# IGNF/StrataNet2-Vegetation-Coverage-Maps

Measured on AMD Instinct MI355X. Metric: plots/s fwd+bwd, 32k-pt synthetic plots, batch 16/GPU, higher is better.
Workload: dtype f32; 1 GPU; C2 ref-arch: 16 plots/GPU x 32768 pts, SA npoint 1024/256 + global, r 1/2 m, train step fwd+P2+loss+bwd+Adam, inputs resident in HBM; plots_per_gpu=16, points_per_plot=32768, batches_per_geometry_pass=8, exchange=none (single GPU), parallelism=single GPU, ranks_seen=1, exchange_in_graph=False

## Files before the change

### include/strata_hip.h

```cpp
#ifndef STRATA_HIP_H
#define STRATA_HIP_H

#include <stddef.h>

#ifdef __cplusplus
extern "C" {
#endif

#define SN2_VERSION 102
#define SN2_EINVAL (-1)
#define SN2_ELIMIT (-2)

#define SN2_MAX_NEIGHBORS 2000
#define SN2_STAT_SLOTS 1024

int sn2_version(void);
int sn2_debug_mfma_chain(const float *a, const float *b, float *d, int mode, void *stream);
int sn2_debug_spin(int blocks, long long clocks, int *out, void *stream);

int sn2_debug_fp1_backward_parts(int mask);
int sn2_debug_fp_rows_form(int form);
int sn2_debug_fp_table_form(int form);
#define SN2_PROBE_SINK_WORDS 4096
int sn2_debug_stream_probe(const float *src, float *dst, size_t n_floats, int mode, float *sink, void *stream);
// ... 35 lines not shown
int sn2_fps_waves(const float *pos_soa, int B, int N, int M, const int *start, int *idx, float *cpos_soa,
                  float *cpos_aos, int *order_ws, int waves, void *stream);
int sn2_fps_status(const float *pos_soa, int B, int N, int M, const int *start, int *idx, float *cpos_soa,
                   float *cpos_aos, int *order_ws, int waves, unsigned *status, void *stream);
int sn2_fps_live(const float *pos_soa, int B, int N, int M, const int *start, const int *n_live, int *idx, float *cpos_soa,
                 float *cpos_aos, int *order_ws, int waves, int *n_live_out, unsigned *status, void *stream);
int sn2_debug_fps_spin_limit(unsigned sweeps);

int sn2_ball_query(const float *src_soa, int B, int N, const float *cpos_soa, int M, float r2, int cap,
                   int *nbr, int *cnt, unsigned long long *total, const int *fps_ws, void *stream);

int sn2_count_sum(const int *cnt, int n, unsigned long long *total, void *stream);
int sn2_count_sum_group(const int *cnt, int G, int n, unsigned long long *total, size_t total_stride, void *stream);

#define SN2_THREE_NN_WS_WORDS(B, S) ((size_t)(B) * (4 * (size_t)(S) + 1032))
size_t sn2_three_nn_ws_words(int B, int S);
int sn2_three_nn(const float *src_soa, int B, int S, const float *dst_soa, int T, int k, int *idx, float *w,
                 void *ws, const int *dst_fps_ws, void *stream);
#define SN2_THREE_NN_XY_WS_WORDS(B, S, T) ((size_t)(B) * (4 * (size_t)(S) + 5 * (size_t)(T) + 1032))
size_t sn2_three_nn_xy_ws_words(int B, int S, int T);
int sn2_three_nn_xy(const float *src_soa, int B, int S, const float *dst_soa, int T, int k, int *idx, float *w,
                    void *ws, void *stream);

int sn2_prepare_plots(const float *raw, long T, const int *offsets, const float *centers, const float *fake_xy, int n_fake,
                      const int *idx, int B, int N, int train, const double *rot, const int *flips, const float *noise,
                      const long *noise_offsets, long noise_T, float z_max, float *cloud, float *xyz, void *stream);

#define SN2_SUBSAMPLE_LDS 1
#define SN2_SUBSAMPLE_GLOBAL 2
#define SN2_SUBSAMPLE_COARSE 4
#define SN2_SUBSAMPLE_LDS_MAX 16384
int sn2_subsample_form(int n_max, int N);
size_t sn2_subsample_ws_words(int B, int n_max, int N, int form);
int sn2_subsample(const int *offsets, int extra, int n_max, int B, int N, unsigned long long seed, const long long *plot_keys,
                  int form, int *ws, size_t ws_words, int *idx, void *stream);

int sn2_train_batch_ws_words(int B, int n_max, int N, size_t *words);
int sn2_train_batch(const float *raw, long T, const int *offsets, const float *centers, const double *coverages, int P,
                    const int *plot_ids, int B, const float *fake_xy, int n_fake, int n_max, int N, int M1, float z_max,
                    unsigned long long seed, long long epoch, const double *cos_sin, int train, int noise, int *ws,
                    size_t ws_words, float *cloud, float *xyz, double *gt, int *fps_start, void *stream);
int sn2_train_batch_live(const float *raw, long T, const int *offsets, const float *centers, const double *coverages, int P,
                         const int *plot_ids, int B, const float *fake_xy, int n_fake, int n_max, int N, int M1, float z_max,
                         unsigned long long seed, long long epoch, const double *cos_sin, int train, int noise, int *ws,
                         size_t ws_words, float *cloud, float *xyz, double *gt, int *fps_start, int *n_live, void *stream);

int sn2_plots_append(const float *src_raw, long src_T, const int *src_offsets, const float *src_centers, const float *src_cov,
                     const int *sel, int K, float *dst_raw, long cap_T, int *dst_offsets, float *dst_centers, double *dst_cov,
                     int cap_P, int P0, long T0, const int *dst_start, long new_T, void *stream);

#define SN2_ZNORM_WS_WORDS(n, cells) ((size_t)5 * (n) + 3 * (size_t)(cells) + 8)
size_t sn2_znorm_ws_words(int n, long cells);
int sn2_znorm(const float *x, const float *y, const float *z, int n, float radius, float x_min, float y_min, float x_max,
              float y_max, int *ws, float *zmin, float *z_out, void *stream);

size_t sn2_parcel_count_ws_words(int P, int rows);
size_t sn2_parcel_znorm_ws_words(long T, float radius, float x_min, float y_min, float x_max, float y_max);
int sn2_parcel_count(const float *cloud, long T, int L, int rows, const float *centers, int P, const int *cell_start,
                     const int *cell_items, int GX, int GY, double gx0, double gy0, double cell_inv, float radius, int *ws,
                     size_t ws_words, int *prefix, long long *total, void *stream);
int sn2_parcel_fill(const float *cloud, long T, int L, int rows, const float *centers, int P, const int *cell_start,
                    const int *cell_items, int GX, int GY, double gx0, double gy0, double cell_inv, float radius, int *prefix,
                    const int *plot_base, long sum_n, float *raw, int *point_index, void *stream);
int sn2_parcel_znorm(const float *cloud, long T, float x_min, float y_min, float x_max, float y_max, float radius,
                     float disc_radius, const int *offsets, const float *centers, int P, const int *point_index, long sum_n,
                     int *ws, size_t ws_words, float *raw, void *stream);

typedef struct sn2_sa {
    int B, Nsrc, M, cap;
    int cf;
    int nl;
    const float *feat; int feat_stride;
    const float *spos; int spos_stride;
    const float *cpos;
    const int *nbr, *cnt;
    const unsigned long long *total;
    const int *order;
    sn2_block blk[2];
    float *ext; int *arg;
    float *out;
    const float *dout;
    float *dfeat;
    float *bwd_ws;
} sn2_sa;
#define SN2_SA_BWD_WS_REPLICAS 32
#define SN2_SA_BWD_WS_WORDS (SN2_SA_BWD_WS_REPLICAS * 2 * 16 * 12)
#define SN2_SA_SOLO_MIN 64
#define SN2_SA_QUAD_MIN 8
#define SN2_SA_OCT_MIN 4
#define SN2_SA_SOLO_FLAG 0x40000000
#define SN2_SA_OCT_FLAG 0x20000000
#define SN2_SA_PACKED_ITEMS(M) ((M) / 8 + 2)
#define SN2_SA_ORDER_WORDS(B, M) ((size_t)4 * (B) * (M) + (size_t)16 * (B) * SN2_SA_PACKED_ITEMS(M) + 8)
size_t sn2_sa_order_words(int B, int M);
int sn2_sa_order(const int *cnt, int B, int M, int *order, void *stream);
int sn2_sa_order_group(const int *cnt, int G, int B, int M, int *order, size_t stride_words, void *stream);
int sn2_sa_forward(const sn2_sa *p, int training, void *stream);
int sn2_sa_backward(const sn2_sa *p, void *stream);

typedef struct sn2_fp {
    int B, R_per_plot, S_per_plot;
    int ca, cb;
    const float *src; int src_stride; const float *src_a, *src_c;
    const int *knn_idx; const float *knn_w;
    const float *skip; int skip_stride;
    sn2_block blk;
    float *h; int h_stride;
    const float *dy;
    float *dsrc; int dsrc_stride;
    float *dskip; int dskip_stride;
    float *du_scratch;
    float *scatter_ws;
    int scatter_ready;
    const int *bn_sums_done;
    float *src_ws;
    int act_bf16;
    const int *row_perm;
} sn2_fp;
#define SN2_INTERP_CHUNKS(R, S) ((3 * (size_t)(R) + 62) / 63 + (size_t)(S))
#define SN2_FP_SRC_WS_WORDS(B, R, S, cout) ((size_t)(B) * SN2_INTERP_CHUNKS(R, S) * ((((cout) + 3) / 4) * 4))
size_t sn2_interp_chunks(int R_per_plot, int S_per_plot);
size_t sn2_fp_src_ws_words(int B, int R_per_plot, int S_per_plot, int cout);
#define SN2_INTERP_WS_WORDS(B, R, S) \
    ((size_t)(B) * (S) * (((R) + 2047) / 2048 + 6) + 6 * (size_t)(B) * (R) + 64 + 4 * (size_t)(B) * SN2_INTERP_CHUNKS(R, S))
size_t sn2_interp_ws_words(int B, int R_per_plot, int S_per_plot);
int sn2_interp_index(const int *knn_idx, const float *knn_w, const float *src_pos, int B, int R_per_plot,
                     int S_per_plot, float *ws, void *stream);
int sn2_interp_index_perm(const int *knn_idx, const float *knn_w, const float *src_pos, const int *row_perm, int B,
                          int R_per_plot, int S_per_plot, float *ws, void *stream);
int sn2_interp_index_group(const int *knn_idx, const float *knn_w, const float *src_pos, const int *row_perm, int G, int B,
                           int R_per_plot, int S_per_plot, float *ws, size_t ws_stride_words, void *stream);
int sn2_fp_forward(const sn2_fp *p, int training, void *stream);
int sn2_fp_backward(const sn2_fp *p, void *stream);

int sn2_plot_max_forward(const float *h, const float *a, const float *c, int B, int R_per_plot, int C, float *out,
                         int *arg, void *stream);
int sn2_plot_max_backward(const float *dout, const int *arg, int B, int R_per_plot, int C, float *dy, void *stream);

int sn2_global_pool_backward(const float *du, int du_stride, const int *arg, const float *h, const float *mean,
                             const float *invstd, int B, int R_per_plot, int C, float *dx, float *dy, float *dgamma,
                             float *dbeta, void *stream);

#define SN2_GLOBAL_MAX_PLOTS 28
#define SN2_GLOBAL_XCHG_WORDS(B) ((size_t)2 * (size_t)(B) * 4 * 128)
#define SN2_GLOBAL_CTL_WORDS 8
size_t sn2_global_xchg_words(int B);
int sn2_global_level_forward(const sn2_fp *sa3, const sn2_fp *fp3, float *x3, int *arg3, unsigned long long *xchg,
                             unsigned *ctl, void *stream);
#define SN2_GLOBAL_BWD_MAX_ROWS 256
#define SN2_GLOBAL_BWD_XCHG_WORDS ((size_t)2 * SN2_GLOBAL_MAX_PLOTS * 128)
#define SN2_GLOBAL_BWD_CTL_WORDS 64
int sn2_global_level_backward(const sn2_fp *sa3, const sn2_fp *fp3, const int *arg3, unsigned long long *xchg, unsigned *ctl,
                              void *stream);
int sn2_debug_global_spin_limit(unsigned sweeps);

#define SN2_HEAD_LOSS_MAX_PLOTS 128
typedef struct sn2_loss_grad {
    const float *pred;
    const double *gt;
    const float *proba;
    const double *pdf;
    const double *grad_total;
    const int *arg, *nocc, *pix;
    int B, N, D;
    double m, e;
} sn2_loss_grad;

typedef struct sn2_head {
    int R, cin, f_stride;
    const float *f, *fa, *fc;
    const float *W1, *b1, *W2, *b2;
    float *coverages, *proba;
    const float *dcoverages, *dproba;
    float *dy;
    float *dW1, *db1, *dW2, *db2;
    int grad_replicas, grad_replica_stride;
    const int *drop_mask;
    float drop_scale;
    int act_bf16;
    float *zero_fill; long zero_fill_words;
    const sn2_loss_grad *loss;
} sn2_head;
int sn2_head_forward(const sn2_head *p, void *stream);
int sn2_fp_head_eval(const sn2_fp *p, const sn2_head *hd, void *stream);
int sn2_head_backward(const sn2_head *p, void *stream);
int sn2_debug_head_backward_occupancy(int bf16, int with_loss);
int sn2_head_bn_sums(const sn2_head *p, const float *gamma, const float *beta, const float *mean, const float *invstd,
                     float *dgamma, float *dbeta, int *ok, void *stream);
int sn2_fp_bn_sums(const sn2_fp *p, const float *gamma, const float *beta, const float *mean, const float *invstd,
                   float *dgamma, float *dbeta, int *ok, void *stream);


int sn2_plot_project_forward(const float *pred_pointwise, const float *cloud_xy, long plot_stride, int B, int N,
                             int D, unsigned long long *keys, int *pix, int *arg, int *nocc, float *pred,
                             void *stream);
#define SN2_P2_KEY_PARTS(N) (((N) + 4095) / 4096 < 1 ? 1 : (((N) + 4095) / 4096 > 64 ? 64 : ((N) + 4095) / 4096))
size_t sn2_p2_key_parts(int N);
int sn2_plot_pixels(const float *cloud_xy, long plot_stride, int B, int N, int D, float *mm, int *pix, void *stream);
int sn2_plot_project_forward_pix(const float *pred_pointwise, const int *pix, int B, int N, int D,
                                 unsigned long long *keys, int *arg, int *nocc, float *pred, void *stream);
int sn2_plot_project_backward(const float *dpred, const int *arg, const int *nocc, const int *pix, int B, int N,
                              int D, float *dpointwise, void *stream);

int sn2_raster_project(const float *coverages, const float *cloud_xy, long plot_stride, int B, int N, int D,
                       int diam_meters, unsigned long long *keys, int *pix, float *rasters, void *stream);

int sn2_mosaic_merge(const float *rasters, const float *weights, const int *offsets, int B, int D, int H, int W,
                     float *mean, float *wsum, int win_y0, int win_x0, int win_h, int win_w, void *stream);

#define SN2_MOSAIC_HIST_WORDS 10004
int sn2_mosaic_finalize(const float *mean, const float *wsum, int H, int W, int *hist_ws, double *sum_ws, float *thr_out,
                        float *out, void *stream);

#define SN2_MOSAIC_CROP_MAX_BANDS 8
#define SN2_MOSAIC_CROP_MAX_EDGES (1 << 20)
#define SN2_MOSAIC_CROP_MAX_BLOCKS 2048
#define SN2_MOSAIC_CROP_BLOCKS(H, W) \
    ((size_t)(H) * (((size_t)(W) + 255) / 256) < SN2_MOSAIC_CROP_MAX_BLOCKS ? (size_t)(H) * (((size_t)(W) + 255) / 256) \
                                                                           : (size_t)SN2_MOSAIC_CROP_MAX_BLOCKS)
#define SN2_MOSAIC_CROP_WS_WORDS(C, H, W) (4 * (size_t)(C) * SN2_MOSAIC_CROP_BLOCKS(H, W))
extern size_t sn2_mosaic_crop_ws_words(int C, int H, int W);
int sn2_mosaic_crop_stats(float *bands, int C, int H, int W, double x_min, double y_max, double pix, const double *edges, int E,
                          void *ws, double *mean, long long *count, void *stream);

#define SN2_ATLAS_CANVAS_COLS 8
#define SN2_ATLAS_SEG_COLS 8
#define SN2_ATLAS_FINALIZE_MAX_BLOCKS 1024
#define SN2_ATLAS_FINALIZE_BLOCKS(H, W) \
    (((size_t)(H) * (size_t)(W) + 255) / 256 < SN2_ATLAS_FINALIZE_MAX_BLOCKS ? ((size_t)(H) * (size_t)(W) + 255) / 256 \
                                                                            : (size_t)SN2_ATLAS_FINALIZE_MAX_BLOCKS)
int sn2_atlas_canvas_table(int K, const int *H, const int *W, const double *x_min, const double *y_max, long long *table);

int sn2_atlas_merge(const float *rasters, const float *weights, const int *place, int B, int D, int K, const long long *canvas_host,
                    const long long *canvas_dev, const int *seg_host, const int *seg_dev, int S, float *mean, float *wsum,
                    void *stream);

#define SN2_ATLAS_FINALIZE_CANVAS_WORDS (SN2_MOSAIC_HIST_WORDS + 2 * SN2_ATLAS_FINALIZE_MAX_BLOCKS)
#define SN2_ATLAS_FINALIZE_WS_WORDS(K) ((size_t)(K) * SN2_ATLAS_FINALIZE_CANVAS_WORDS)
int sn2_atlas_finalize_ws_words(int K, size_t *words);
int sn2_atlas_finalize(const float *mean, const float *wsum, int K, const long long *canvas_host, const long long *canvas_dev,
                       void *ws, float *thr, float *bands, void *stream);

int sn2_atlas_crop_stats(float *bands, int C, int K, const long long *canvas_host, const long long *canvas_dev, double pix,
                         const double *edges, const int *edge_start_host, const int *edge_start_dev, void *ws, double *mean,
                         long long *count, void *stream);

int sn2_kde_lookup(const float *cloud, int B, int C, int N, int z_channel, float z_max, const double *X, const double *Y,
                   int K, double *pdf, void *stream);
#define SN2_KDE_FIT_MAX_K 65536
#define SN2_KDE_FIT_ABS_SLOTS 256
#define SN2_KDE_FIT_SLICES 8
#define SN2_KDE_FIT_WS_WORDS(K) \
    (2 * ((4 + 3 * SN2_KDE_FIT_SLICES) * (size_t)(K) + 3 * (((size_t)(K) + 255) / 256)) + SN2_KDE_FIT_ABS_SLOTS)
size_t sn2_kde_fit_ws_words(int K);
int sn2_kde_fit(const float *z, long n, double bw, int K, void *ws, double *X, double *Y, void *stream);
#define SN2_LOSS_BLOCKS 1024
int sn2_loss_forward(const float *pred, const double *gt, int B, const float *proba, const double *pdf, int R, double m,
                     double e, double *partials, double *out, void *stream);
int sn2_loss_backward(const float *pred, const double *gt, int B, const float *proba, const double *pdf, int R, double m,
                      double e, const double *grad_total, float *dpred, float *dproba, void *stream);

#define SN2_PROJECTED_LOSS_WS (2 * 512 + 2)
int sn2_projected_loss_forward(const float *coverages, const int *pix, const float *proba, const double *pdf, const double *gt,
                               int B, int N, int D, double m, double e, unsigned long long *keys, int *arg, int *nocc,
                               float *pred, double *partials, double *out, void *stream);
int sn2_projected_loss_backward(const float *pred, const double *gt, int B, const float *proba, const double *pdf, int N, int D,
                                double m, double e, const double *grad_total, const int *arg, const int *nocc, const int *pix,
                                float *dcoverages, float *dproba, void *stream);

#define SN2_PLOT_LOSSES_SLICE_ROWS 2048
#define SN2_PLOT_LOSSES_SLICES(N) \
    (((N) + SN2_PLOT_LOSSES_SLICE_ROWS - 1) / SN2_PLOT_LOSSES_SLICE_ROWS < 1 ? 1 : \
     (((N) + SN2_PLOT_LOSSES_SLICE_ROWS - 1) / SN2_PLOT_LOSSES_SLICE_ROWS > 64 ? 64 : ((N) + SN2_PLOT_LOSSES_SLICE_ROWS - 1) / SN2_PLOT_LOSSES_SLICE_ROWS))
size_t sn2_plot_losses_ws_words(int B, int N, int D);
int sn2_plot_losses(const float *coverages, const int *pix, const float *proba, const double *pdf, const double *gt, int B, int N,
                    int D, double m, double e, void *ws, float *pred, double *out, void *stream);

int sn2_adam_step(float *param, const float *grad, float *exp_avg, float *exp_avg_sq, int n, float lr, float beta1,
                  float beta2, float eps, float weight_decay, int *step_dev ,
                  float grad_scale, void *stream);

#define SN2_METER_TERMS 4
int sn2_adam_step_dev(float *param, const float *grad, float *exp_avg, float *exp_avg_sq, int n, const float *lr_dev, float beta1,
                      float beta2, float eps, float weight_decay, int *step_dev, float grad_scale, const double *terms, int n_terms,
                      double *meter, void *stream);


typedef struct sn2_net_layer {
    int cin, cout;
    const float *W, *b, *gamma, *beta;
    float *running_mean, *running_var;
    long long *num_batches_tracked;
    int gW, gb, ggamma, gbeta;
    int mma_bf16;
} sn2_net_layer;

typedef struct sn2_net_model {
    sn2_net_layer sa1[2], sa2, sa3, fp3, fp2, fp1;
    const float *lin1_W, *lin1_b, *lin2_W, *lin2_b;
    int g_lin1_W, g_lin1_b, g_lin2_W, g_lin2_b;
    int n_flat;
    float r1_sq, r2_sq;
    int max_neighbors;
    float drop_p;
    int fuse_global_level;
    int fuse_eval_head;
    int source_side;
    int fps_waves_shared, fps_waves_many;
} sn2_net_model;

typedef struct sn2_net_dims {
    int B, N, M1, M2;
    int cap1, cap2;
    int act_bf16;
    int p2_diam_pix;
} sn2_net_dims;

typedef struct sn2_net_geo {
    const float *xyz;
    int *idx1; float *pos1_soa, *pos1_aos; int *ws1;
    int *nbr1, *cnt1; unsigned long long *tot1; int *ord1;
    int *idx2; float *pos2_soa, *pos2_aos; int *ws2;
    int *nbr2, *cnt2; unsigned long long *tot2; int *ord2;
    const float *pos3;
    int *knn3_idx; float *knn3_w;
    int *knn2_idx; float *knn2_w;
    int *knn1_idx; float *knn1_w;
    float *inv3, *inv2, *inv1;
    int *nn_ws2, *nn_ws1;
    const int *rank1;
    float *rows0;
    int *p2_pix; float *p2_mm;
} sn2_net_geo;

typedef struct sn2_net_act {
    float *aux;
    float *stats;
    float *ext1; int *arg1; float *x1;
    float *ext2; int *arg2; float *x2;
    float *h_sa3, *h3;
    float *x3; int *arg3;
    float *h2;
    void *h1;
    float *src_ws1, *src_ws2;
    float *cov, *proba;
    const int *drop_mask;
    float *bwd_arena; long bwd_arena_words;
} sn2_net_act;

#define SN2_NET_GRAD_IMAGES 32
typedef struct sn2_net_bwd {
    const float *dcov, *dproba;
    float *arena; long arena_words;
    int images, image_stride;
    float *dy2, *dy3, *dx1, *dx2, *dx3, *dy_sa3;
    float *sa1_ws;
    void *dy1, *du1;
    float *du2, *du3;
    int *bn_ok;
    float *src_ws1, *src_ws2;
    int defer_grad_reduce;
    int arena_is_zero;
    int frozen_stats;
    unsigned long long *gl_xchg; unsigned *gl_ctl;
    const sn2_loss_grad *loss;
} sn2_net_bwd;

#define SN2_NET_FORK 1
#define SN2_NET_SHARED 2
#define SN2_NET_INVERTED 4
#define SN2_NET_DEFER_JOIN 8
#define SN2_NET_INPUT_ONLY 16
#define SN2_NET_HAS_ROWS0 32
#define SN2_NET_JOIN_PENDING 64
#define SN2_NET_WITH_GEOMETRY 128
#define SN2_NET_HAS_INVERTED 256

typedef struct sn2_net_io {
    const float *cloud;
    const int *fps_start;
    unsigned *fps_status;
    unsigned long long *gl_xchg; unsigned *gl_ctl;
    void *stream_b, *stream_c, *stream_pack;
    void *ctx;
    int flags;
    int training;
    const int *fps_live;
    int *fps_live1;
} sn2_net_io;

int sn2_net_ctx_create(void **ctx);
int sn2_net_ctx_destroy(void *ctx);
int sn2_net_geo_carve(const sn2_net_model *m, const sn2_net_dims *d, void *base, sn2_net_geo *out, size_t *bytes);
int sn2_net_act_carve(const sn2_net_model *m, const sn2_net_dims *d, int training, void *base, sn2_net_act *out, size_t *bytes);
int sn2_net_bwd_carve(const sn2_net_model *m, const sn2_net_dims *d, void *arena_base, void *scratch_base, sn2_net_bwd *out,
                      size_t *arena_bytes, size_t *scratch_bytes);
int sn2_net_geometry(const sn2_net_model *m, const sn2_net_dims *d, const sn2_net_geo *g, const sn2_net_io *io, void *stream);
int sn2_net_forward(const sn2_net_model *m, const sn2_net_dims *d, const sn2_net_geo *g, const sn2_net_act *a,
                    const sn2_net_io *io, void *stream);
int sn2_net_backward(const sn2_net_model *m, const sn2_net_dims *d, const sn2_net_geo *g, const sn2_net_act *a,
                     const sn2_net_bwd *b, void *stream);

int sn2_adam_step_images(float *param, float *grad_images, int replicas, int stride, float *exp_avg, float *exp_avg_sq, int n,
                         float lr, float beta1, float beta2, float eps, float weight_decay, int *step_dev, float grad_scale,
                         void *stream);
int sn2_adam_step_images_dev(float *param, float *grad_images, int replicas, int stride, float *exp_avg, float *exp_avg_sq, int n,
                             const float *lr_dev, float beta1, float beta2, float eps, float weight_decay, int *step_dev,
                             float grad_scale, const double *terms, int n_terms, double *meter, void *stream);

int sn2_fps_fills_ws(int B, int N, int M);
int sn2_three_nn_uses_grid(int S, int T);
int sn2_fp_rows_small(long R);
int sn2_fp_source_side(long R, int cb, int force);
int sn2_global_level_forward_route(int B, int bf16);
int sn2_global_level_backward_route(int B, int M2, int frozen, int bf16);
int sn2_head_loss_route(int B, int N, int D);

#ifdef __cplusplus
}
#endif
#endif
```

### stratanet2_vegetation_coverage_maps_amd/_lib.py

```python
import ctypes
import functools
import os
from ctypes import POINTER, Structure, c_double, c_float, c_int, c_long, c_longlong, c_void_p

HERE = os.path.dirname(os.path.abspath(__file__))
LIB_PATH = os.path.join(HERE, "csrc", "libstrata_hip.so")

CONSTANTS = {
    "SN2_VERSION": 102, "SN2_EINVAL": -1, "SN2_ELIMIT": -2,
    "SN2_MAX_NEIGHBORS": 2000, "SN2_STAT_SLOTS": 1024, "SN2_BN_FROZEN_KEEP": 2,
    "SN2_FPS_WS_GRID_WORDS": 4104, "SN2_FPS_WS_CTL_WORDS": 32,
    "SN2_SUBSAMPLE_LDS": 1, "SN2_SUBSAMPLE_GLOBAL": 2, "SN2_SUBSAMPLE_COARSE": 4, "SN2_SUBSAMPLE_LDS_MAX": 16384,
    "SN2_SA_BWD_WS_WORDS": 32 * 2 * 16 * 12,
    "SN2_GLOBAL_MAX_PLOTS": 28, "SN2_GLOBAL_CTL_WORDS": 8, "SN2_GLOBAL_BWD_MAX_ROWS": 256,
    "SN2_GLOBAL_BWD_XCHG_WORDS": 2 * 28 * 128, "SN2_GLOBAL_BWD_CTL_WORDS": 64,
    "SN2_MOSAIC_HIST_WORDS": 10004, "SN2_MOSAIC_CROP_MAX_BANDS": 8, "SN2_MOSAIC_CROP_MAX_EDGES": 1 << 20,
    "SN2_MOSAIC_CROP_MAX_BLOCKS": 2048, "SN2_ATLAS_CANVAS_COLS": 8, "SN2_ATLAS_SEG_COLS": 8, "SN2_ATLAS_FINALIZE_MAX_BLOCKS": 1024,
    "SN2_ATLAS_FINALIZE_CANVAS_WORDS": 10004 + 2 * 1024, "SN2_KDE_FIT_MAX_K": 65536, "SN2_LOSS_BLOCKS": 1024, "SN2_PROJECTED_LOSS_WS": 2 * 512 + 2,
    "SN2_NET_GRAD_IMAGES": 32, "SN2_METER_TERMS": 4,
    "SN2_NET_FORK": 1, "SN2_NET_SHARED": 2, "SN2_NET_INVERTED": 4, "SN2_NET_DEFER_JOIN": 8, "SN2_NET_INPUT_ONLY": 16,
    "SN2_NET_HAS_ROWS0": 32, "SN2_NET_JOIN_PENDING": 64, "SN2_NET_WITH_GEOMETRY": 128, "SN2_NET_HAS_INVERTED": 256,
}
globals().update(CONSTANTS)
MAX_NEIGHBORS, STAT_SLOTS, BN_FROZEN_KEEP = CONSTANTS["SN2_MAX_NEIGHBORS"], CONSTANTS["SN2_STAT_SLOTS"], CONSTANTS["SN2_BN_FROZEN_KEEP"]
(NET_FORK, NET_SHARED, NET_INVERTED, NET_DEFER_JOIN, NET_INPUT_ONLY, NET_HAS_ROWS0, NET_JOIN_PENDING, NET_WITH_GEOMETRY,
 NET_HAS_INVERTED) = (CONSTANTS["SN2_NET_" + n] for n in ("FORK", "SHARED", "INVERTED", "DEFER_JOIN", "INPUT_ONLY", "HAS_ROWS0",
                                                          "JOIN_PENDING", "WITH_GEOMETRY", "HAS_INVERTED"))


class Block(Structure):
    _fields_ = [("cin", c_int), ("cout", c_int), ("W", c_void_p), ("b", c_void_p), ("gamma", c_void_p),
                ("beta", c_void_p), ("running_mean", c_void_p), ("running_var", c_void_p), ("a", c_void_p),
                ("c", c_void_p), ("mean", c_void_p), ("invstd", c_void_p), ("stat_slots", c_void_p),
                ("dW", c_void_p), ("db", c_void_p), ("dgamma", c_void_p), ("dbeta", c_void_p),
                ("grad_replicas", c_int), ("grad_replica_stride", c_int), ("mma_bf16", c_int),
                ("num_batches_tracked", c_void_p), ("frozen_stats", c_int)]


class SA(Structure):
    _fields_ = [("B", c_int), ("Nsrc", c_int), ("M", c_int), ("cap", c_int), ("cf", c_int), ("nl", c_int),
                ("feat", c_void_p), ("feat_stride", c_int), ("spos", c_void_p), ("spos_stride", c_int),
                ("cpos", c_void_p), ("nbr", c_void_p), ("cnt", c_void_p), ("total", c_void_p), ("order", c_void_p),
                ("blk", Block * 2),
                ("ext", c_void_p), ("arg", c_void_p), ("out", c_void_p), ("dout", c_void_p), ("dfeat", c_void_p),
                ("bwd_ws", c_void_p)]


class FP(Structure):
    _fields_ = [("B", c_int), ("R_per_plot", c_int), ("S_per_plot", c_int), ("ca", c_int), ("cb", c_int),
                ("src", c_void_p), ("src_stride", c_int), ("src_a", c_void_p), ("src_c", c_void_p),
                ("knn_idx", c_void_p), ("knn_w", c_void_p), ("skip", c_void_p), ("skip_stride", c_int),
                ("blk", Block), ("h", c_void_p), ("h_stride", c_int), ("dy", c_void_p), ("dsrc", c_void_p),
                ("dsrc_stride", c_int), ("dskip", c_void_p), ("dskip_stride", c_int), ("du_scratch", c_void_p),
                ("scatter_ws", c_void_p), ("scatter_ready", c_int), ("bn_sums_done", c_void_p), ("src_ws", c_void_p),
                ("act_bf16", c_int), ("row_perm", c_void_p)]


class LossGrad(Structure):
    _fields_ = [(n, c_void_p) for n in ("pred", "gt", "proba", "pdf", "grad_total", "arg", "nocc", "pix")] + [
        ("B", c_int), ("N", c_int), ("D", c_int), ("m", c_double), ("e", c_double)]


class Head(Structure):
    _fields_ = [("R", c_int), ("cin", c_int), ("f_stride", c_int), ("f", c_void_p), ("fa", c_void_p),
                ("fc", c_void_p), ("W1", c_void_p), ("b1", c_void_p), ("W2", c_void_p), ("b2", c_void_p),
                ("coverages", c_void_p), ("proba", c_void_p), ("dcoverages", c_void_p), ("dproba", c_void_p),
                ("dy", c_void_p), ("dW1", c_void_p), ("db1", c_void_p), ("dW2", c_void_p), ("db2", c_void_p),
                ("grad_replicas", c_int), ("grad_replica_stride", c_int), ("drop_mask", c_void_p), ("drop_scale", c_float),
                ("act_bf16", c_int), ("zero_fill", c_void_p), ("zero_fill_words", c_long), ("loss", POINTER(LossGrad))]


class NetLayer(Structure):
    _fields_ = [("cin", c_int), ("cout", c_int), ("W", c_void_p), ("b", c_void_p), ("gamma", c_void_p), ("beta", c_void_p),
                ("running_mean", c_void_p), ("running_var", c_void_p), ("num_batches_tracked", c_void_p),
                ("gW", c_int), ("gb", c_int), ("ggamma", c_int), ("gbeta", c_int), ("mma_bf16", c_int)]


class NetModel(Structure):
    _fields_ = [("sa1", NetLayer * 2), ("sa2", NetLayer), ("sa3", NetLayer), ("fp3", NetLayer), ("fp2", NetLayer), ("fp1", NetLayer),
                ("lin1_W", c_void_p), ("lin1_b", c_void_p), ("lin2_W", c_void_p), ("lin2_b", c_void_p),
                ("g_lin1_W", c_int), ("g_lin1_b", c_int), ("g_lin2_W", c_int), ("g_lin2_b", c_int), ("n_flat", c_int),
                ("r1_sq", c_float), ("r2_sq", c_float), ("max_neighbors", c_int), ("drop_p", c_float),
                ("fuse_global_level", c_int), ("fuse_eval_head", c_int), ("source_side", c_int),
                ("fps_waves_shared", c_int), ("fps_waves_many", c_int)]


class NetDims(Structure):
    _fields_ = [("B", c_int), ("N", c_int), ("M1", c_int), ("M2", c_int), ("cap1", c_int), ("cap2", c_int), ("act_bf16", c_int),
                ("p2_diam_pix", c_int)]


class NetGeo(Structure):
    _fields_ = [(n, c_void_p) for n in (
        "xyz", "idx1", "pos1_soa", "pos1_aos", "ws1", "nbr1", "cnt1", "tot1", "ord1",
        "idx2", "pos2_soa", "pos2_aos", "ws2", "nbr2", "cnt2", "tot2", "ord2", "pos3",
        "knn3_idx", "knn3_w", "knn2_idx", "knn2_w", "knn1_idx", "knn1_w", "inv3", "inv2", "inv1", "nn_ws2", "nn_ws1",
        "rank1", "rows0", "p2_pix", "p2_mm")]


class NetAct(Structure):
    _fields_ = [(n, c_void_p) for n in (
        "aux", "stats", "ext1", "arg1", "x1", "ext2", "arg2", "x2", "h_sa3", "h3", "x3", "arg3", "h2", "h1", "src_ws1", "src_ws2",
        "cov", "proba", "drop_mask", "bwd_arena")] + [("bwd_arena_words", c_long)]


class NetBwd(Structure):
    _fields_ = [("dcov", c_void_p), ("dproba", c_void_p), ("arena", c_void_p), ("arena_words", c_long), ("images", c_int),
                ("image_stride", c_int)] + [(n, c_void_p) for n in (
                    "dy2", "dy3", "dx1", "dx2", "dx3", "dy_sa3", "sa1_ws", "dy1", "du1", "du2", "du3", "bn_ok", "src_ws1", "src_ws2")] + [
                        ("defer_grad_reduce", c_int), ("arena_is_zero", c_int), ("frozen_stats", c_int), ("gl_xchg", c_void_p),
                        ("gl_ctl", c_void_p), ("loss", POINTER(LossGrad))]


class NetIO(Structure):
    _fields_ = [("cloud", c_void_p), ("fps_start", c_void_p), ("fps_status", c_void_p), ("gl_xchg", c_void_p), ("gl_ctl", c_void_p),
                ("stream_b", c_void_p), ("stream_c", c_void_p), ("stream_pack", c_void_p), ("ctx", c_void_p), ("flags", c_int),
                ("training", c_int), ("fps_live", c_void_p), ("fps_live1", c_void_p)]


SIGNATURES = {
    "sn2_version": [],
    "sn2_debug_mfma_chain": [c_void_p, c_void_p, c_void_p, c_int, c_void_p],
    "sn2_debug_spin": [c_int, c_longlong, c_void_p, c_void_p],
    "sn2_debug_fp1_backward_parts": [c_int],
    "sn2_debug_fp_rows_form": [c_int],
    "sn2_debug_fp_table_form": [c_int],
    "sn2_debug_stream_probe": [c_void_p, c_void_p, ctypes.c_size_t, c_int, c_void_p, c_void_p],
    "sn2_debug_mfma_probe": [c_int, c_int, c_void_p, POINTER(c_double), c_void_p],
    "sn2_pack_rows": [c_void_p, c_void_p, c_int, c_int, c_int, c_void_p, c_void_p],
    "sn2_fps": [c_void_p, c_int, c_int, c_int, c_void_p, c_void_p, c_void_p, c_void_p, c_void_p, c_void_p],
    "sn2_fps_waves": [c_void_p, c_int, c_int, c_int, c_void_p, c_void_p, c_void_p, c_void_p, c_void_p, c_int, c_void_p],
    "sn2_fps_status": [c_void_p, c_int, c_int, c_int, c_void_p, c_void_p, c_void_p, c_void_p, c_void_p, c_int, c_void_p, c_void_p],
    "sn2_fps_live": [c_void_p, c_int, c_int, c_int, c_void_p, c_void_p, c_void_p, c_void_p, c_void_p, c_void_p, c_int, c_void_p, c_void_p,
                     c_void_p],
    "sn2_debug_fps_spin_limit": [ctypes.c_uint],
    "sn2_ball_query": [c_void_p, c_int, c_int, c_void_p, c_int, c_float, c_int, c_void_p, c_void_p, c_void_p, c_void_p,
                       c_void_p],
    "sn2_three_nn": [c_void_p, c_int, c_int, c_void_p, c_int, c_int, c_void_p, c_void_p, c_void_p, c_void_p, c_void_p],
    "sn2_count_sum": [c_void_p, c_int, c_void_p, c_void_p],
    "sn2_count_sum_group": [c_void_p, c_int, c_int, c_void_p, ctypes.c_size_t, c_void_p],
    "sn2_three_nn_xy": [c_void_p, c_int, c_int, c_void_p, c_int, c_int, c_void_p, c_void_p, c_void_p, c_void_p],
    "sn2_prepare_plots": [c_void_p, c_long, c_void_p, c_void_p, c_void_p, c_int, c_void_p, c_int, c_int, c_int, c_void_p,
                          c_void_p, c_void_p, c_void_p, c_long, c_float, c_void_p, c_void_p, c_void_p],
    "sn2_znorm": [c_void_p, c_void_p, c_void_p, c_int, c_float, c_float, c_float, c_float, c_float, c_void_p, c_void_p,
                  c_void_p, c_void_p],
    "sn2_parcel_count": [c_void_p, c_long, c_int, c_int, c_void_p, c_int, c_void_p, c_void_p, c_int, c_int, c_double, c_double,
                         c_double, c_float, c_void_p, ctypes.c_size_t, c_void_p, c_void_p, c_void_p],
    "sn2_parcel_fill": [c_void_p, c_long, c_int, c_int, c_void_p, c_int, c_void_p, c_void_p, c_int, c_int, c_double, c_double,
                        c_double, c_float, c_void_p, c_void_p, c_long, c_void_p, c_void_p, c_void_p],
    "sn2_parcel_znorm": [c_void_p, c_long, c_float, c_float, c_float, c_float, c_float, c_float, c_void_p, c_void_p, c_int,
                         c_void_p, c_long, c_void_p, ctypes.c_size_t, c_void_p, c_void_p],
    "sn2_subsample_form": [c_int, c_int],
    "sn2_subsample": [c_void_p, c_int, c_int, c_int, c_int, ctypes.c_ulonglong, c_void_p, c_int, c_void_p, ctypes.c_size_t,
                      c_void_p, c_void_p],
    "sn2_train_batch_ws_words": [c_int, c_int, c_int, POINTER(ctypes.c_size_t)],
    "sn2_train_batch": [c_void_p, c_long, c_void_p, c_void_p, c_void_p, c_int, c_void_p, c_int, c_void_p, c_int, c_int, c_int, c_int,
                        c_float, ctypes.c_ulonglong, c_longlong, c_void_p, c_int, c_int, c_void_p, ctypes.c_size_t, c_void_p, c_void_p,
                        c_void_p, c_void_p, c_void_p],
    "sn2_train_batch_live": [c_void_p, c_long, c_void_p, c_void_p, c_void_p, c_int, c_void_p, c_int, c_void_p, c_int, c_int, c_int, c_int,
                             c_float, ctypes.c_ulonglong, c_longlong, c_void_p, c_int, c_int, c_void_p, ctypes.c_size_t, c_void_p,
                             c_void_p, c_void_p, c_void_p, c_void_p, c_void_p],
    "sn2_plots_append": [c_void_p, c_long, c_void_p, c_void_p, c_void_p, c_void_p, c_int, c_void_p, c_long, c_void_p, c_void_p,
                         c_void_p, c_int, c_int, c_long, c_void_p, c_long, c_void_p],
    "sn2_sa_order": [c_void_p, c_int, c_int, c_void_p, c_void_p],
    "sn2_sa_order_group": [c_void_p, c_int, c_int, c_int, c_void_p, ctypes.c_size_t, c_void_p],
    "sn2_sa_forward": [POINTER(SA), c_int, c_void_p],
    "sn2_sa_backward": [POINTER(SA), c_void_p],
    "sn2_grad_reduce": [c_void_p, c_int, c_int, c_int, c_void_p],
    "sn2_interp_index": [c_void_p, c_void_p, c_void_p, c_int, c_int, c_int, c_void_p, c_void_p],
    "sn2_interp_index_perm": [c_void_p, c_void_p, c_void_p, c_void_p, c_int, c_int, c_int, c_void_p, c_void_p],
    "sn2_interp_index_group": [c_void_p, c_void_p, c_void_p, c_void_p, c_int, c_int, c_int, c_int, c_void_p, ctypes.c_size_t, c_void_p],
    "sn2_fp_forward": [POINTER(FP), c_int, c_void_p],
    "sn2_fp_backward": [POINTER(FP), c_void_p],
    "sn2_plot_max_forward": [c_void_p, c_void_p, c_void_p, c_int, c_int, c_int, c_void_p, c_void_p, c_void_p],
    "sn2_plot_max_backward": [c_void_p, c_void_p, c_int, c_int, c_int, c_void_p, c_void_p],
    "sn2_global_pool_backward": [c_void_p, c_int, c_void_p, c_void_p, c_void_p, c_void_p, c_int, c_int, c_int, c_void_p, c_void_p,
                                 c_void_p, c_void_p, c_void_p],
    "sn2_global_level_forward": [POINTER(FP), POINTER(FP), c_void_p, c_void_p, c_void_p, c_void_p, c_void_p],
    "sn2_global_level_backward": [POINTER(FP), POINTER(FP), c_void_p, c_void_p, c_void_p, c_void_p],
    "sn2_debug_global_spin_limit": [ctypes.c_uint],
    "sn2_head_forward": [POINTER(Head), c_void_p],
    "sn2_fp_head_eval": [POINTER(FP), POINTER(Head), c_void_p],
    "sn2_fp_bn_sums": [POINTER(FP), c_void_p, c_void_p, c_void_p, c_void_p, c_void_p, c_void_p, c_void_p, c_void_p],
    "sn2_head_bn_sums": [POINTER(Head), c_void_p, c_void_p, c_void_p, c_void_p, c_void_p, c_void_p, c_void_p, c_void_p],
    "sn2_head_backward": [POINTER(Head), c_void_p],
    "sn2_debug_head_backward_occupancy": [c_int, c_int],
    "sn2_plot_project_forward": [c_void_p, c_void_p, c_long, c_int, c_int, c_int, c_void_p, c_void_p, c_void_p,
                                 c_void_p, c_void_p, c_void_p],
    "sn2_plot_pixels": [c_void_p, c_long, c_int, c_int, c_int, c_void_p, c_void_p, c_void_p],
    "sn2_plot_project_forward_pix": [c_void_p, c_void_p, c_int, c_int, c_int, c_void_p, c_void_p, c_void_p, c_void_p, c_void_p],
    "sn2_plot_project_backward": [c_void_p, c_void_p, c_void_p, c_void_p, c_int, c_int, c_int, c_void_p, c_void_p],
    "sn2_raster_project": [c_void_p, c_void_p, c_long, c_int, c_int, c_int, c_int, c_void_p, c_void_p, c_void_p,
                           c_void_p],
    "sn2_mosaic_merge": [c_void_p, c_void_p, c_void_p, c_int, c_int, c_int, c_int, c_void_p, c_void_p,
                         c_int, c_int, c_int, c_int, c_void_p],
    "sn2_mosaic_finalize": [c_void_p, c_void_p, c_int, c_int, c_void_p, c_void_p, c_void_p, c_void_p, c_void_p],
    "sn2_mosaic_crop_stats": [c_void_p, c_int, c_int, c_int, c_double, c_double, c_double, c_void_p, c_int, c_void_p, c_void_p,
                              c_void_p, c_void_p],
    "sn2_atlas_canvas_table": [c_int, c_void_p, c_void_p, c_void_p, c_void_p, c_void_p],
    "sn2_atlas_finalize_ws_words": [c_int, POINTER(ctypes.c_size_t)],
    "sn2_atlas_merge": [c_void_p, c_void_p, c_void_p, c_int, c_int, c_int, c_void_p, c_void_p, c_void_p, c_void_p, c_int, c_void_p,
                        c_void_p, c_void_p],
    "sn2_atlas_finalize": [c_void_p, c_void_p, c_int, c_void_p, c_void_p, c_void_p, c_void_p, c_void_p, c_void_p],
    "sn2_atlas_crop_stats": [c_void_p, c_int, c_int, c_void_p, c_void_p, c_double, c_void_p, c_void_p, c_void_p, c_void_p, c_void_p,
                             c_void_p, c_void_p],
    "sn2_kde_lookup": [c_void_p, c_int, c_int, c_int, c_int, c_float, c_void_p, c_void_p, c_int, c_void_p, c_void_p],
    "sn2_kde_fit": [c_void_p, c_long, c_double, c_int, c_void_p, c_void_p, c_void_p, c_void_p],
    "sn2_loss_forward": [c_void_p, c_void_p, c_int, c_void_p, c_void_p, c_int, c_double, c_double, c_void_p, c_void_p,
                         c_void_p],
    "sn2_loss_backward": [c_void_p, c_void_p, c_int, c_void_p, c_void_p, c_int, c_double, c_double, c_void_p, c_void_p,
                          c_void_p, c_void_p],
    "sn2_adam_step": [c_void_p, c_void_p, c_void_p, c_void_p, c_int, c_float, c_float, c_float, c_float, c_float,
                      c_void_p, c_float, c_void_p],
    "sn2_adam_step_dev": [c_void_p, c_void_p, c_void_p, c_void_p, c_int, c_void_p, c_float, c_float, c_float, c_float,
                          c_void_p, c_float, c_void_p, c_int, c_void_p, c_void_p],
    "sn2_projected_loss_forward": [c_void_p, c_void_p, c_void_p, c_void_p, c_void_p, c_int, c_int, c_int, c_double, c_double, c_void_p,
                                   c_void_p, c_void_p, c_void_p, c_void_p, c_void_p, c_void_p],
    "sn2_projected_loss_backward": [c_void_p, c_void_p, c_int, c_void_p, c_void_p, c_int, c_int, c_double, c_double, c_void_p, c_void_p,
                                    c_void_p, c_void_p, c_void_p, c_void_p, c_void_p],
    "sn2_plot_losses": [c_void_p, c_void_p, c_void_p, c_void_p, c_void_p, c_int, c_int, c_int, c_double, c_double, c_void_p, c_void_p,
                        c_void_p, c_void_p],
    "sn2_adam_step_images": [c_void_p, c_void_p, c_int, c_int, c_void_p, c_void_p, c_int, c_float, c_float, c_float, c_float, c_float,
                             c_void_p, c_float, c_void_p],
    "sn2_adam_step_images_dev": [c_void_p, c_void_p, c_int, c_int, c_void_p, c_void_p, c_int, c_void_p, c_float, c_float, c_float,
                                 c_float, c_void_p, c_float, c_void_p, c_int, c_void_p, c_void_p],
    "sn2_net_ctx_create": [POINTER(c_void_p)],
    "sn2_net_ctx_destroy": [c_void_p],
    "sn2_net_geo_carve": [POINTER(NetModel), POINTER(NetDims), c_void_p, POINTER(NetGeo), POINTER(ctypes.c_size_t)],
    "sn2_net_act_carve": [POINTER(NetModel), POINTER(NetDims), c_int, c_void_p, POINTER(NetAct), POINTER(ctypes.c_size_t)],
    "sn2_net_bwd_carve": [POINTER(NetModel), POINTER(NetDims), c_void_p, c_void_p, POINTER(NetBwd), POINTER(ctypes.c_size_t),
                          POINTER(ctypes.c_size_t)],
    "sn2_net_geometry": [POINTER(NetModel), POINTER(NetDims), POINTER(NetGeo), POINTER(NetIO), c_void_p],
    "sn2_net_forward": [POINTER(NetModel), POINTER(NetDims), POINTER(NetGeo), POINTER(NetAct), POINTER(NetIO), c_void_p],
    "sn2_net_backward": [POINTER(NetModel), POINTER(NetDims), POINTER(NetGeo), POINTER(NetAct), POINTER(NetBwd), c_void_p],
    "sn2_fps_fills_ws": [c_int, c_int, c_int],
    "sn2_three_nn_uses_grid": [c_int, c_int],
    "sn2_fp_rows_small": [c_long],
    "sn2_fp_source_side": [c_long, c_int, c_int],
    "sn2_global_level_forward_route": [c_int, c_int],
    "sn2_global_level_backward_route": [c_int, c_int, c_int, c_int],
    "sn2_head_loss_route": [c_int, c_int, c_int],
}

SIZE_HELPERS = {
    "sn2_fps_ws_words": [c_int, c_int],
    "sn2_fps_ws_grid_offset": [c_int, c_int],
    "sn2_fps_ws_ctl_offset": [c_int, c_int],
    "sn2_fps_ws_rank_offset": [c_int, c_int],
    "sn2_three_nn_ws_words": [c_int, c_int],
    "sn2_three_nn_xy_ws_words": [c_int, c_int, c_int],
    "sn2_znorm_ws_words": [c_int, c_long],
    "sn2_sa_order_words": [c_int, c_int],
    "sn2_interp_chunks": [c_int, c_int],
    "sn2_interp_ws_words": [c_int, c_int, c_int],
    "sn2_fp_src_ws_words": [c_int, c_int, c_int, c_int],
    "sn2_global_xchg_words": [c_int],
    "sn2_p2_key_parts": [c_int],
    "sn2_kde_fit_ws_words": [c_int],
    "sn2_parcel_count_ws_words": [c_int, c_int],
    "sn2_parcel_znorm_ws_words": [c_long, c_float, c_float, c_float, c_float, c_float],
    "sn2_subsample_ws_words": [c_int, c_int, c_int, c_int],
    "sn2_plot_losses_ws_words": [c_int, c_int, c_int],
}

EXTERN_SIZE_HELPERS = {
    "sn2_mosaic_crop_ws_words": [c_int, c_int, c_int],
}

_lib = None


class StrataHipError(RuntimeError):
    pass


def load():
    global _lib
    if _lib is not None:
        return _lib
    if not os.path.exists(LIB_PATH):
        raise StrataHipError(
            f"{LIB_PATH} not found: build it with `python -m stratanet2_vegetation_coverage_maps_amd._build` "
            "(or __graft_entry__.build()); the HIP library is mandatory, there is no fallback path")
    lib = ctypes.CDLL(LIB_PATH)
    for name, argtypes in SIGNATURES.items():
        fn = getattr(lib, name)
        fn.argtypes = argtypes
        fn.restype = c_int
    for name, argtypes in list(SIZE_HELPERS.items()) + list(EXTERN_SIZE_HELPERS.items()):
        fn = getattr(lib, name)
        fn.argtypes = argtypes
        fn.restype = ctypes.c_size_t
    if lib.sn2_version() != SN2_VERSION:
        raise StrataHipError(f"libstrata_hip.so version {lib.sn2_version()} != binding {SN2_VERSION}: rebuild")
    _lib = lib
    return lib


@functools.lru_cache(maxsize=4096)
def host_value(name: str, *args) -> int:
    return getattr(load(), name)(*args)


def check(rc: int, what: str):
    if rc != 0:
        kind = "hipError_t" if rc > 0 else {-1: "SN2_EINVAL", -2: "SN2_ELIMIT"}.get(rc, "error")
        raise StrataHipError(f"{what} failed: {kind} {rc}")
```

### stratanet2_vegetation_coverage_maps_amd/csrc/common.h

```cpp
#pragma once
#include <hip/hip_runtime.h>
#include <stdint.h>

#include "../../include/strata_hip.h"

#define SN2_WAVE 64

#define SN2_RETURN_LAUNCH()                                   \
    do {                                                      \
        hipError_t e__ = hipGetLastError();                   \
        return e__ == hipSuccess ? 0 : (int)e__;              \
    } while (0)

#define SN2_TRY(expr)                \
    do {                             \
        int r__ = (expr);            \
        if (r__ != 0) return r__;    \
    } while (0)

#ifdef SN2_NO_FLUSH
#define SN2_FLUSH_ADD(ptr, v) do { if ((v) == 12345.678f) atomicAdd((ptr), (v)); } while (0)
#else
#define SN2_FLUSH_ADD(ptr, v) atomicAdd((ptr), (v))
#endif

#ifdef __HIPCC__
__device__ __forceinline__ int sn2_grad_image(int replicas, int stride) {
    return replicas > 1 ? (int)(blockIdx.x % (unsigned)replicas) * stride : 0;
}
#endif

static inline int sn2_cdiv(long a, long b) { return (int)((a + b - 1) / b); }

constexpr int GL_MAX_PLOTS = SN2_GLOBAL_MAX_PLOTS;
constexpr int GL_BWD_MAX_ROWS = SN2_GLOBAL_BWD_MAX_ROWS;

#ifdef __HIPCC__
static __global__ __launch_bounds__(256) void sn2_fill_words_kernel(uint32_t* __restrict__ p, uint32_t v, size_t n) {
    for (size_t i = (size_t)blockIdx.x * 256 + threadIdx.x; i < n; i += (size_t)gridDim.x * 256) p[i] = v;
}
static inline void sn2_fill_words(void* p, uint32_t v, size_t nwords, hipStream_t st) {
    if (nwords == 0) return;
    int grid = sn2_cdiv((long)nwords, 256 * 4);
    grid = grid < 1 ? 1 : (grid > 2048 ? 2048 : grid);
    hipLaunchKernelGGL(sn2_fill_words_kernel, dim3(grid), dim3(256), 0, st, (uint32_t*)p, v, nwords);
}
#endif

static inline bool sn2_small_sort_wg(int B) { return B > 32; }

static inline int sn2_cu_count() {
    static int n = 0;
    if (n == 0) {
        int dev = 0, v = 0;
        if (hipGetDevice(&dev) == hipSuccess &&
            hipDeviceGetAttribute(&v, hipDeviceAttributeMultiprocessorCount, dev) == hipSuccess && v > 0)
            n = v;
        else
            n = 256;
    }
    return n;
}

int sn2_subsample_ids(const int* offsets, const int* ids, int extra, int n_max, int B, int N, unsigned long long seed,
                      const long long* plot_keys, int form, int* ws, size_t ws_words, int* idx, hipStream_t stream);

typedef const float __attribute__((address_space(4)))* cfp;
__device__ __forceinline__ cfp as_const(const float* p) { return (cfp)(uintptr_t)p; }
__device__ __forceinline__ cfp opaque(cfp p) {
    uint64_t v = (uint64_t)p;
    asm volatile("" : "+s"(v));
    return (cfp)v;
}

__device__ __forceinline__ float sn2_d2(float ax, float ay, float az, float bx, float by, float bz) {
#pragma clang fp contract(off)
    float dx = ax - bx;
    float dy = ay - by;
    float dz = az - bz;
    float xx = dx * dx;
    float yy = dy * dy;
    float zz = dz * dz;
    float s = xx + yy;
    return s + zz;
}

__device__ __forceinline__ unsigned long long wave_max_u64(unsigned long long v) {
#pragma unroll
    for (int o = 32; o > 0; o >>= 1) {
        unsigned long long t = __shfl_xor(v, o);
        v = t > v ? t : v;
    }
    return v;
}

#define SN2_DPP(x, ctrl, rmask) __builtin_amdgcn_update_dpp((x), (x), (ctrl), (rmask), 0xF, false)
__device__ __forceinline__ float wave_max_dpp(float v) {
    v = fmaxf(v, __int_as_float(SN2_DPP(__float_as_int(v), 0xB1, 0xF)));
    v = fmaxf(v, __int_as_float(SN2_DPP(__float_as_int(v), 0x4E, 0xF)));
    v = fmaxf(v, __int_as_float(SN2_DPP(__float_as_int(v), 0x141, 0xF)));
    v = fmaxf(v, __int_as_float(SN2_DPP(__float_as_int(v), 0x140, 0xF)));
    v = fmaxf(v, __int_as_float(SN2_DPP(__float_as_int(v), 0x142, 0xA)));
    v = fmaxf(v, __int_as_float(SN2_DPP(__float_as_int(v), 0x143, 0xC)));
    return __int_as_float(__builtin_amdgcn_readlane(__float_as_int(v), 63));
}
__device__ __forceinline__ float wave_min_dpp(float v) { return -wave_max_dpp(-v); }
__device__ __forceinline__ float wave_sum_dpp(float v) {
    v += __int_as_float(SN2_DPP(__float_as_int(v), 0xB1, 0xF));
    v += __int_as_float(SN2_DPP(__float_as_int(v), 0x4E, 0xF));
    v += __int_as_float(SN2_DPP(__float_as_int(v), 0x141, 0xF));
    v += __int_as_float(SN2_DPP(__float_as_int(v), 0x140, 0xF));
// ... 28 lines not shown
```

### stratanet2_vegetation_coverage_maps_amd/csrc/global_level_bwd.hip

```cpp
#include <type_traits>
#include "global_level.h"

namespace {

#ifdef SN2_GB_STAMPS
__device__ unsigned long long g_gb_dbg[16];
extern "C" int sn2_debug_gb_stamps(unsigned long long* out) {
    return (int)hipMemcpyFromSymbol(out, HIP_SYMBOL(g_gb_dbg), sizeof(g_gb_dbg));
}
#define BSTAMP(i)                                                                                   \
    if (blockIdx.x == 0 && threadIdx.x == 0) {                                                      \
        unsigned long long t_;                                                                      \
        asm volatile("s_memtime %0\n\ts_waitcnt lgkmcnt(0)" : "=s"(t_)::"memory");                   \
        g_gb_dbg[i] = t_;                                                                           \
    }
#else
#define BSTAMP(i)
#endif
constexpr int GB_QS = OuterAcc<16, 36>::QS;
constexpr int GB_LD = 68;
constexpr int GB_WC = 33;
constexpr int GB_TILES = GL_GROUPS * 64 * (GB_QS + GB_LD);
constexpr int GB_FIXED_FLOATS = GB_TILES + 128 * GB_WC + 8 * 64 + 16 * 128 + 2 * 128 + 4 * 64;
static_assert(GB_QS >= 48, "three 16-column tiles of staged inputs");
static_assert(GL_GROUPS * 128 * 37 <= GB_TILES, "the groups' dW | db partials go through the staging tiles");
static_assert((GB_FIXED_FLOATS + GL_MAX_PLOTS * 128) * 4 <= 160 * 1024, "LDS");

struct GbLayer {
    const float *W, *gamma, *mean, *invstd, *h;
    float *dW, *db, *dgamma, *dbeta;
};
struct GbArgs {
    int B, M2;
    const float* x2;
    const float* pos2;
    const float* x3;
    const int* arg3;
    const float* dy3;
    float* dx2;
    float* dx3;
    GbLayer sa3, fp3;
    int img_stride;
    gl_u64* xchg;
    unsigned* ctl;
    unsigned spin_limit;
};

__device__ __forceinline__ void gb_wave_sums(float (&s)[4], float* s_red, int wv, int lane, int off) {
#pragma unroll
    for (int t = 0; t < 4; ++t) {
        s[t] += __shfl_xor(s[t], 16);
        s[t] += __shfl_xor(s[t], 32);
    }
    if (lane < 16) {
#pragma unroll
        for (int t = 0; t < 4; ++t) s_red[wv * 128 + off + 4 * lane + t] = s[t];
    }
}

template <bool ONE_TRIP>
__device__ __forceinline__ bool gb_plot(const GbArgs& A, float* smem, int b, unsigned epoch, bool publish_only, bool repair) {
    const int tid = threadIdx.x, lane = tid & 63, t256 = tid & 255;
    const int grp = __builtin_amdgcn_readfirstlane(tid >> 8), g = __builtin_amdgcn_readfirstlane((tid >> 6) & 3);
    const int wv = __builtin_amdgcn_readfirstlane(tid >> 6);
    float* s_q = smem + grp * 64 * GB_QS;
    float* s_p = smem + GL_GROUPS * 64 * GB_QS + grp * 64 * GB_LD;
    float* s_wc = smem + GB_TILES;
    float* s_par = s_wc + 128 * GB_WC;
    float* s_cf = s_par + 6 * 64;
    float* s_red = s_cf + 2 * 64;
    float* s_bnf = s_red + 16 * 128;
    float* s_bn3 = s_bnf + 128;
    float* s_sdp = s_bn3 + 128;
    float* s_g = s_sdp + 64;
    float* s_x3 = s_g + 64;
    int* s_arg = reinterpret_cast<int*>(s_x3 + 64);
    float* s_x = s_x3 + 128;
    __shared__ int s_fail;
    const int B = A.B, M2 = A.M2;
    const long row_lo = (long)b * M2, R_lim = row_lo + M2;
    const int nblk = (M2 + 63) >> 6, trips = ONE_TRIP ? 1 : (nblk + GL_GROUPS - 1) / GL_GROUPS;
    const float invR = 1.0f / (float)(B * M2);
    const int qd = t256 & 15, rw = t256 >> 4;
    const int r4 = lane >> 4, c16 = lane & 15;
    const int n_gran = B * 128;
    gl_u64* xa = A.xchg;
    gl_u64* xb = A.xchg + GL_MAX_PLOTS * 128;
    const unsigned tag_a = epoch * 2u, tag_b = epoch * 2u + 1u;
    __syncthreads();
    BSTAMP(0)
#pragma unroll
    for (int j = 0; j < 4; ++j) {
        const int i = tid + 1024 * j, k = i >> 5, c = i & 31;
        s_wc[k * GB_WC + c] = k < 64 ? A.fp3.W[k * 96 + 64 + c] : A.sa3.W[(k - 64) * 35 + c];
    }
    float wa[4];
#pragma unroll
    for (int j = 0; j < 4; ++j) wa[j] = A.fp3.W[(4 * (tid >> 6) + j) * 96 + (tid & 63)];
    float dx3_old = 0.f, xh_arg = 0.f;
    bool arg_ok = false;
    if (tid < 64) {
        s_par[0 * 64 + tid] = A.fp3.mean[tid], s_par[1 * 64 + tid] = A.fp3.invstd[tid], s_par[2 * 64 + tid] = A.fp3.gamma[tid];
        const float m3 = A.sa3.mean[tid], is3 = A.sa3.invstd[tid];
        s_par[3 * 64 + tid] = m3, s_par[4 * 64 + tid] = is3, s_par[5 * 64 + tid] = A.sa3.gamma[tid];
        s_x3[tid] = A.x3[(size_t)b * 64 + tid];
        const int ra = A.arg3[(size_t)b * 64 + tid];
        arg_ok = ra >= 0 && ra < M2;
        s_arg[tid] = arg_ok ? ra : -1;
        if (arg_ok) xh_arg = (A.sa3.h[(size_t)(row_lo + ra) * 64 + tid] - m3) * is3;
        dx3_old = A.dx3[(size_t)b * 64 + tid];
    }
    if (tid == 0) s_fail = 0;
    if constexpr (ONE_TRIP) {
        if (grp < nblk)
            stage_inputs<32, 3, false>(s_q, GB_QS, g, lane, row_lo + (long)grp * 64, (int)R_lim, M2, M2, A.x2, 32, nullptr, nullptr, nullptr,
                                       nullptr, A.pos2, 4);
    }
    float4 hv[4], dv[4];
    auto load_rows = [&](const float* __restrict__ p, long r0, float4 (&v)[4]) {
#pragma unroll
        for (int u = 0; u < 4; ++u) {
            const long r = r0 + rw + 16 * u;
            v[u] = reinterpret_cast<const float4*>(p + (size_t)(r < R_lim ? r : R_lim - 1) * 64)[qd];
        }
    };
    __syncthreads();
    BSTAMP(1)
    auto quad = [&](const float* p, float (&v)[4]) {
        const float4 q = *reinterpret_cast<const float4*>(p + 4 * qd);
        v[0] = q.x, v[1] = q.y, v[2] = q.z, v[3] = q.w;
    };
    {
        float s1[4] = {0.f, 0.f, 0.f, 0.f}, s2[4] = {0.f, 0.f, 0.f, 0.f}, mean_f[4], is_f[4];
        quad(s_par, mean_f), quad(s_par + 64, is_f);
        for (int it = 0; it < trips; ++it) {
            const int blk = it * GL_GROUPS + grp;
            const long r0 = row_lo + (long)blk * 64;
            if (blk < nblk) {
                load_rows(A.fp3.h, r0, hv);
                load_rows(A.dy3, r0, dv);
#pragma unroll
                for (int u = 0; u < 4; ++u) {
                    const bool live = r0 + rw + 16 * u < R_lim;
                    const float hq[4] = {hv[u].x, hv[u].y, hv[u].z, hv[u].w}, dq[4] = {dv[u].x, dv[u].y, dv[u].z, dv[u].w};
#pragma unroll
                    for (int t = 0; t < 4; ++t) {
                        const float dd = live ? dq[t] : 0.f;
                        s1[t] += dd;
                        s2[t] = fmaf(dd, (hq[t] - mean_f[t]) * is_f[t], s2[t]);
                    }
                }
            }
        }
        gb_wave_sums(s1, s_red, wv, lane, 0);
        gb_wave_sums(s2, s_red, wv, lane, 64);
        __syncthreads();
        if (tid < 128) {
            float v = 0.f;
#pragma unroll
            for (int w = 0; w < 16; ++w) v += s_red[w * 128 + tid];
            __hip_atomic_store(xa + (size_t)b * 128 + tid, ((gl_u64)tag_a << 32) | (gl_u64)__float_as_uint(v), __ATOMIC_RELAXED,
                               __HIP_MEMORY_SCOPE_AGENT);
        }
    }
    BSTAMP(2)
    if (!gl_collect(xa, n_gran, tag_a, s_x, A.spin_limit)) s_fail = 1;
    __syncthreads();
    BSTAMP(3)
    if (s_fail) {
        if (!repair && tid < 128)
            __hip_atomic_store(xb + (size_t)b * 128 + tid, (gl_u64)(tag_b ^ GL_POISON) << 32, __ATOMIC_RELAXED, __HIP_MEMORY_SCOPE_AGENT);
        return false;
    }
    if (tid < 128) {
        double acc = 0.0;
        for (int w = 0; w < B; ++w) acc += (double)s_x[w * 128 + tid];
        s_bnf[tid] = (float)acc;
        s_cf[tid] = (float)acc * invR;
    }
    __syncthreads();
    auto dp_of = [&](float hh, float dd, float mean, float is, float gam, float dbeta_r, float dgamma_r, bool live) {
        const float xh = (hh - mean) * is;
        const float dh = gam * is * (dd - dbeta_r - xh * dgamma_r);
        return (live && hh > 0.f) ? dh : 0.f;
    };
    auto stage_dp_fp3 = [&](long r0, float (&sd)[4]) {
        float mean_f[4], is_f[4], gam_f[4], dbt_f[4], dgm_f[4];
        quad(s_par, mean_f), quad(s_par + 64, is_f), quad(s_par + 128, gam_f), quad(s_cf, dbt_f), quad(s_cf + 64, dgm_f);
#pragma unroll
        for (int u = 0; u < 4; ++u) {
            const bool live = r0 + rw + 16 * u < R_lim;
            const float hq[4] = {hv[u].x, hv[u].y, hv[u].z, hv[u].w}, dq[4] = {dv[u].x, dv[u].y, dv[u].z, dv[u].w};
            float p[4];
#pragma unroll
            for (int t = 0; t < 4; ++t) {
                p[t] = dp_of(hq[t], dq[t], mean_f[t], is_f[t], gam_f[t], dbt_f[t], dgm_f[t], live);
                sd[t] += p[t];
            }
            *reinterpret_cast<float4*>(&s_p[(rw + 16 * u) * GB_LD + 4 * qd]) = make_float4(p[0], p[1], p[2], p[3]);
        }
    };
    {
        float sd[4] = {0.f, 0.f, 0.f, 0.f};
        for (int it = 0; it < trips; ++it) {
            const int blk = it * GL_GROUPS + grp;
            const long r0 = row_lo + (long)blk * 64;
            if (blk < nblk) {
                if constexpr (!ONE_TRIP) {
                    load_rows(A.fp3.h, r0, hv);
                    load_rows(A.dy3, r0, dv);
                }
                stage_dp_fp3(r0, sd);
            }
        }
        gb_wave_sums(sd, s_red, wv, lane, 0);
        __syncthreads();
        if (tid < 64) {
            float v = 0.f;
#pragma unroll
            for (int w = 0; w < 16; ++w) v += s_red[w * 128 + tid];
            s_sdp[tid] = v;
        }
        __syncthreads();
        {
            const int part = tid >> 6;
            float acc = 0.f;
#pragma unroll
            for (int j = 0; j < 4; ++j) acc = fmaf(s_sdp[4 * part + j], wa[j], acc);
            s_red[part * 128 + 64 + (tid & 63)] = acc;
        }
        __syncthreads();
        if (tid < 64) {
            float v = 0.f;
#pragma unroll
            for (int k = 0; k < 16; ++k) v += s_red[k * 128 + 64 + tid];
            const float gg = dx3_old + v;
            s_g[tid] = gg;
            const float g1 = arg_ok ? gg : 0.f;
            __hip_atomic_store(xb + (size_t)b * 128 + tid, ((gl_u64)tag_b << 32) | (gl_u64)__float_as_uint(g1), __ATOMIC_RELAXED,
                               __HIP_MEMORY_SCOPE_AGENT);
            __hip_atomic_store(xb + (size_t)b * 128 + 64 + tid, ((gl_u64)tag_b << 32) | (gl_u64)__float_as_uint(g1 * xh_arg),
                               __ATOMIC_RELAXED, __HIP_MEMORY_SCOPE_AGENT);
        }
    }
    BSTAMP(4)
    if (publish_only) return true;
    f32x4 acc_f[2], acc_3[3];
    f32x4 D[2];
    acc_f[0] = acc_f[1] = acc_3[0] = acc_3[1] = acc_3[2] = D[0] = D[1] = f32x4{0.f, 0.f, 0.f, 0.f};
    float4 hs[4];
    float dx2_old[2][4];
    auto ask_block = [&](long r0) {
#pragma unroll
        for (int jt = 0; jt < 2; ++jt)
#pragma unroll
            for (int r = 0; r < 4; ++r) {
                const long row = r0 + 16 * g + 4 * r4 + r;
                dx2_old[jt][r] = A.dx2[(size_t)(row < R_lim ? row : R_lim - 1) * 32 + 16 * jt + c16];
            }
        load_rows(A.sa3.h, r0, hs);
    };
    auto contract_tile = [&](auto& acc, auto nt, int k0) {
        constexpr int NT = decltype(nt)::value;
#pragma unroll 4
        for (int st = 0; st < 16; ++st) {
            const float av = s_p[(4 * st + r4) * GB_LD + 16 * g + c16];
#pragma unroll
            for (int c = 0; c < NT; ++c)
                acc[c] = __builtin_amdgcn_mfma_f32_16x16x4f32(av, s_q[(4 * st + r4) * GB_QS + 16 * c + c16], acc[c], 0, 0, 0);
        }
#pragma unroll 4
        for (int kb = 0; kb < 16; ++kb) {
            const float av = s_p[(16 * g + c16) * GB_LD + 4 * kb + r4];
#pragma unroll
            for (int jt = 0; jt < 2; ++jt)
                D[jt] = __builtin_amdgcn_mfma_f32_16x16x4f32(av, s_wc[(k0 + 4 * kb + r4) * GB_WC + 16 * jt + c16], D[jt], 0, 0, 0);
        }
    };
    if constexpr (ONE_TRIP) {
        if (grp < nblk) {
            ask_block(row_lo + (long)grp * 64);
            contract_tile(acc_f, std::integral_constant<int, 2>{}, 0);
        }
    }
    if (!gl_collect(xb, n_gran, tag_b, s_x, A.spin_limit)) s_fail = 1;
    __syncthreads();
    BSTAMP(5)
    if (s_fail) return false;
    if (tid < 128) {
        double acc = 0.0;
        for (int w = 0; w < B; ++w) acc += (double)s_x[w * 128 + tid];
        s_bn3[tid] = (float)acc;
    }
    __syncthreads();
    for (int it = 0; it < trips; ++it) {
        const int blk = it * GL_GROUPS + grp;
        const long r0 = row_lo + (long)blk * 64;
        const bool act = blk < nblk;
        if constexpr (!ONE_TRIP) {
            if (act) {
                ask_block(r0);
                stage_inputs<32, 3, false>(s_q, GB_QS, g, lane, r0, (int)R_lim, M2, M2, A.x2, 32, nullptr, nullptr, nullptr, nullptr,
                                           A.pos2, 4);
                float sd[4] = {0.f, 0.f, 0.f, 0.f};
                load_rows(A.fp3.h, r0, hv);
                load_rows(A.dy3, r0, dv);
                stage_dp_fp3(r0, sd);
            }
            __syncthreads();
            D[0] = D[1] = f32x4{0.f, 0.f, 0.f, 0.f};
            if (act) contract_tile(acc_f, std::integral_constant<int, 2>{}, 0);
            __syncthreads();
        }
        if (act) {
#pragma unroll
            for (int u = 0; u < 4; ++u) {
                const int rp = blk * 64 + rw + 16 * u;
                const bool live = rp < M2;
                const float hq[4] = {hs[u].x, hs[u].y, hs[u].z, hs[u].w};
                float p[4];
#pragma unroll
                for (int t = 0; t < 4; ++t) {
                    const int c = 4 * qd + t;
                    const float dd = s_arg[c] == rp ? s_g[c] : 0.f;
                    p[t] = dp_of(hq[t], dd, s_par[3 * 64 + c], s_par[4 * 64 + c], s_par[5 * 64 + c], s_bn3[c] * invR, s_bn3[64 + c] * invR, live);
                }
                *reinterpret_cast<float4*>(&s_p[(rw + 16 * u) * GB_LD + 4 * qd]) = make_float4(p[0], p[1], p[2], p[3]);
            }
        }
        __syncthreads();
        if (act) {
            contract_tile(acc_3, std::integral_constant<int, 3>{}, 64);
#pragma unroll
            for (int jt = 0; jt < 2; ++jt)
#pragma unroll
                for (int r = 0; r < 4; ++r) {
                    const long row = r0 + 16 * g + 4 * r4 + r;
                    if (row < R_lim) A.dx2[(size_t)row * 32 + 16 * jt + c16] = dx2_old[jt][r] + D[jt][r];
                }
        }
        __syncthreads();
    }
    BSTAMP(6)
    {
        float* s_acc = smem;
        const int img = b * A.img_stride;
        float* dst[5];
        float old[5], old_o[4], old_bn[2] = {0.f, 0.f};
#pragma unroll
        for (int j = 0; j < 5; ++j) {
            const int i = tid + 1024 * j, o = i / 36, k = i - o * 36;
            dst[j] = nullptr;
            if (i < 128 * 36) {
                if (o < 64) {
                    if (k < 32) dst[j] = A.fp3.dW + img + o * 96 + 64 + k;
                    else if (k == 35) dst[j] = A.fp3.db + img + o;
                } else {
                    dst[j] = k < 35 ? A.sa3.dW + img + (o - 64) * 35 + k : A.sa3.db + img + (o - 64);
                }
            }
            old[j] = dst[j] ? *dst[j] : 0.f;
        }
#pragma unroll
        for (int j = 0; j < 4; ++j) {
            const int i = tid + 1024 * j;
            old_o[j] = A.fp3.dW[img + (i >> 6) * 96 + (i & 63)];
        }
        float* bn_dst[2] = {nullptr, nullptr};
        if (b == 0 && tid < 128) {
            bn_dst[0] = tid < 64 ? A.fp3.dbeta + tid : A.fp3.dgamma + (tid - 64);
            bn_dst[1] = tid < 64 ? A.sa3.dbeta + tid : A.sa3.dgamma + (tid - 64);
            old_bn[0] = *bn_dst[0], old_bn[1] = *bn_dst[1];
        }
#pragma unroll
        for (int c = 0; c < 3; ++c)
#pragma unroll
            for (int q = 0; q < 4; ++q) {
                const int o = 16 * g + 4 * r4 + q, k = 16 * c + c16;
                if (k < 36) {
                    if (c < 2) s_acc[(grp * 128 + o) * 37 + k] = acc_f[c][q];
                    s_acc[(grp * 128 + 64 + o) * 37 + k] = acc_3[c][q];
                }
            }
        __syncthreads();
#pragma unroll
        for (int j = 0; j < 5; ++j) {
            const int i = tid + 1024 * j, o = i / 36, k = i - o * 36;
            if (dst[j]) {
                const float v = (o < 64 && k == 35) ? s_sdp[o]
                                                    : (s_acc[(0 * 128 + o) * 37 + k] + s_acc[(1 * 128 + o) * 37 + k]) +
                                                          (s_acc[(2 * 128 + o) * 37 + k] + s_acc[(3 * 128 + o) * 37 + k]);
                *dst[j] = old[j] + v;
            }
        }
#pragma unroll
        for (int j = 0; j < 4; ++j) {
            const int i = tid + 1024 * j, o = i >> 6, k = i & 63;
            A.fp3.dW[img + o * 96 + k] = old_o[j] + s_sdp[o] * s_x3[k];
        }
        if (tid < 64) A.dx3[(size_t)b * 64 + tid] = s_g[tid];
        if (bn_dst[0]) {
            *bn_dst[0] = old_bn[0] + s_bnf[tid];
            *bn_dst[1] = old_bn[1] + s_bn3[tid];
        }
    }
    BSTAMP(7)
    return true;
}

template <bool ONE_TRIP>
__device__ __noinline__ void gb_repair(GbArgs A, float* smem, unsigned epoch) {
    for (int pass = 0; pass < 2; ++pass)
        for (int b = 0; b < A.B; ++b)
            if (__hip_atomic_load(&A.ctl[8 + b], __ATOMIC_RELAXED, __HIP_MEMORY_SCOPE_AGENT)) gb_plot<ONE_TRIP>(A, smem, b, epoch, pass == 0, true);
    __syncthreads();
    if (threadIdx.x == 0) {
        for (int b = 0; b < A.B; ++b) __hip_atomic_store(&A.ctl[8 + b], 0u, __ATOMIC_RELAXED, __HIP_MEMORY_SCOPE_AGENT);
        __hip_atomic_store(&A.ctl[2], __hip_atomic_load(&A.ctl[1], __ATOMIC_RELAXED, __HIP_MEMORY_SCOPE_AGENT), __ATOMIC_RELAXED,
                           __HIP_MEMORY_SCOPE_AGENT);
    }
}

template <bool ONE_TRIP>
__global__ __launch_bounds__(1024) void global_level_bwd_kernel(GbArgs A) {
    extern __shared__ __attribute__((aligned(16))) float gb_smem[];
    __shared__ unsigned s_epoch;
    __shared__ int s_last;
    const int tid = threadIdx.x;
    if (tid == 0) s_epoch = __hip_atomic_load(&A.ctl[0], __ATOMIC_RELAXED, __HIP_MEMORY_SCOPE_AGENT) + 1u;
    __syncthreads();
    const unsigned epoch = s_epoch;
    const bool ok = gb_plot<ONE_TRIP>(A, gb_smem, (int)blockIdx.x, epoch, false, false);
    if (!ok && tid == 0) {
        __hip_atomic_store(&A.ctl[8 + blockIdx.x], 1u, __ATOMIC_RELAXED, __HIP_MEMORY_SCOPE_AGENT);
        atomicAdd(&A.ctl[1], 1u);
    }
    __syncthreads();
    if (tid == 0) {
        const unsigned t = atomicAdd(&A.ctl[4], 1u);
        int last = 0;
        if (t == gridDim.x - 1) {
            __hip_atomic_store(&A.ctl[4], 0u, __ATOMIC_RELAXED, __HIP_MEMORY_SCOPE_AGENT);
            last = __hip_atomic_load(&A.ctl[1], __ATOMIC_RELAXED, __HIP_MEMORY_SCOPE_AGENT) !=
                           __hip_atomic_load(&A.ctl[2], __ATOMIC_RELAXED, __HIP_MEMORY_SCOPE_AGENT)
                       ? 2
                       : 1;
        }
        s_last = last;
    }
    __syncthreads();
    if (!s_last) return;
    if (s_last == 2) gb_repair<ONE_TRIP>(A, gb_smem, epoch);
    if (tid == 0) __hip_atomic_store(&A.ctl[0], epoch, __ATOMIC_RELAXED, __HIP_MEMORY_SCOPE_AGENT);
}

}

static bool gl_bwd_covers(int B, int frozen, int bf16) { return B <= GL_MAX_PLOTS && !frozen && !bf16; }
extern "C" int sn2_global_level_backward_route(int B, int M2, int frozen, int bf16) {
    return gl_bwd_covers(B, frozen, bf16) && M2 <= GL_BWD_MAX_ROWS;
}

extern "C" int sn2_global_level_backward(const sn2_fp* sa3, const sn2_fp* fp3, const int* arg3, unsigned long long* xchg,
                                         unsigned* ctl, void* stream) {
    if (!sa3 || !fp3 || !arg3 || !xchg || !ctl) return SN2_EINVAL;
    const int B = sa3->B, M2 = sa3->R_per_plot;
    if (!(B > 0 && M2 > 0 && fp3->B == B && fp3->R_per_plot == M2 && sa3->S_per_plot == M2 && fp3->S_per_plot == 1)) return SN2_EINVAL;
    if (!(sa3->ca == 32 && sa3->cb == 3 && sa3->blk.cin == 35 && sa3->blk.cout == 64 && fp3->ca == 64 && fp3->cb == 32 &&
          fp3->blk.cin == 96 && fp3->blk.cout == 64))
        return SN2_ELIMIT;
    if (!gl_bwd_covers(B, sa3->blk.frozen_stats || fp3->blk.frozen_stats, sa3->blk.mma_bf16 || fp3->blk.mma_bf16) || sa3->act_bf16 ||
        fp3->act_bf16)
        return SN2_ELIMIT;
    if (sa3->knn_idx || sa3->src_a || !fp3->knn_idx || fp3->src_a) return SN2_EINVAL;
    if (!sa3->src || sa3->src_stride != 32 || !sa3->skip || sa3->skip_stride != 4 || !sa3->h || sa3->h_stride != 64) return SN2_EINVAL;
    if (!fp3->src || fp3->src_stride != 64 || fp3->skip != sa3->src || fp3->skip_stride != 32 || !fp3->h || fp3->h_stride != 64)
        return SN2_EINVAL;
    if (!fp3->dy || !fp3->dsrc || fp3->dsrc_stride != 64 || !fp3->dskip || fp3->dskip_stride != 32 || sa3->dsrc != fp3->dskip ||
        sa3->dsrc_stride != 32)
        return SN2_EINVAL;
    for (const sn2_block* k : {&sa3->blk, &fp3->blk})
        if (!k->W || !k->gamma || !k->mean || !k->invstd || !k->dW || !k->db || !k->dgamma || !k->dbeta) return SN2_EINVAL;
    if ((long)B * M2 >= (1L << 31) / 64) return SN2_ELIMIT;
    if (sa3->blk.grad_replicas < B || fp3->blk.grad_replicas < B || sa3->blk.grad_replica_stride != fp3->blk.grad_replica_stride)
        return SN2_ELIMIT;
    GbArgs A;
    A.B = B, A.M2 = M2;
    A.x2 = sa3->src, A.pos2 = sa3->skip, A.x3 = fp3->src, A.arg3 = arg3, A.dy3 = fp3->dy, A.dx2 = fp3->dskip, A.dx3 = fp3->dsrc;
    auto layer = [](const sn2_fp* p) {
        GbLayer l;
        l.W = p->blk.W, l.gamma = p->blk.gamma, l.mean = p->blk.mean, l.invstd = p->blk.invstd, l.h = p->h;
        l.dW = p->blk.dW, l.db = p->blk.db, l.dgamma = p->blk.dgamma, l.dbeta = p->blk.dbeta;
        return l;
    };
    A.sa3 = layer(sa3), A.fp3 = layer(fp3);
    A.img_stride = sa3->blk.grad_replica_stride;
    A.xchg = xchg, A.ctl = ctl;
    A.spin_limit = g_gl_spin_limit;
    const size_t lds = ((size_t)GB_FIXED_FLOATS + (size_t)B * 128) * 4;
    auto kern = M2 <= GL_GROUPS * 64 ? &global_level_bwd_kernel<true> : &global_level_bwd_kernel<false>;
    (void)hipFuncSetAttribute(reinterpret_cast<const void*>(kern), hipFuncAttributeMaxDynamicSharedMemorySize, (int)lds);
    hipLaunchKernelGGL(kern, dim3(B), dim3(1024), lds, (hipStream_t)stream, A);
    SN2_RETURN_LAUNCH();
}
```

### stratanet2_vegetation_coverage_maps_amd/csrc/net.hip

```cpp
#include "common.h"

#include <cstring>
#include <new>

namespace {

constexpr int WIDTHS[7] = {16, 16, 32, 64, 64, 34, 34};
constexpr int WIDTH_SUM = 260;
constexpr int GRAD_IMAGES = SN2_NET_GRAD_IMAGES;

struct NetCtx {
    hipEvent_t fork, b_tables, b_nn, b_done, c_nn, c_done, pack_fork, packed;
};

inline bool fp_src_ws_wanted(const sn2_net_model* m, long R, int cb, bool force) {
    return m->source_side && sn2_fp_source_side(R, cb, force);
}
inline bool fused_eval_head(const sn2_net_model* m, const sn2_net_dims* d, int training) {
    return !training && m->fuse_eval_head && !d->act_bf16 && m->source_side;
}
inline int gl_bf16(const sn2_net_model* m) { return m->sa3.mma_bf16 || m->fp3.mma_bf16; }

struct Carver {
    uintptr_t base;
// ... 454 lines not shown
    fp_desc(&p3, d, a, sa3_in(m, d, g, a), nograd);
    fp_desc(&pf3, d, a, fp3_in(m, d, g, a), nograd);
    if (batch_stats && m->fuse_global_level && io->gl_xchg && io->gl_ctl && sn2_global_level_forward_route(B, gl_bf16(m))) {
        SN2_TRY(sn2_global_level_forward(&p3, &pf3, a->x3, a->arg3, io->gl_xchg, io->gl_ctl, cur));
    } else {
        SN2_TRY(sn2_fp_forward(&p3, mode, cur));
        SN2_TRY(sn2_plot_max_forward(a->h_sa3, p3.blk.a, p3.blk.c, B, M2, 64, a->x3, a->arg3, cur));
        SN2_TRY(sn2_fp_forward(&pf3, mode, cur));
    }
    sn2_fp p2;
    fp_desc(&p2, d, a, fp2_in(m, d, g, a, a->src_ws2), nograd);
    SN2_TRY(sn2_fp_forward(&p2, mode, cur));
    if (join_c) NET_HIP(hipStreamWaitEvent(cur, ctx->c_nn, 0));
    sn2_fp p1;
    sn2_head hd;
    if (fused_eval) {
        if (!a->src_ws1) return SN2_EINVAL;
        sn2_net_act a2 = *a;
        a2.h1 = nullptr;
        fp_desc(&p1, d, &a2, fp1_in(m, d, g, &a2, a->src_ws1), nograd);
        head_desc(&hd, m, d, &a2, 0);
        SN2_TRY(sn2_fp_head_eval(&p1, &hd, cur));
    } else {
        fp_desc(&p1, d, a, fp1_in(m, d, g, a, a->src_ws1), nograd);
        SN2_TRY(sn2_fp_forward(&p1, mode, cur));
        head_desc(&hd, m, d, a, batch_stats);
        if (training && a->bwd_arena && a->bwd_arena_words > 0) hd.zero_fill = a->bwd_arena, hd.zero_fill_words = a->bwd_arena_words;
        SN2_TRY(sn2_head_forward(&hd, cur));
    }
    if (join_b) NET_HIP(hipStreamWaitEvent(cur, ctx->b_done, 0));
    if (join_c) NET_HIP(hipStreamWaitEvent(cur, ctx->c_done, 0));
    return 0;
}

extern "C" int sn2_net_backward(const sn2_net_model* m, const sn2_net_dims* d, const sn2_net_geo* g, const sn2_net_act* a,
                                const sn2_net_bwd* b, void* stream) {
    SN2_TRY(check_dims(m, d));
    SN2_TRY(check_model_ptrs(m));
    if (!a || !b) return SN2_EINVAL;
    SN2_TRY(check_geo(d, g));
    if (!g->inv1 || !g->inv2 || !g->inv3) return SN2_EINVAL;
    if (!a->aux || !a->stats || !a->h1 || !a->h2 || !a->h3 || !a->h_sa3 || !a->x3 || !a->arg3) return SN2_EINVAL;
    if (!b->arena || b->images != GRAD_IMAGES || b->image_stride < m->n_flat || !b->dy1 || !b->du1 || !b->du2 || !b->du3 || !b->bn_ok ||
        !b->dy2 || !b->dy3 || !b->dx1 || !b->dx2 || !b->dx3 || !b->dy_sa3 || b->arena_words <= 0)
        return SN2_EINVAL;
    const int B = d->B, M2 = d->M2;
    if (b->loss && (b->dcov || b->dproba || b->loss->B != d->B || b->loss->N != d->N ||
                    !sn2_head_loss_route(b->loss->B, b->loss->N, b->loss->D)))
        return SN2_EINVAL;
    hipStream_t cur = (hipStream_t)stream;
    if (!b->arena_is_zero) {
        sn2_fill_words(b->arena, 0u, (size_t)b->arena_words, cur);
        NET_HIP(hipGetLastError());
    }
    const GradDst gd{b->arena, b->image_stride, b->frozen_stats ? 1 : 0};
    sn2_head hd;
    head_desc(&hd, m, d, a, b->frozen_stats ? 0 : 1);
    hd.coverages = hd.proba = nullptr;
    hd.dcoverages = b->dcov, hd.dproba = b->dproba, hd.dy = static_cast<float*>(b->dy1);
    hd.loss = b->loss;
    hd.dW1 = b->arena + m->g_lin1_W, hd.db1 = b->arena + m->g_lin1_b, hd.dW2 = b->arena + m->g_lin2_W, hd.db2 = b->arena + m->g_lin2_b;
    hd.grad_replicas = GRAD_IMAGES, hd.grad_replica_stride = b->image_stride;
    SN2_TRY(sn2_head_backward(&hd, cur));
    SN2_TRY(sn2_head_bn_sums(&hd, m->fp1.gamma, m->fp1.beta, aux_row(a, 6, 2), aux_row(a, 6, 3), b->arena + m->fp1.ggamma,
                             b->arena + m->fp1.gbeta, b->bn_ok + 0, cur));
    sn2_fp p1;
    fp_desc(&p1, d, a, fp1_in(m, d, g, a, b->src_ws1), gd);
    p1.dy = static_cast<const float*>(b->dy1), p1.dsrc = b->dy2, p1.dsrc_stride = 36, p1.dskip = nullptr, p1.dskip_stride = 0;
    p1.du_scratch = static_cast<float*>(b->du1), p1.scatter_ws = g->inv1, p1.scatter_ready = 1, p1.bn_sums_done = b->bn_ok + 0;
    p1.row_perm = (g->rank1 && p1.src_ws) ? g->rank1 : nullptr;
    SN2_TRY(sn2_fp_backward(&p1, cur));
    SN2_TRY(sn2_fp_bn_sums(&p1, m->fp2.gamma, m->fp2.beta, aux_row(a, 5, 2), aux_row(a, 5, 3), b->arena + m->fp2.ggamma,
                           b->arena + m->fp2.gbeta, b->bn_ok + 1, cur));
    sn2_fp p2;
    fp_desc(&p2, d, a, fp2_in(m, d, g, a, b->src_ws2), gd);
    p2.dy = b->dy2, p2.dsrc = b->dy3, p2.dsrc_stride = 64, p2.dskip = b->dx1, p2.dskip_stride = 16;
    p2.du_scratch = b->du2, p2.scatter_ws = g->inv2, p2.scatter_ready = 1, p2.bn_sums_done = b->bn_ok + 1;
    SN2_TRY(sn2_fp_backward(&p2, cur));
    sn2_fp pf3, p3;
    fp_desc(&pf3, d, a, fp3_in(m, d, g, a), gd);
    pf3.dy = b->dy3, pf3.dsrc = b->dx3, pf3.dsrc_stride = 64, pf3.dskip = b->dx2, pf3.dskip_stride = 32;
    fp_desc(&p3, d, a, sa3_in(m, d, g, a), gd);
    p3.dsrc = b->dx2, p3.dsrc_stride = 32;
    if (m->fuse_global_level && b->gl_xchg && b->gl_ctl && sn2_global_level_backward_route(B, M2, b->frozen_stats, gl_bf16(m))) {
        SN2_TRY(sn2_global_level_backward(&p3, &pf3, a->arg3, b->gl_xchg, b->gl_ctl, cur));
    } else {
        SN2_TRY(sn2_fp_bn_sums(&p2, m->fp3.gamma, m->fp3.beta, aux_row(a, 4, 2), aux_row(a, 4, 3), b->arena + m->fp3.ggamma,
                               b->arena + m->fp3.gbeta, b->bn_ok + 2, cur));
        pf3.du_scratch = b->du3, pf3.scatter_ws = g->inv3, pf3.scatter_ready = -1, pf3.bn_sums_done = b->bn_ok + 2;
        SN2_TRY(sn2_fp_backward(&pf3, cur));
        SN2_TRY(sn2_global_pool_backward(b->du3, 64, a->arg3, a->h_sa3, aux_row(a, 3, 2), aux_row(a, 3, 3), B, M2, 64, b->dx3,
                                         b->dy_sa3, b->arena + m->sa3.ggamma, b->arena + m->sa3.gbeta, cur));
        p3.dy = b->dy_sa3, p3.bn_sums_done = b->bn_ok + 3;
        SN2_TRY(sn2_fp_backward(&p3, cur));
    }
    sn2_sa sa;
    sa2_desc(&sa, m, d, g, a, gd, b->dx2, b->dx1);
    SN2_TRY(sn2_sa_backward(&sa, cur));
    sa1_desc(&sa, m, d, g, a, gd, b->dx1, b->sa1_ws);
    SN2_TRY(sn2_sa_backward(&sa, cur));
    if (b->defer_grad_reduce) return 0;
    return sn2_grad_reduce(b->arena, m->n_flat, GRAD_IMAGES, b->image_stride, cur);
}
```

### stratanet2_vegetation_coverage_maps_amd/csrc/sa.hip

```cpp
#include "mlp.h"

template <int CF, int NL, int C1, int C2, int PASS>
int sa_mfma_launch_fwd(const sn2_sa* p, int training, hipStream_t st, int* nblocks_out);
template <int CF, int NL, int C1, int C2, int PASS>
int sa_mfma_launch_bwd(const sn2_sa* p, float* ws, hipStream_t st);

namespace {


__global__ __launch_bounds__(256) void sa_bwd_prep_kernel(const float* __restrict__ dout, const float* __restrict__ ext,
                                                          const int* __restrict__ arg, const float* __restrict__ mean,
                                                          const float* __restrict__ invstd, int rows, int C,
                                                          float* __restrict__ dgamma, float* __restrict__ dbeta) {
    const int o = threadIdx.x % C, g = threadIdx.x / C, G = 256 / C;
    float sb = 0.f, sg = 0.f;
    const float mu = mean[o], is = invstd[o];
    const int step = gridDim.x * G;
    for (int r0 = blockIdx.x * G + g; g < G && r0 < rows; r0 += 8 * step) {
        int ar[8];
        float dv[8], ev[8];
#pragma unroll
        for (int u = 0; u < 8; ++u) {
            const int r = r0 + u * step;
            const size_t i = (size_t)(r < rows ? r : r0) * C + o;
            ar[u] = r < rows ? arg[i] : -1;
            dv[u] = dout[i];
            ev[u] = ext[i];
        }
#pragma unroll
        for (int u = 0; u < 8; ++u)
            if (ar[u] >= 0) {
                sb += dv[u];
                sg = fmaf(dv[u], (ev[u] - mu) * is, sg);
            }
    }
    __shared__ float s_red[128];
    for (int i = threadIdx.x; i < 2 * C; i += 256) s_red[i] = 0.f;
    __syncthreads();
    if (g < G) {
        atomicAdd(&s_red[o], sb);
        atomicAdd(&s_red[C + o], sg);
    }
    __syncthreads();
    if (threadIdx.x < 2 * C) {
        const float v = s_red[threadIdx.x];
        if (v != 0.f) atomicAdd(threadIdx.x < C ? &dbeta[threadIdx.x] : &dgamma[threadIdx.x - C], v);
    }
}

__global__ __launch_bounds__(256) void sa_bwd_combine_kernel(const float* __restrict__ ws, const float* __restrict__ dgamma,
                                                             const float* __restrict__ dbeta,
                                                             const unsigned long long* __restrict__ total, int C, int CIN,
                                                             float* __restrict__ dW, float* __restrict__ db) {
    const int n = C * (CIN + 1), i = threadIdx.x;
    if (i >= n) return;
    float part[2][SN2_SA_BWD_WS_REPLICAS];
#pragma unroll
    for (int r = 0; r < SN2_SA_BWD_WS_REPLICAS; ++r) {
        part[0][r] = ws[(size_t)r * 2 * n + i];
        part[1][r] = ws[(size_t)r * 2 * n + n + i];
    }
    const unsigned long long etot = *total;
    const float invE = etot > 0 ? (float)(1.0 / (double)etot) : 0.f;
    const int o = i / (CIN + 1), k = i - o * (CIN + 1);
    const float dg = dgamma[o] * invE, de = dbeta[o] * invE;
    float sx = 0.f, sm = 0.f;
#pragma unroll
    for (int r = 0; r < SN2_SA_BWD_WS_REPLICAS; ++r) sx += part[0][r], sm += part[1][r];
    const float v = -fmaf(dg, sx, de * sm);
    float* dst = k < CIN ? &dW[o * CIN + k] : &db[o];
    *dst += v;
}

int check(const sn2_sa* p) {
    if (!p || p->B <= 0 || p->Nsrc <= 0 || p->M <= 0 || p->cap <= 0) return SN2_EINVAL;
    if (!p->feat || !p->spos || !p->cpos || !p->nbr || !p->cnt || !p->total || !p->ext || !p->arg || !p->out)
        return SN2_EINVAL;
    if (p->feat_stride < p->cf || (p->feat_stride & 3) || p->spos_stride < 4 || (p->spos_stride & 3)) return SN2_EINVAL;
    const bool sa1 = p->cf == 8 && p->nl == 2 && p->blk[0].cin == 11 && p->blk[0].cout == 16 && p->blk[1].cin == 16 &&
                     p->blk[1].cout == 16;
    const bool sa2 = p->cf == 16 && p->nl == 1 && p->blk[0].cin == 19 && p->blk[0].cout == 32;
    const bool sa3 = p->cf == 32 && p->nl == 1 && p->blk[0].cin == 35 && p->blk[0].cout == 64;
    return (sa1 || sa2 || sa3) ? 0 : SN2_ELIMIT;
}

template <int CF, int NL, int C1, int C2>
int forward_t(const sn2_sa* p, int training, hipStream_t st) {
    const sn2_block* last = &p->blk[NL - 1];
    int nb = 0;
    const int batch_stats = training == 1;
    if constexpr (NL == 2) {
        if (batch_stats) SN2_TRY((sa_mfma_launch_fwd<CF, NL, C1, C2, 0>(p, training, st, &nb)));
        SN2_TRY(sn2_bn_finalize(&p->blk[0], nb, p->total, 0, batch_stats, st));
    }
    if (!training) {
        SN2_TRY(sn2_bn_finalize(last, 0, p->total, 0, 0, st));
        return sa_mfma_launch_fwd<CF, NL, C1, C2, 1>(p, 0, st, &nb);
    }
    SN2_TRY((sa_mfma_launch_fwd<CF, NL, C1, C2, 1>(p, training, st, &nb)));
    return sn2_bn_finalize_apply(last, batch_stats ? nb : 0, p->total, 0, batch_stats, p->ext, p->arg, p->out, (long)p->B * p->M, st);
}

template <int CF, int NL, int C1, int C2>
int backward_t(const sn2_sa* p, hipStream_t st) {
    const sn2_block* last = &p->blk[NL - 1];
    const int rows = p->B * p->M, C = last->cout;
    int pb = sn2_cdiv(rows, 256 / C);
    if (pb > 256) pb = 256;
    hipLaunchKernelGGL(sa_bwd_prep_kernel, dim3(pb), dim3(256), 0, st, p->dout, p->ext, p->arg, last->mean, last->invstd,
                       rows, C, last->dgamma, last->dbeta);
    if constexpr (NL == 2) {
        const sn2_block* k0 = &p->blk[0];
        if (!p->dfeat && p->bwd_ws && !k0->mma_bf16) {
            SN2_TRY((sa_mfma_launch_bwd<CF, NL, C1, C2, 2>(p, p->bwd_ws, st)));
            if (k0->frozen_stats || last->frozen_stats) return 0;
            static_assert(C1 * (CF + 4) <= 256, "one thread per element of [dW0 | db0]");
            hipLaunchKernelGGL(sa_bwd_combine_kernel, dim3(1), dim3((C1 * (CF + 4) + 63) / 64 * 64), 0, st, p->bwd_ws, k0->dgamma,
                               k0->dbeta, p->total, C1, CF + 3, k0->dW, k0->db);
            SN2_RETURN_LAUNCH();
        }
        SN2_TRY((sa_mfma_launch_bwd<CF, NL, C1, C2, 2>(p, nullptr, st)));
    }
    SN2_TRY((sa_mfma_launch_bwd<CF, NL, C1, C2, 3>(p, nullptr, st)));
    return 0;
}

}

namespace {
__global__ __launch_bounds__(1024) void sa_order_sort_kernel(const int* __restrict__ cnt, int B, int M, int P2,
                                                             int* __restrict__ order_all, size_t stride) {
    extern __shared__ __attribute__((aligned(16))) unsigned s_key[];
    __shared__ int s_n[3];
    const int bg = blockIdx.x, tid = threadIdx.x, NT = (int)blockDim.x;
    const int hb = bg / B, b = bg - hb * B;
    int* __restrict__ order = order_all + (size_t)hb * stride;
    const int* cb = cnt + (size_t)bg * M;
    if (tid < 3) s_n[tid] = 0;
    __syncthreads();
    int n_here[3] = {0, 0, 0};
    for (int i = tid; i < P2; i += NT) {
        unsigned key = 0xFFFFFFFFu;
        if (i < M) {
            const int c = cb[i];
            key = ((unsigned)(0x3FFFF - c) << 14) | (unsigned)i;
            n_here[0] += c > SN2_SA_SOLO_MIN ? 1 : 0;
            n_here[1] += (c > SN2_SA_QUAD_MIN && c <= SN2_SA_SOLO_MIN) ? 1 : 0;
            n_here[2] += (c > SN2_SA_OCT_MIN && c <= SN2_SA_QUAD_MIN) ? 1 : 0;
        }
        s_key[i] = key;
    }
#pragma unroll
    for (int k = 0; k < 3; ++k)
        if (n_here[k]) atomicAdd(&s_n[k], n_here[k]);
    __syncthreads();
    for (int k = 2; k <= P2; k <<= 1) {
        for (int j = k >> 1; j > 0; j >>= 1) {
            for (int t = tid; t < (P2 >> 1); t += NT) {
                const int lo = ((t & ~(j - 1)) << 1) | (t & (j - 1)), hi = lo | j;
                const unsigned a = s_key[lo], c = s_key[hi];
                const bool up = (lo & k) == 0;
                if ((a > c) == up) {
                    s_key[lo] = c;
                    s_key[hi] = a;
                }
            }
            __syncthreads();
        }
    }
    const int nsolo = s_n[0], r_oct = nsolo + s_n[1], r_hex = r_oct + s_n[2];
    const int items_a = nsolo + ((s_n[1] + 3) >> 2), n_oct_items = (s_n[2] + 7) >> 3, n_hex_items = (M - r_hex + 15) >> 4;
    int* packed = order + (size_t)4 * B * M;
    for (int r = tid; r < M; r += NT) {
        const int id = b * M + (int)(s_key[r] & 0x3FFFu);
        if (r < nsolo) {
            int* dst = order + 4 * ((size_t)r * B + b);
            dst[0] = dst[1] = dst[2] = dst[3] = id | SN2_SA_SOLO_FLAG;
        } else if (r < r_oct) {
            const int rl = r - nsolo;
            order[4 * ((size_t)(nsolo + (rl >> 2)) * B + b) + (rl & 3)] = id;
        } else if (r < r_hex) {
            const int rl = r - r_oct;
            int* dst = packed + 16 * ((size_t)(rl >> 3) * B + b) + 2 * (rl & 7);
            dst[0] = dst[1] = id | SN2_SA_OCT_FLAG;
        } else {
            const int rl = r - r_hex;
            packed[16 * ((size_t)(n_oct_items + (rl >> 4)) * B + b) + (rl & 15)] = id;
        }
    }
    if (tid == 0) {
        int* trailer = packed + (size_t)16 * B * SN2_SA_PACKED_ITEMS(M);
        atomicMax(&trailer[0], items_a);
        atomicMax(&trailer[1], n_oct_items + n_hex_items);
// ... 44 lines not shown
```

### stratanet2_vegetation_coverage_maps_amd/csrc/sa_mfma.hip

```cpp
#include "mlp.h"

namespace {

struct SaFwdArgs {
    int B, Nsrc, M, cap, feat_stride, spos_stride, group;
    const float *feat, *spos, *cpos;
    const int *nbr, *cnt, *order;
    const float *W0, *b0, *a0, *c0, *gamma0;
    const float *W1, *b1, *gamma1;
    float *slots;
    float* ext;
    int* arg;
    const float *al, *cl;
    float* out;
};

__device__ __forceinline__ float row_max(float v) {
    v = fmaxf(v, __int_as_float(SN2_DPP(__float_as_int(v), 0xB1, 0xF)));
    v = fmaxf(v, __int_as_float(SN2_DPP(__float_as_int(v), 0x4E, 0xF)));
    v = fmaxf(v, __int_as_float(SN2_DPP(__float_as_int(v), 0x141, 0xF)));
    v = fmaxf(v, __int_as_float(SN2_DPP(__float_as_int(v), 0x140, 0xF)));
    return v;
}
__device__ __forceinline__ unsigned row_min_u32(unsigned v) {
// ... 310 lines not shown
#pragma unroll
                    for (int io = 0; io < TOL; ++io)
#pragma unroll
                        for (int r = 0; r < 4; ++r) {
                            if constexpr (STATS) {
                                const bool take = best[t][io][r] > best[0][io][r] ||
                                                  (best[t][io][r] == best[0][io][r] && barg[t][io][r] < barg[0][io][r]);
                                best[0][io][r] = take ? best[t][io][r] : best[0][io][r];
                                barg[0][io][r] = take ? barg[t][io][r] : barg[0][io][r];
                            } else {
                                best[0][io][r] = fmaxf(best[0][io][r], best[t][io][r]);
                            }
                        }
            }
            const int W = it.W;
            const bool writer = (c & (W - 1)) == 0;
#pragma unroll
            for (int t = 0; t < 4; ++t) {
                if (it.solo && t > 0) continue;
#pragma unroll
                for (int io = 0; io < TOL; ++io) {
                    float ev[4];
                    int av[4];
#pragma unroll
                    for (int r = 0; r < 4; ++r) {
                        const float m = seg_max(best[t][io][r], W);
                        ev[r] = it.ln[t] > 0 ? sgn[io][r] * m : 0.f;
                        if constexpr (STATS) {
                            const unsigned am = seg_min_u32(best[t][io][r] == m ? (unsigned)barg[t][io][r] : 0xFFFFFFFFu, W);
                            av[r] = it.ln[t] > 0 ? (int)am : -1;
                        } else {
                            av[r] = 0;
                            ev[r] = it.ln[t] > 0 ? fmaf(alv[io][r], ev[r], clv[io][r]) : 0.f;
                        }
                    }
                    if (writer && it.ln[t] >= 0) {
                        const size_t o = (size_t)it.lc[t] * CL + 16 * io + 4 * q;
                        if constexpr (STATS) {
                            *reinterpret_cast<float4*>(a.ext + o) = make_float4(ev[0], ev[1], ev[2], ev[3]);
                            *reinterpret_cast<int4*>(a.arg + o) = make_int4(av[0], av[1], av[2], av[3]);
                        } else {
                            *reinterpret_cast<float4*>(a.out + o) = make_float4(ev[0], ev[1], ev[2], ev[3]);
                        }
                    }
                }
            }
        }
    }

    if (STATS && a.slots) {
        const int wv = threadIdx.x >> 6;
        for (int i = threadIdx.x; i < 4 * 2 * CS; i += 256) (&s_red[0][0])[i] = 0.f;
        __syncthreads();
#pragma unroll
        for (int io = 0; io < TOS; ++io)
#pragma unroll
            for (int r = 0; r < 4; ++r) {
                const float s1 = row_sum(ssum[io][r]), s2 = row_sum(ssq[io][r]);
                if (c == 0) {
                    s_red[wv][16 * io + 4 * q + r] = s1;
                    s_red[wv][CS + 16 * io + 4 * q + r] = s2;
                }
            }
        __syncthreads();
        for (int i = threadIdx.x; i < 2 * CS; i += 256)
            a.slots[(size_t)blockIdx.x * 2 * CS + i] = (s_red[0][i] + s_red[1][i]) + (s_red[2][i] + s_red[3][i]);
    }
}


struct SaBwdArgs {
    int B, Nsrc, M, cap, feat_stride, spos_stride, group, frozen;
    const float *feat, *spos, *cpos;
    const int *nbr, *cnt, *order;
    const unsigned long long* total;
    const float *W0, *b0, *a0, *c0, *gamma0, *mean0, *invstd0, *dgamma0, *dbeta0;
    const float *W1, *b1, *gamma1, *mean1, *invstd1, *dgamma1, *dbeta1;
    const float* dout;
    const int* arg;
    float *dW0, *db0, *dW1, *db1, *dgamma0_out, *dbeta0_out;
    int rep_k, rep_stride;
    float* dfeat;
    float* ws;
};

#ifdef SN2_SA_STAMPS
__device__ unsigned long long g_sa_dbg[4096 * 10];
extern "C" int sn2_debug_sa_stamps(unsigned long long* out) {
    return (int)hipMemcpyFromSymbol(out, HIP_SYMBOL(g_sa_dbg), sizeof(g_sa_dbg));
}
#define SASTAMP(i)                                                                                  \
    if (CF == 8 && PASS == 3 && (threadIdx.x & 63) == 0 && wave < 4096) {                              \
        unsigned long long t_;                                                                      \
        asm volatile("s_memtime %0\n\ts_waitcnt lgkmcnt(0)" : "=s"(t_)::"memory");                   \
        g_sa_dbg[wave * 10 + (i)] = t_;                                                              \
    }
#define SACOUNT(i, v) if (CF == 8 && PASS == 3 && (threadIdx.x & 63) == 0 && wave < 4096) g_sa_dbg[wave * 10 + (i)] = (v);
#else
#define SASTAMP(i)
#define SACOUNT(i, v)
#endif

template <int CF, int NL, int C1, int C2, int PASS, bool BF16>
struct SaBwdLds {
    static constexpr bool LAST2 = NL == 2 && PASS == 2;
    static constexpr int OWN = OuterAcc<(LAST2 ? C2 : C1), (LAST2 ? C1 : CF + 4)>::LDS_FLOATS;
    static constexpr int FLOATS = OWN + ((LAST2 && !BF16) ? 2 * 64 * 16 : 0);
};

template <int CF, int NL, int C1, int C2, int PASS, bool BF16>
__global__ __launch_bounds__(256, (NL == 2 && PASS == 2 && !BF16) ? 2 : 1) void sa_mfma_bwd_kernel(const SaBwdArgs a) {
    constexpr int CIN = CF + 3, KB1 = CF / 4 + 1, TO1 = C1 / 16, TO2 = C2 / 16;
    constexpr bool LAST2 = NL == 2 && PASS == 2;
    constexpr int PO = LAST2 ? C2 : C1;
    constexpr int QK = LAST2 ? C1 : CIN + 1;
    using Acc = OuterAcc<PO, QK>;
    constexpr int PS = Acc::PS, QS = Acc::QS, TP = Acc::TO, TQ = Acc::TK;
    constexpr bool ONE = LAST2 && !BF16;
    static_assert(!ONE || (C1 == 16 && C2 == 16 && CIN + 1 <= 16), "one-pass round: 16-column images");
    constexpr int QK0 = CIN + 1;
    constexpr int WAVE_LDS = SaBwdLds<CF, NL, C1, C2, PASS, BF16>::FLOATS;
    const bool one = ONE && a.ws != nullptr;
    extern __shared__ __attribute__((aligned(16))) float smem[];
    const int lane = threadIdx.x & 63, q = lane >> 4, c = lane & 15;
    const int wib = threadIdx.x >> 6;
    const int wave = __builtin_amdgcn_readfirstlane((int)(blockIdx.x * 4 + wib));
    const int nwaves = gridDim.x * 4;
    const int ncent = a.B * a.M;
    const SaFirst first = sa_first(a.order, a.cnt, a.B, a.M, wave);
    float* lds_p = smem + wib * WAVE_LDS;
    float* lds_q = lds_p + 64 * PS;
    float* lds_x0 = lds_p + Acc::LDS_FLOATS;
    float* lds_q0 = lds_x0 + 64 * 16;
    SASTAMP(0);
    for (int i = lane; i < WAVE_LDS; i += 64) lds_p[i] = 0.f;

    const unsigned long long etot = *a.total;
    const float invE = (etot > 0 && !a.frozen) ? (float)(1.0 / (double)etot) : 0.f;

    float A1[TO1][KB1], bias1[TO1][4];
#pragma unroll
    for (int io = 0; io < TO1; ++io) {
#pragma unroll
        for (int kb = 0; kb < KB1; ++kb) {
            const int k = 4 * kb + q, o = 16 * io + c;
            A1[io][kb] = k < CIN ? a.W0[o * CIN + k] : ((k == CIN && !BF16) ? a.b0[o] : 0.f);
        }
#pragma unroll
        for (int r = 0; r < 4; ++r) bias1[io][r] = BF16 ? a.b0[16 * io + 4 * q + r] : 0.f;
    }
    float A2[NL == 2 ? TO2 : 1][TO1][4], A2T[TO1][NL == 2 ? TO2 : 1][4], bias2[NL == 2 ? TO2 : 1][4], a1v[TO1][4], c1v[TO1][4];
    float cA0[TO1][4], cC0[TO1][4], cD0[TO1][4], mu0[TO1][4], is0[TO1][4];
    float cA1[NL == 2 ? TO2 : 1][4], cC1[NL == 2 ? TO2 : 1][4], cD1[NL == 2 ? TO2 : 1][4];
#pragma unroll
    for (int is = 0; is < TO1; ++is)
#pragma unroll
        for (int r = 0; r < 4; ++r) {
            const int ch = 16 * is + 4 * q + r;
            mu0[is][r] = a.mean0[ch];
            is0[is][r] = a.invstd0[ch];
            a1v[is][r] = NL == 2 ? a.a0[ch] : 0.f;
            c1v[is][r] = NL == 2 ? a.c0[ch] : 0.f;
            if (NL == 1 || PASS == 3) {
                const float g = a.gamma0[ch], dg = a.dgamma0[ch], db = a.dbeta0[ch], m = mu0[is][r], s = is0[is][r];
                cA0[is][r] = g * s;
                cC0[is][r] = g * s * s * dg * invE;
                cD0[is][r] = g * s * (m * s * dg - db) * invE;
            } else {
                cA0[is][r] = cC0[is][r] = cD0[is][r] = 0.f;
            }
        }
    if constexpr (NL == 2) {
#pragma unroll
        for (int io = 0; io < TO2; ++io) {
#pragma unroll
            for (int is = 0; is < TO1; ++is)
#pragma unroll
                for (int kb = 0; kb < 4; ++kb) {
                    A2[io][is][kb] = a.W1[(16 * io + c) * C1 + 16 * is + 4 * q + kb];
                    A2T[is][io][kb] = a.W1[(16 * io + 4 * q + kb) * C1 + 16 * is + c];
                }
#pragma unroll
            for (int r = 0; r < 4; ++r) {
                const int ch = 16 * io + 4 * q + r;
                bias2[io][r] = a.b1[ch];
                const float g = a.gamma1[ch], dg = a.dgamma1[ch], db = a.dbeta1[ch], m = a.mean1[ch], s = a.invstd1[ch];
                cA1[io][r] = g * s;
                cC1[io][r] = g * s * s * dg * invE;
                cD1[io][r] = g * s * (m * s * dg - db) * invE;
            }
        }
    }
    constexpr int TF = CF / 16 > 0 ? CF / 16 : 1;
    float A0T[TF][TO1][4];
    if (PASS == 3 && a.dfeat) {
#pragma unroll
        for (int kt = 0; kt < TF; ++kt)
#pragma unroll
            for (int io = 0; io < TO1; ++io)
#pragma unroll
                for (int kb = 0; kb < 4; ++kb) {
                    const int k = 16 * kt + c;
                    A0T[kt][io][kb] = k < CF ? a.W0[(16 * io + 4 * q + kb) * CIN + k] : 0.f;
                }
    }

    f32x4 acc[TP][TQ];
#pragma unroll
    for (int i = 0; i < TP; ++i)
#pragma unroll
        for (int j = 0; j < TQ; ++j) acc[i][j] = f32x4{0.f, 0.f, 0.f, 0.f};
    f32x4 acc0[3];
#pragma unroll
    for (int i = 0; i < 3; ++i) acc0[i] = f32x4{0.f, 0.f, 0.f, 0.f};
    float dbias[LAST2 ? TO2 : 1][4], dbe0[TO1][4], dga0[TO1][4];
#pragma unroll
    for (int i = 0; i < (LAST2 ? TO2 : 1); ++i)
#pragma unroll
        for (int r = 0; r < 4; ++r) dbias[i][r] = 0.f;
#pragma unroll
    for (int i = 0; i < TO1; ++i)
#pragma unroll
        for (int r = 0; r < 4; ++r) dbe0[i][r] = dga0[i][r] = 0.f;

    constexpr int CL = NL == 2 ? C2 : C1, TOL = CL / 16;
    SASTAMP(1);
    unsigned long long n_items_dbg = 0, n_steps_dbg = 0;
    const int nA = first.nA, nB = first.nB;
    const int G = a.group > 0 && a.group < a.B ? a.group : a.B;
    const int nitems = a.order ? (nA + nB) * G * ((a.B + G - 1) / G) : (ncent + 3) >> 2;
    for (int round = 0;; ++round) {
        const int qi = round * nwaves + ((round & 1) ? nwaves - 1 - wave : wave);
        if (round * nwaves >= nitems) break;
        if (qi >= nitems) continue;
        SaItem it;
        if (!sa_item(it, a.order, a.cnt, a.B, a.M, nA, nB, G, qi, c, round == 0 ? first.rec : nullptr)) continue;
        if (n_items_dbg == 0) { SASTAMP(2); }
        ++n_items_dbg;
        n_steps_dbg += (it.nmax + it.estep - 1) / it.estep;
        const int nmax = it.nmax, estep = it.estep;
        float cpq[4];
        float dov[4][TOL][4];
        int arv[4][TOL][4];
#pragma unroll
        for (int t = 0; t < 4; ++t) {
            cpq[t] = a.cpos[(size_t)it.lc[t] * 4 + (q < 3 ? q : 0)];
#pragma unroll
            for (int io = 0; io < TOL; ++io) {
                const size_t o = (size_t)it.lc[t] * CL + 16 * io + 4 * q;
                const float4 dv = *reinterpret_cast<const float4*>(a.dout + o);
                const int4 av = *reinterpret_cast<const int4*>(a.arg + o);
                dov[t][io][0] = dv.x; dov[t][io][1] = dv.y; dov[t][io][2] = dv.z; dov[t][io][3] = dv.w;
                arv[t][io][0] = av.x; arv[t][io][1] = av.y; arv[t][io][2] = av.z; arv[t][io][3] = av.w;
            }
        }
        int jn[4];
#pragma unroll
        for (int t = 0; t < 4; ++t) {
            const int e = it.le0 + it.eoff * t;
            jn[t] = a.nbr[(size_t)it.lc[t] * a.cap + (e < a.cap ? e : 0)];
        }
#pragma unroll
        for (int t = 0; t < 4; ++t) jn[t] = it.le0 + it.eoff * t < it.ln[t] ? jn[t] : 0;
        for (int e0 = 0; e0 < nmax; e0 += estep) {
            f32x4 D1[TO1][4];
            float bks[4][KB1];
            bool val[4];
            size_t rows[4];
            int jc[4];
// ... 293 lines not shown
        if (i < NW) {
            if constexpr (LAST2) {
                SN2_FLUSH_ADD(&a.dW1[img + i], v);
            } else {
                const int o = i / QK, k = i - o * QK;
                if (k < CIN) SN2_FLUSH_ADD(&a.dW0[img + o * CIN + k], v);
                else SN2_FLUSH_ADD(&a.db0[img + o], v);
            }
        } else if (i < NW + NB) {
            SN2_FLUSH_ADD(&a.db1[img + i - NW], v);
        } else if (i < NW + NB + C1) {
            SN2_FLUSH_ADD(&a.dbeta0_out[i - NW - NB], v);
        } else {
            SN2_FLUSH_ADD(&a.dgamma0_out[i - NW - NB - C1], v);
        }
    }
    SASTAMP(7);
}

}

static int sa_plot_group(int B) {
    static const int g_env = getenv("SN2_SA_GROUP") ? atoi(getenv("SN2_SA_GROUP")) : 0;
    if (g_env > 0) return g_env;
    return B <= 32 ? B : 8;
}

template <int CF, int NL, int C1, int C2, int PASS>
int sa_mfma_launch_fwd(const sn2_sa* p, int training, hipStream_t st, int* nblocks_out) {
    const bool bf16 = p->blk[0].mma_bf16 != 0;
    SaFwdArgs a;
    a.B = p->B; a.Nsrc = p->Nsrc; a.M = p->M; a.cap = p->cap; a.feat_stride = p->feat_stride; a.spos_stride = p->spos_stride;
    a.feat = p->feat; a.spos = p->spos; a.cpos = p->cpos; a.nbr = p->nbr; a.cnt = p->cnt; a.order = p->order;
    a.group = sa_plot_group(p->B);
    const sn2_block& k0 = p->blk[0];
    const sn2_block& k1 = p->blk[NL == 2 ? 1 : 0];
    a.W0 = k0.W; a.b0 = k0.b; a.a0 = k0.a; a.c0 = k0.c; a.gamma0 = k0.gamma;
    a.W1 = k1.W; a.b1 = k1.b; a.gamma1 = k1.gamma;
    a.slots = training == 1 ? (PASS == 0 ? k0.stat_slots : k1.stat_slots) : nullptr;
    a.ext = p->ext; a.arg = p->arg;
    a.al = k1.a; a.cl = k1.c; a.out = p->out;
    int blocks = sn2_cdiv((long)p->B * p->M, 16);
    if (blocks > SN2_STAT_SLOTS) blocks = SN2_STAT_SLOTS;
    static const int occ_env = getenv("SN2_SA_FWD_OCC") ? atoi(getenv("SN2_SA_FWD_OCC")) : 0;
    const int occ = occ_env > 0 ? occ_env : (CF == 8 ? (PASS == 0 ? 4 : 3) : (CF == 16 ? 2 : 1));
    if (blocks > sn2_cu_count() * occ) blocks = sn2_cu_count() * occ;
    if (nblocks_out) *nblocks_out = blocks;
    if constexpr (PASS == 1) {
        if (!training) {
            if (bf16) hipLaunchKernelGGL((sa_mfma_fwd_kernel<CF, NL, C1, C2, PASS, true, false>), dim3(blocks), dim3(256), 0, st, a);
            else hipLaunchKernelGGL((sa_mfma_fwd_kernel<CF, NL, C1, C2, PASS, false, false>), dim3(blocks), dim3(256), 0, st, a);
            SN2_RETURN_LAUNCH();
        }
    }
    if (bf16) hipLaunchKernelGGL((sa_mfma_fwd_kernel<CF, NL, C1, C2, PASS, true>), dim3(blocks), dim3(256), 0, st, a);
    else hipLaunchKernelGGL((sa_mfma_fwd_kernel<CF, NL, C1, C2, PASS, false>), dim3(blocks), dim3(256), 0, st, a);
    SN2_RETURN_LAUNCH();
}

template int sa_mfma_launch_fwd<8, 2, 16, 16, 0>(const sn2_sa*, int, hipStream_t, int*);
template int sa_mfma_launch_fwd<8, 2, 16, 16, 1>(const sn2_sa*, int, hipStream_t, int*);
template int sa_mfma_launch_fwd<16, 1, 32, 32, 1>(const sn2_sa*, int, hipStream_t, int*);
template int sa_mfma_launch_fwd<32, 1, 64, 64, 1>(const sn2_sa*, int, hipStream_t, int*);

template <int CF, int NL, int C1, int C2, int PASS>
int sa_mfma_launch_bwd(const sn2_sa* p, float* ws, hipStream_t st) {
    if (ws && (PASS != 2 || NL != 2 || p->blk[0].mma_bf16)) return SN2_EINVAL;
    SaBwdArgs a;
    a.B = p->B; a.Nsrc = p->Nsrc; a.M = p->M; a.cap = p->cap; a.feat_stride = p->feat_stride; a.spos_stride = p->spos_stride;
    a.feat = p->feat; a.spos = p->spos; a.cpos = p->cpos; a.nbr = p->nbr; a.cnt = p->cnt; a.order = p->order; a.total = p->total;
    a.group = sa_plot_group(p->B);
    const sn2_block& k0 = p->blk[0];
    const sn2_block& k1 = p->blk[NL == 2 ? 1 : 0];
    a.frozen = (k0.frozen_stats || k1.frozen_stats) ? 1 : 0;
    a.W0 = k0.W; a.b0 = k0.b; a.a0 = k0.a; a.c0 = k0.c; a.gamma0 = k0.gamma; a.mean0 = k0.mean; a.invstd0 = k0.invstd;
    a.dgamma0 = k0.dgamma; a.dbeta0 = k0.dbeta;
    a.W1 = k1.W; a.b1 = k1.b; a.gamma1 = k1.gamma; a.mean1 = k1.mean; a.invstd1 = k1.invstd; a.dgamma1 = k1.dgamma;
    a.dbeta1 = k1.dbeta;
    a.dout = p->dout; a.arg = p->arg;
    a.dW0 = k0.dW; a.db0 = k0.db; a.dW1 = k1.dW; a.db1 = k1.db; a.dgamma0_out = k0.dgamma; a.dbeta0_out = k0.dbeta;
    a.rep_k = k0.grad_replicas; a.rep_stride = k0.grad_replica_stride;
    a.dfeat = p->dfeat;
    a.ws = ws;
    int blocks = sn2_cdiv((long)p->B * p->M, 16);
    static const int occ_env = getenv("SN2_SA_BWD_OCC") ? atoi(getenv("SN2_SA_BWD_OCC")) : 0;
    const int occ = occ_env > 0 ? occ_env : (CF == 8 ? 2 : 1);
    if (blocks > sn2_cu_count() * occ) blocks = sn2_cu_count() * occ;
    const size_t lds = (size_t)(p->blk[0].mma_bf16 ? SaBwdLds<CF, NL, C1, C2, PASS, true>::FLOATS
                                                   : SaBwdLds<CF, NL, C1, C2, PASS, false>::FLOATS) * 4 * sizeof(float);
    auto kern = p->blk[0].mma_bf16 ? &sa_mfma_bwd_kernel<CF, NL, C1, C2, PASS, true> : &sa_mfma_bwd_kernel<CF, NL, C1, C2, PASS, false>;
    if (lds > 48 * 1024)
        (void)hipFuncSetAttribute(reinterpret_cast<const void*>(kern), hipFuncAttributeMaxDynamicSharedMemorySize, (int)lds);
    hipLaunchKernelGGL(kern, dim3(blocks), dim3(256), lds, st, a);
    SN2_RETURN_LAUNCH();
}

template int sa_mfma_launch_bwd<8, 2, 16, 16, 2>(const sn2_sa*, float*, hipStream_t);
template int sa_mfma_launch_bwd<8, 2, 16, 16, 3>(const sn2_sa*, float*, hipStream_t);
template int sa_mfma_launch_bwd<16, 1, 32, 32, 3>(const sn2_sa*, float*, hipStream_t);
template int sa_mfma_launch_bwd<32, 1, 64, 64, 3>(const sn2_sa*, float*, hipStream_t);
```

### stratanet2_vegetation_coverage_maps_amd/executor.py

```python
import ctypes
import weakref
from ctypes import byref

import torch

from . import _lib
from . import hip_ops as ops
from ._lib import NetAct, NetBwd, NetDims, NetGeo, NetIO, NetModel, StrataHipError

F32, I32, I64, BF16, U8 = torch.float32, torch.int32, torch.int64, torch.bfloat16, torch.uint8
_FAKE_BASE = 1 << 40
_ITEM = {F32: 4, I32: 4, I64: 8, BF16: 2, U8: 1}


def _geo_shapes(B, N, M1, M2, cap1, cap2):
    return {
        "idx1": (I32, (B, M1)), "pos1_soa": (F32, (B, 3, M1)), "pos1_aos": (F32, (B * M1, 4)), "ws1": (I32, (ops.fps_ws_words(B, N),)),
        "nbr1": (I32, (B * M1, cap1)), "cnt1": (I32, (B * M1,)), "tot1": (I64, (1,)), "ord1": (I32, (ops.sa_order_len(B, M1),)),
        "idx2": (I32, (B, M2)), "pos2_soa": (F32, (B, 3, M2)), "pos2_aos": (F32, (B * M2, 4)), "ws2": (I32, (ops.fps_ws_words(B, M1),)),
        "nbr2": (I32, (B * M2, cap2)), "cnt2": (I32, (B * M2,)), "tot2": (I64, (1,)), "ord2": (I32, (ops.sa_order_len(B, M2),)),
        "knn3_idx": (I32, (B * M2, 3)), "knn3_w": (F32, (B * M2, 3)), "knn2_idx": (I32, (B * M1, 3)), "knn2_w": (F32, (B * M1, 3)),
        "knn1_idx": (I32, (B * N, 3)), "knn1_w": (F32, (B * N, 3)),
        "inv3": (F32, (ops.interp_ws_words(B, M2, 1),)), "inv2": (F32, (ops.interp_ws_words(B, M1, M2),)),
        "inv1": (F32, (ops.interp_ws_words(B, N, M1),)),
# ... 139 lines not shown
    pos3 = getattr(g, "pos3", None)
    if pos3 is None:
        pos3 = g.pos3 = _pos3(g.idx1.device, g.B)
    cg.pos3 = pos3.data_ptr()
    g.cgeo = cg
    return cg


def _check_handle(g, plan, what):
    d = plan.dims
    ok = (g.B, g.N, g.M1, g.M2) == (d.B, d.N, d.M1, d.M2)
    if ok:
        gp = getattr(g, "plan", None)
        if gp is not None:
            ok = gp is plan or (gp.dims.cap1, gp.dims.cap2, gp.geo_bytes) == (d.cap1, d.cap2, plan.geo_bytes) or \
                (gp.dims.cap1, gp.dims.cap2) == (d.cap1, d.cap2) and gp.dims.p2_diam_pix >= d.p2_diam_pix
        else:
            ok = g.nbr1.shape[1] == d.cap1 and g.nbr2.shape[1] == d.cap2
    if not ok:
        raise ValueError(f"{what} do not match this batch")


class NetSaved:

    def __init__(self, plan, geo, arena, cact, training):
        self.plan, self.geo, self.arena, self.cact, self.training = plan, geo, arena, cact, training
        self.B, self.N, self.M1, self.M2 = plan.B, plan.N, plan.M1, plan.M2

    def __getattr__(self, name):
        d = self.__dict__
        plan = d.get("plan")
        if plan is None:
            raise AttributeError(name)
        spec = plan.act_offsets[1 if d["training"] else 0].get(name)
        if spec is not None:
            v = d[name] = _view(d["arena"], *spec)
            return v
        return getattr(d["geo"], name)


_BLOCKS = ("sa1_module.conv.local_nn.0", "sa1_module.conv.local_nn.1", "sa2_module.conv.local_nn.0", "sa3_module.nn.0",
           "fp3_module.nn.0", "fp2_module.nn.0", "fp1_module.nn.0")


class ModelStruct:

    def __init__(self, model, params, max_neighbors):
        offs, n_flat = ops.flat_layout(params)
        off_of = {id(p): o for p, o in zip(params, offs)}
        self.param_offsets, self.n_flat = offs, n_flat
        self.param_shapes = [tuple(p.shape) for p in params]
        self.param_numels = [p.numel() for p in params]
        m = NetModel()
        mods = dict(model.named_modules())
        layers = [m.sa1[0], m.sa1[1], m.sa2, m.sa3, m.fp3, m.fp2, m.fp1]
        self.tensors = []
        for L, name in zip(layers, _BLOCKS):
            blk = mods[name]
            lin, bn = blk[0], blk[2]
            prefix = name.rsplit(".", 1)[0]
            for t in (lin.weight, lin.bias, bn.weight, bn.bias, bn.running_mean, bn.running_var):
                ops._chk(t, F32, None, name)
            L.cin, L.cout = lin.in_features, lin.out_features
            L.W, L.b, L.gamma, L.beta = lin.weight.data_ptr(), lin.bias.data_ptr(), bn.weight.data_ptr(), bn.bias.data_ptr()
            L.running_mean, L.running_var = bn.running_mean.data_ptr(), bn.running_var.data_ptr()
            nbt = bn.num_batches_tracked
            if nbt is not None:
                ops._chk(nbt, I64, None, "num_batches_tracked")
            L.num_batches_tracked = None if nbt is None else nbt.data_ptr()
            L.gW, L.gb, L.ggamma, L.gbeta = (off_of[id(t)] for t in (lin.weight, lin.bias, bn.weight, bn.bias))
            L.mma_bf16 = int(model.mma_dtype == "bf16" and prefix in model.BF16_BLOCKS)
            self.tensors += [lin.weight, lin.bias, bn.weight, bn.bias, bn.running_mean, bn.running_var] + ([nbt] if nbt is not None else [])
        for t, shape in ((model.lin1.weight, (16, 34)), (model.lin1.bias, (16,)), (model.lin2.weight, (5, 16)), (model.lin2.bias, (5,))):
            ops._chk(t, F32, shape, "head parameter")
        m.lin1_W, m.lin1_b, m.lin2_W, m.lin2_b = (t.data_ptr() for t in (model.lin1.weight, model.lin1.bias, model.lin2.weight, model.lin2.bias))
        m.g_lin1_W, m.g_lin1_b, m.g_lin2_W, m.g_lin2_b = (off_of[id(t)] for t in (model.lin1.weight, model.lin1.bias, model.lin2.weight,
                                                                                model.lin2.bias))
        self.tensors += [model.lin1.weight, model.lin1.bias, model.lin2.weight, model.lin2.bias]
        m.n_flat = n_flat
        m.r1_sq, m.r2_sq = ops.r2_threshold(model.sa1_module.r), ops.r2_threshold(model.sa2_module.r)
        m.max_neighbors = int(max_neighbors)
        m.drop_p = float(model.drop)
        m.fuse_global_level, m.fuse_eval_head, m.source_side = int(bool(model.fuse_global_level)), int(bool(model.fuse_eval_head)), int(bool(ops.SOURCE_SIDE))
        m.fps_waves_shared, m.fps_waves_many = int(model.fps_waves_shared), int(model.fps_waves_many)
        self.c = m
        self.settings = settings_of(model, max_neighbors)
        self.key = tuple(t.data_ptr() for t in self.tensors)
        self.plans = {}
        dev = model.lin1.weight.device
        if any(t.device != dev for t in self.tensors):
            raise StrataHipError("PointNet2: parameters and buffers must live on one HIP device")

    def current(self, model, max_neighbors):
        return self.settings == settings_of(model, max_neighbors) and self.key == tuple(t.data_ptr() for t in self.tensors)

    def plan(self, model, B, N):
        k = (B, N)
        p = self.plans.get(k)
        if p is None:
            if len(self.plans) > 32:
                self.plans.clear()
            p = self.plans[k] = Plan(model, self.c, B, N, self.c.max_neighbors)
        return p


def settings_of(model, max_neighbors):
    return (model.mma_dtype, float(model.drop), bool(model.fuse_global_level), bool(model.fuse_eval_head), bool(ops.SOURCE_SIDE),
            int(model.fps_waves_shared), int(model.fps_waves_many), float(model.sa1_module.r), float(model.sa2_module.r),
            float(model.sa1_module.ratio), float(model.sa2_module.ratio), int(max_neighbors), model.p2_diam_pix,
            bool(model.fp1_morton_rows))


class NetCtx:

    def __init__(self):
        h = ctypes.c_void_p()
        _lib.check(_lib.load().sn2_net_ctx_create(byref(h)), "sn2_net_ctx_create")
        self.handle = h.value
        self._fin = weakref.finalize(self, _destroy_ctx, self.handle)


def _destroy_ctx(handle):
    try:
        _lib.load().sn2_net_ctx_destroy(handle)
    except Exception:
        pass


def _io(model, dev, training, flags, cloud=None, fps_start=None, fork=False, n_live=None, geo=None):
    io = NetIO()
    if n_live is not None:
        io.fps_live, io.fps_live1 = n_live.data_ptr(), geo.fps_live1.data_ptr()
    io.cloud = None if cloud is None else cloud.data_ptr()
    io.fps_start = None if fps_start is None else fps_start.data_ptr()
    io.fps_status = ops.fps_status_word(dev).data_ptr()
    io.training = int(training) if training in (0, 1, 2) else int(bool(training))
    if fork:
        io.stream_b = ops.shared_stream(dev, "fork_b").cuda_stream
        io.stream_c = ops.shared_stream(dev, "fork_c").cuda_stream
        io.stream_pack = ops.shared_stream(dev, "pack").cuda_stream
        io.ctx = model._net_ctx().handle
    io.flags = flags
    return io


def geometry(model, ms, xyz, fps_start, out=None, fork=None, shared=False, defer_join=False, inverted=True, cloud=None, n_live=None):
    dev = xyz.device
    B, _, N = xyz.shape
    ops._chk(xyz, F32, (B, 3, N), "xyz")
    ops._chk(fps_start, I32, (2, B), "fps_start")
    if n_live is not None:
        ops._chk(n_live, I32, (B,), "n_live")
    plan = ms.plan(model, B, N)
    g = out if out is not None else ArenaGeometry(plan, dev, model)
    _check_handle(g, plan, "geometry buffers")
    cg = geo_struct(g)
    g.xyz = xyz
    cg.xyz = xyz.data_ptr()
    fork = model.geometry_fork if fork is None else fork
    flags = (_lib.NET_FORK if fork else 0) | (_lib.NET_SHARED if shared else 0) | (_lib.NET_INVERTED if inverted else 0)
    if fork and defer_join:
        flags |= _lib.NET_DEFER_JOIN
    if cloud is not None:
        ops._chk(cloud, F32, (B, 10, N), "cloud")
        flags |= _lib.NET_INPUT_ONLY
    io = _io(model, dev, model.training, flags, cloud=cloud, fps_start=fps_start, fork=fork, n_live=n_live, geo=g)
    _lib.check(_lib.load().sn2_net_geometry(byref(ms.c), byref(plan.dims), byref(cg), byref(io), ops._stream()), "sn2_net_geometry")
    g.has_inverted = bool(inverted)
    g.has_rows0 = cloud is not None
    if cloud is not None and plan.dims.p2_diam_pix > 0 and getattr(g, "p2_pix", None) is not None:
        g.p2_diam_pix = int(plan.dims.p2_diam_pix)
    g._join = "ctx" if (fork and defer_join) else None
    return g


def forward(model, ms, xyz, cloud, fps_start, training, geo=None, drop_keep=None, need_grad=True, n_live=None):
    dev = xyz.device
    B, _, N = xyz.shape
    ops._chk(xyz, F32, (B, 3, N), "xyz")
    ops._chk(cloud, F32, (B, 10, N), "cloud")
    plan = ms.plan(model, B, N)
    lib = _lib.load()
    fork = False
    frozen = (not training) and bool(need_grad)
    keep = bool(training) or frozen
    mode = 1 if training else (_lib.BN_FROZEN_KEEP if frozen else 0)
    if geo is None:
        ops._chk(fps_start, I32, (2, B), "fps_start")
        geo = ArenaGeometry(plan, dev, model)
        fork = bool(model.geometry_fork)
# ... 92 lines not shown
```

### stratanet2_vegetation_coverage_maps_amd/hip_ops.py

```python
import ctypes
import math
from typing import Optional

import numpy as np
import torch

from . import _lib
from ._lib import FP, SA, Block, Head, LossGrad, StrataHipError, check

I32, F32, F64, I64, BF16 = torch.int32, torch.float32, torch.float64, torch.int64, torch.bfloat16


_timing = None


class timing:

    def __init__(self, names=None):
        self.names = None if names is None else set(names)
        self.events = []

    def __enter__(self):
        global _timing
        self._prev, _timing = _timing, self
# ... 609 lines not shown
        raise ValueError("cell_items: expected 1..P centre ids")
    return start, items, int(GX), int(GY), float(gx0), float(gy0), float(inv)


def parcel_count(cloud: torch.Tensor, centers: torch.Tensor, grid, radius: float, L: int, rows: int):
    _, T = cloud.shape
    _chk(cloud, F32, (10, T), "cloud")
    P = centers.shape[0]
    _chk(centers, F32, (P, 2), "centers")
    start, items, GX, GY, gx0, gy0, inv = _chk_center_grid(grid, P)
    dev = cloud.device
    nw = parcel_count_ws_words(P, rows)
    ws = torch.empty(nw + 4, dtype=I32, device=dev)
    prefix = torch.empty(P * rows + 1, dtype=I32, device=dev)
    total = torch.empty(1, dtype=I64, device=dev)
    _call("sn2_parcel_count", _ptr(cloud), T, int(L), int(rows), _ptr(centers), P, _ptr(start), _ptr(items), GX, GY, gx0, gy0,
          inv, float(radius), _ptr(ws), nw, _ptr(prefix), _ptr(total), _stream())
    return prefix, total


def parcel_fill(cloud: torch.Tensor, centers: torch.Tensor, grid, radius: float, L: int, rows: int, prefix: torch.Tensor,
                plot_base: torch.Tensor, sum_n: int):
    _, T = cloud.shape
    _chk(cloud, F32, (10, T), "cloud")
    P = centers.shape[0]
    _chk(centers, F32, (P, 2), "centers")
    start, items, GX, GY, gx0, gy0, inv = _chk_center_grid(grid, P)
    _chk(prefix, I32, (P * rows + 1,), "prefix")
    _chk(plot_base, I32, (P,), "plot_base")
    dev = cloud.device
    raw = torch.empty(10, sum_n, dtype=F32, device=dev)
    pidx = torch.empty(sum_n, dtype=I32, device=dev)
    _call("sn2_parcel_fill", _ptr(cloud), T, int(L), int(rows), _ptr(centers), P, _ptr(start), _ptr(items), GX, GY, gx0, gy0,
          inv, float(radius), _ptr(prefix), _ptr(plot_base), int(sum_n), _ptr(raw), _ptr(pidx), _stream())
    return raw, pidx


def parcel_znorm(cloud: torch.Tensor, bbox, radius: float, disc_radius: float, offsets: torch.Tensor, centers: torch.Tensor,
                 point_index: torch.Tensor, raw: torch.Tensor):
    _, T = cloud.shape
    _chk(cloud, F32, (10, T), "cloud")
    P = centers.shape[0]
    _chk(centers, F32, (P, 2), "centers")
    _chk(offsets, I32, (P + 1,), "offsets")
    sum_n = point_index.shape[0]
    _chk(point_index, I32, (sum_n,), "point_index")
    _chk(raw, F32, (10, sum_n), "raw")
    nw = parcel_znorm_ws_words(T, radius, *bbox)
    if nw == 0:
        raise ValueError("parcel_znorm: the parcel's extent needs more than 2^26 cells of the z-norm radius")
    ws = torch.empty(nw + 4, dtype=I32, device=cloud.device)
    _call("sn2_parcel_znorm", _ptr(cloud), T, *[float(v) for v in bbox], float(radius), float(disc_radius), _ptr(offsets),
          _ptr(centers), P, _ptr(point_index), sum_n, _ptr(ws), nw, _ptr(raw), _stream())
    return raw


def sa_order_len(B: int, M: int) -> int:
    return _host("sn2_sa_order_words", int(B), int(M))


def sa_order(cnt: torch.Tensor, B: int, M: int, out: Optional[torch.Tensor] = None) -> torch.Tensor:
    _chk(cnt, I32, (B * M,), "cnt")
    n = sa_order_len(B, M)
    if out is None:
        out = torch.empty(n, dtype=I32, device=cnt.device)
    else:
        _chk(out, I32, (n,), "out order")
    _call("sn2_sa_order", _ptr(cnt), B, M, _ptr(out), _stream())
    return out


def sa_order_group(cnt: torch.Tensor, G: int, B: int, M: int, out_all: torch.Tensor, stride: int):
    _chk(cnt, I32, (G * B * M,), "cnt")
    if stride < sa_order_len(B, M):
        raise ValueError("sa_order_group: stride smaller than a table")
    _chk(out_all, I32, (G * stride,), "out order tables")
    _call("sn2_sa_order_group", _ptr(cnt), G, B, M, _ptr(out_all), stride, _stream(), key="sn2_sa_order")


SA_BWD_WS_WORDS = _lib.SN2_SA_BWD_WS_WORDS


def sa_desc(blocks, feat, cf, spos, cpos_aos, nbr, cnt, total, B, Nsrc, M, ext, arg, out, dout=None, dfeat=None,
            with_grads=False, order=None, bwd_ws=None) -> SA:
    cap = nbr.shape[1]
    cl = blocks[-1].cout
    feat_stride = _chk_rows(feat, F32, B * Nsrc, cf, "feat")
    spos_stride = _chk_rows(spos, F32, B * Nsrc, 4, "spos")
    _chk(cpos_aos, F32, (B * M, 4), "cpos_aos")
    _chk(nbr, I32, (B * M, cap), "nbr")
    _chk(cnt, I32, (B * M,), "cnt")
    _chk(total, I64, (1,), "total")
    _chk(ext, F32, (B * M, cl), "ext")
    _chk(arg, I32, (B * M, cl), "arg")
    _chk(out, F32, (B * M, cl), "out")
    d = SA()
    d.B, d.Nsrc, d.M, d.cap, d.cf, d.nl = B, Nsrc, M, cap, cf, len(blocks)
    d.feat, d.feat_stride, d.spos, d.spos_stride = _ptr(feat), feat_stride, _ptr(spos), spos_stride
    d.cpos, d.nbr, d.cnt, d.total = _ptr(cpos_aos), _ptr(nbr), _ptr(cnt), _ptr(total)
    if order is not None:
        _chk(order, I32, (sa_order_len(B, M),), "order")
    d.order = _ptr(order)
    for i, bb in enumerate(blocks):
        bb.fill(d.blk[i], with_grads)
    d.ext, d.arg, d.out = _ptr(ext), _ptr(arg), _ptr(out)
    if dout is not None:
        _chk(dout, F32, (B * M, cl), "dout")
    if dfeat is not None:
        _chk(dfeat, F32, (B * Nsrc, cf), "dfeat")
    if bwd_ws is not None:
        _chk(bwd_ws, F32, (SA_BWD_WS_WORDS,), "bwd_ws")
    d.dout, d.dfeat, d.bwd_ws = _ptr(dout), _ptr(dfeat), _ptr(bwd_ws)
    return d


def sa_forward(d: SA, training: bool):
    _call("sn2_sa_forward", d, int(training), _stream(), tag=f"cf={d.cf}")


def sa_backward(d: SA):
    _call("sn2_sa_backward", d, _stream(), tag=f"cf={d.cf}")


def interp_ws_words(B: int, R_per_plot: int, S_per_plot: int) -> int:
    return _host("sn2_interp_ws_words", int(B), int(R_per_plot), int(S_per_plot))


def interp_chunks(R_per_plot: int, S_per_plot: int) -> int:
    return _host("sn2_interp_chunks", int(R_per_plot), int(S_per_plot))


def fp_src_ws_words(B: int, R_per_plot: int, S_per_plot: int, cout: int) -> int:
    return _host("sn2_fp_src_ws_words", int(B), int(R_per_plot), int(S_per_plot), int(cout))


def fp_rows_small(R: int) -> bool:
    return bool(_host("sn2_fp_rows_small", int(R)))


def fp_source_side(R: int, cb: int, force: bool = False) -> bool:
    return bool(_host("sn2_fp_source_side", int(R), int(cb), int(bool(force))))


def interp_index(knn, B: int, R_per_plot: int, S_per_plot: int, out: Optional[torch.Tensor] = None,
                 src_pos: Optional[torch.Tensor] = None, row_perm: Optional[torch.Tensor] = None) -> torch.Tensor:
    if src_pos is not None:
        _chk(src_pos, F32, (B * S_per_plot, 4), "src_pos")
    if row_perm is not None:
        _chk(row_perm, I32, (B * R_per_plot,), "row_perm")
    R = B * R_per_plot
    _chk(knn[0], I32, (R, 3), "knn_idx")
    _chk(knn[1], F32, (R, 3), "knn_w")
    n = interp_ws_words(B, R_per_plot, S_per_plot)
    if out is None:
        out = torch.empty(n, dtype=F32, device=knn[0].device)
    else:
        _chk(out, F32, (n,), "out index")
    _call("sn2_interp_index_perm", _ptr(knn[0]), _ptr(knn[1]), _ptr(src_pos), _ptr(row_perm), B, R_per_plot, S_per_plot, _ptr(out),
          _stream(), key="sn2_interp_index")
    return out


def interp_index_group(knn, G: int, B: int, R_per_plot: int, S_per_plot: int, out_all: torch.Tensor, stride: int,
                       src_pos: Optional[torch.Tensor] = None, row_perm: Optional[torch.Tensor] = None):
    R = G * B * R_per_plot
    _chk(knn[0], I32, (R, 3), "knn_idx")
    _chk(knn[1], F32, (R, 3), "knn_w")
    if src_pos is not None:
        _chk(src_pos, F32, (G * B * S_per_plot, 4), "src_pos")
    if row_perm is not None:
        _chk(row_perm, I32, (R,), "row_perm")
    if stride % 4 or stride < interp_ws_words(B, R_per_plot, S_per_plot):
        raise ValueError("interp_index_group: stride must be a multiple of 4 words and hold one index")
    _chk(out_all, F32, (G * stride,), "out indices")
    _call("sn2_interp_index_group", _ptr(knn[0]), _ptr(knn[1]), _ptr(src_pos), _ptr(row_perm), G, B, R_per_plot, S_per_plot, _ptr(out_all),
          stride, _stream(), key="sn2_interp_index")


SOURCE_SIDE = True


def fp_desc(block: BlockBuffers, B, R_per_plot, S_per_plot, ca, cb, src, h, src_affine=None, knn=None, skip=None,
            dy=None, dsrc=None, dskip=None, du_scratch=None, with_grads=False, interp_index=None,
            bn_sums_done=None, row_perm=None, force_src_ws=False, gather=True) -> FP:
    R = B * R_per_plot
    hs = (block.cout + 3) // 4 * 4
    AT = BF16 if (h is not None and h.dtype == BF16) else F32
    n_src_rows = R if knn is None else B * S_per_plot
    src_stride = _chk_rows(src, F32, n_src_rows, ca, "src")
    if src.shape[1] < (ca + 3) // 4 * 4 and src_stride < (ca + 3) // 4 * 4:
        raise ValueError("fp: src rows must be padded to a multiple of 4 floats")
    if h is not None or not force_src_ws:
        _chk(h, AT, (R, hs), "h")
    d = FP()
    d.B, d.R_per_plot, d.S_per_plot, d.ca, d.cb = B, R_per_plot, S_per_plot, ca, cb
# ... 53 lines not shown
            d.scatter_ws = _ptr(d._scatter_ws)
            if not gather:
                d.scatter_ready = -1
    d.dy, d.dsrc, d.dskip, d.du_scratch = _ptr(dy), _ptr(dsrc), _ptr(dskip), _ptr(du_scratch)
    return d


def fp_bn_sums(d: FP, gamma, beta, mean, invstd, dgamma, dbeta, ok):
    for t, n in ((gamma, "gamma"), (beta, "beta"), (mean, "mean"), (invstd, "invstd"), (dgamma, "dgamma"), (dbeta, "dbeta")):
        _chk(t, F32, (d.ca,), n)
    _chk(ok, I32, (1,), "ok")
    _call("sn2_fp_bn_sums", d, _ptr(gamma), _ptr(beta), _ptr(mean), _ptr(invstd), _ptr(dgamma), _ptr(dbeta), _ptr(ok), _stream())


def fp_forward(d: FP, training: bool):
    _call("sn2_fp_forward", d, int(training), _stream(), tag=f"{d.ca}+{d.cb}->{d.blk.cout}")


def fp_backward(d: FP):
    _call("sn2_fp_backward", d, _stream(), tag=f"{d.ca}+{d.cb}->{d.blk.cout}")


def plot_max_forward(h, a, c, B, R_per_plot, C):
    hs = (C + 3) // 4 * 4
    _chk(h, F32, (B * R_per_plot, hs), "h")
    _chk(a, F32, (C,), "a")
    _chk(c, F32, (C,), "c")
    out = torch.empty(B, C, dtype=F32, device=h.device)
    arg = torch.empty(B, C, dtype=I32, device=h.device)
    _call("sn2_plot_max_forward", _ptr(h), _ptr(a), _ptr(c), B, R_per_plot, C, _ptr(out), _ptr(arg), _stream())
    return out, arg


GL_MAX_PLOTS = _lib.SN2_GLOBAL_MAX_PLOTS
_GLOBAL_WS = {}
_GLOBAL_WS_ALL = []


class _GlobalWs(list):
    __slots__ = ("__weakref__",)


def global_level_ws(dev, B: int = GL_MAX_PLOTS, owner=None):
    dev = torch.device(dev)
    if B > GL_MAX_PLOTS:
        raise ValueError(f"global_level_forward takes at most {GL_MAX_PLOTS} plots")
    key = dev.index if dev.index is not None else torch.cuda.current_device()
    store = _GLOBAL_WS if owner is None else owner.__dict__.setdefault("_gl_ws", {})
    ws = store.get(key)
    if ws is None:
        if torch.cuda.is_current_stream_capturing():
            raise StrataHipError("global_level_forward: its exchange area must exist before a stream capture starts -- run one "
                                 "eager training forward first (TrainPipeline.capture does) or call hip_ops.global_level_ws(dev, owner=model)")
        ws = _GlobalWs([torch.zeros(_host("sn2_global_xchg_words", GL_MAX_PLOTS), dtype=I64, device=dev),
                        torch.zeros(_lib.SN2_GLOBAL_CTL_WORDS, dtype=I32, device=dev), 0,
                        torch.zeros(_lib.SN2_GLOBAL_BWD_XCHG_WORDS, dtype=I64, device=dev),
                        torch.zeros(_lib.SN2_GLOBAL_BWD_CTL_WORDS, dtype=I32, device=dev)])
        store[key] = ws
        import weakref
        _GLOBAL_WS_ALL[:] = [r for r in _GLOBAL_WS_ALL if r() is not None]
        _GLOBAL_WS_ALL.append(weakref.ref(ws))
    return ws


def global_level_forward_fused(B: int, *blocks) -> bool:
    return bool(_host("sn2_global_level_forward_route", int(B), int(any(b.mma_bf16 for b in blocks))))


def global_level_forward(d_sa3: FP, d_fp3: FP, x3: torch.Tensor, arg3: torch.Tensor, owner=None):
    B = d_sa3.B
    _chk(x3, F32, (B, 64), "x3")
    _chk(arg3, I32, (B, 64), "arg3")
    ws = global_level_ws(x3.device, B, owner=owner)
    _call("sn2_global_level_forward", d_sa3, d_fp3, _ptr(x3), _ptr(arg3), _ptr(ws[0]), _ptr(ws[1]), _stream())


GL_BWD_MAX_ROWS = _lib.SN2_GLOBAL_BWD_MAX_ROWS


def global_level_backward_fused(B: int, M2: int, frozen: bool, *blocks) -> bool:
    return bool(_host("sn2_global_level_backward_route", int(B), int(M2), int(bool(frozen)), int(any(b.mma_bf16 for b in blocks))))


def global_level_backward(d_sa3: FP, d_fp3: FP, arg3: torch.Tensor, owner=None):
    B = d_sa3.B
    _chk(arg3, I32, (B, 64), "arg3")
    ws = global_level_ws(arg3.device, B, owner=owner)
    _call("sn2_global_level_backward", d_sa3, d_fp3, _ptr(arg3), _ptr(ws[3]), _ptr(ws[4]), _stream())


def global_level_gave_up(dev, warn: bool = True) -> int:
    dev = torch.device(dev)
    key = dev.index if dev.index is not None else torch.cuda.current_device()
    total = 0
    for r in list(_GLOBAL_WS_ALL):
        ws = r()
        if ws is None or ws[1].device.index != key:
            continue
        n = int(ws[1][1].item()) + int(ws[4][1].item())
        total += n
        if n > ws[2]:
            seen, ws[2] = ws[2], n
            if warn:
                import warnings
                warnings.warn(f"global_level_forward / backward: {n - seen} exchange wait(s) gave up on {dev}; those launches were finished "
                              "by their last workgroup alone (results unaffected, the passes took longer); set "
                              "PointNet2.fuse_global_level = False where other kernels or processes share the device",
                              StrataHipWarning, stacklevel=2)
    return total


def plot_max_backward(dout, arg, B, R_per_plot, C, dy):
    hs = (C + 3) // 4 * 4
    _chk(dout, F32, (B, C), "dout")
    _chk(arg, I32, (B, C), "arg")
    _chk(dy, F32, (B * R_per_plot, hs), "dy")
    _call("sn2_plot_max_backward", _ptr(dout), _ptr(arg), B, R_per_plot, C, _ptr(dy), _stream())


def global_pool_backward(du, arg, h, mean, invstd, B, R_per_plot, dx, dy, dgamma, dbeta):
    _chk(du, F32, (B * R_per_plot, 64), "du")
    _chk(arg, I32, (B, 64), "arg")
    _chk(h, F32, (B * R_per_plot, 64), "h")
    for t, n in ((mean, "mean"), (invstd, "invstd"), (dgamma, "dgamma"), (dbeta, "dbeta")):
        _chk(t, F32, (64,), n)
    _chk(dx, F32, (B, 64), "dx")
    _chk(dy, F32, (B * R_per_plot, 64), "dy")
    _call("sn2_global_pool_backward", _ptr(du), 64, _ptr(arg), _ptr(h), _ptr(mean), _ptr(invstd), B, R_per_plot, 64, _ptr(dx), _ptr(dy),
          _ptr(dgamma), _ptr(dbeta), _stream())


def dropout_mask_words(keep: torch.Tensor) -> torch.Tensor:
    if keep.dim() != 2 or keep.shape[1] != 16:
        raise ValueError("dropout mask must be (rows, 16)")
    pow2 = (2 ** torch.arange(16, device=keep.device, dtype=torch.int32))
    return ((keep != 0).to(torch.int32) * pow2).sum(1, dtype=torch.int32).contiguous()


def head_loss_route(B: int, N: int, diam_pix: int) -> bool:
    return bool(_host("sn2_head_loss_route", int(B), int(N), int(diam_pix)))


def loss_grad_desc(pred, gt, proba, pdf, grad_total, arg, nocc, pix, B: int, N: int, diam_pix: int, m: float, e: float) -> LossGrad:
    R, D = B * N, int(diam_pix)
    _chk(pred, F32, (B, 4), "pred")
    _chk(gt, F64, (B, 4), "gt")
    _chk(proba, F32, (R, 4), "proba")
    if pdf is not None:
        _chk(pdf, F64, (R, 3), "pdf")
    _chk(grad_total, F64, None, "grad_total")
    _chk(arg, I32, (B * D * D * 3,), "arg")
    _chk(nocc, I32, (B,), "nocc")
    _chk(pix, I32, (R,), "pix")
    if grad_total.numel() != 1:
        raise ValueError("loss_grad_desc: grad_total is ONE fp64 scalar on the device")
    g = LossGrad()
    g.pred, g.gt, g.proba, g.pdf, g.grad_total = _ptr(pred), _ptr(gt), _ptr(proba), _ptr(pdf), _ptr(grad_total)
    g.arg, g.nocc, g.pix = _ptr(arg), _ptr(nocc), _ptr(pix)
    g.B, g.N, g.D, g.m, g.e = int(B), int(N), D, float(m), float(e)
    g.tensors = (pred, gt, proba, pdf, grad_total, arg, nocc, pix)
    return g


def head_desc(f, fa, fc, lin1, lin2, coverages=None, proba=None, dcov=None, dproba=None, dy=None, grads=None,
              grad_images=(1, 0), drop_mask=None, drop_p: float = 0.0, rows: Optional[int] = None, loss: Optional[LossGrad] = None) -> Head:
    if f is None:
        if rows is None or coverages is None:
            raise ValueError("head_desc: without f the row count and the outputs must be given")
        R, AT = int(rows), F32
    else:
        R = f.shape[0]
# ... 595 lines not shown
```

### stratanet2_vegetation_coverage_maps_amd/point_net2.py

```python
import os
from collections import OrderedDict

import torch
import torch.nn as nn
from torch.nn import BatchNorm1d as BN
from torch.nn import Linear as Lin
from torch.nn import ReLU
from torch.nn import Sequential as Seq

from . import executor as X
from . import hip_ops as ops
from ._lib import BN_FROZEN_KEEP, MAX_NEIGHBORS as _MAXN, STAT_SLOTS, StrataHipError

MAX_NEIGHBORS = _MAXN

F32, I32, I64, F64 = torch.float32, torch.int32, torch.int64, torch.float64


def MLP(channels):
    return Seq(*[Seq(Lin(channels[i - 1], channels[i]), ReLU(), BN(channels[i])) for i in range(1, len(channels))])


class PointConv(nn.Module):

# ... 59 lines not shown
    def forward(ctx, model, xyz, cloud, fps_start, geo, drop_keep, *params):
        training = model.training
        need_grad = bool(getattr(model, "_grad_mode_at_call", True)) and any(ctx.needs_input_grad[6:])
        n_live = model.__dict__.pop("_n_live_at_call", None)
        cov, proba, saved = model._forward_impl(xyz, cloud, fps_start, training, geo, drop_keep, need_grad=need_grad,
                                                **({} if n_live is None else {"n_live": n_live}))
        ctx.model = model
        if not isinstance(saved, X.NetSaved):
            saved.training = training
        ctx.saved = saved if need_grad else None
        ctx.n_params = len(params)
        return cov, proba

    @staticmethod
    def backward(ctx, dcov, dproba):
        if ctx.saved is None:
            raise RuntimeError("PointNet2: backward through a forward that recorded no graph")
        pending = ctx.__dict__.pop("loss_grad", None)
        loss = None
        if pending is not None:
            if pending.is_placeholder(dcov) and pending.is_placeholder(dproba):
                loss, dcov, dproba = pending.desc(), None, None
            else:
                gc, gp = pending.materialize()
                dcov = gc if (dcov is None or pending.is_placeholder(dcov)) else dcov + gc
                dproba = gp if (dproba is None or pending.is_placeholder(dproba)) else dproba + gp
        grads = ctx.model._backward_impl(ctx.saved, dcov, dproba) if loss is None else ctx.model._backward_impl(ctx.saved, None, None, loss=loss)
        ctx.saved = None
        return (None, None, None, None, None, None) + tuple(grads)


class PointNet2(nn.Module):
    def __init__(self, args):
        super().__init__()
        self._init_fields(args)
        ndim = 3
        mlp1 = [self.n_input_feats + ndim, 16, 16]
        mlp2 = [mlp1[-1] + ndim, 32]
        mlp3 = [mlp2[-1] + ndim, 64]
        self.sa1_module = SAModule(args.ratio1, args.r1, MLP(mlp1))
        self.sa2_module = SAModule(args.ratio2, args.r2, MLP(mlp2))
        self.sa3_module = GlobalSAModule(MLP(mlp3))
        mlp3_fp = [mlp3[-1] + mlp2[-1], 64]
        mlp2_fp = [mlp3_fp[-1] + mlp1[-1], 34]
        mlp1_fp = [mlp2_fp[-1] + self.n_input_feats, 34]
        self.fp3_module = FPModule(1, MLP(mlp3_fp))
        self.fp2_module = FPModule(3, MLP(mlp2_fp))
        self.fp1_module = FPModule(3, MLP(mlp1_fp))
        self.lin1 = nn.Linear(mlp1_fp[-1], 16)
        self.lin2 = nn.Linear(16, self.n_class + 1)
        self.lin2.bias = nn.Parameter(torch.tensor([0.733, 0.266, 0.235, 0.358, 0.500]))
        self.softmax = nn.Softmax(dim=1)
        self.sigmoid = nn.Sigmoid()
        if self.cuda_device is not None:
            self.cuda(self.cuda_device)

    def _init_fields(self, args):
        self.cuda_device = args.cuda
        self.subsample_size = args.subsample_size
        self.n_class = args.n_class
        self.drop = args.drop
        self.n_input_feats = args.n_input_feats - 2
        self.set_patience_attributes(args)
        self.log_embeddings = args.log_embeddings
        self.last_G_tensor = None
        self._last_flat_grad = None
        self._last_cloud_dev = None
        self.set_mma_dtype(getattr(args, "mma_dtype", "fp32"))
        if self.n_class != 4 or self.n_input_feats != 8:
            raise ValueError("the HIP kernels cover the reference architecture: n_class=4, 10 input features")

    BF16_BLOCKS = ("sa1_module.conv.local_nn", "sa2_module.conv.local_nn", "sa3_module.nn", "fp3_module.nn", "fp2_module.nn")
    mma_dtype = "fp32"
    fps_waves_shared = int(os.environ.get("SN2_FPS_WAVES_SHARED", "8"))
    fps_waves_many = int(os.environ.get("SN2_FPS_WAVES_MANY", "4"))
    geometry_fork = True
    executor = os.environ.get("SN2_EXECUTOR", "1") == "1"
    defer_grad_reduce = False
    _grad_images_pending = None
    geometry_pair_takes_group_cloud = True
    fuse_eval_head = os.environ.get("SN2_FUSE_EVAL_HEAD", "1") == "1"
    fuse_global_level = os.environ.get("SN2_FUSE_GLOBAL_LEVEL", "1") == "1"
    fuse_loss_backward = os.environ.get("SN2_FUSE_LOSS_BACKWARD", "1") == "1"
    p2_diam_pix = None

    def set_mma_dtype(self, dtype: str):
        if dtype not in ("fp32", "bf16"):
            raise ValueError("mma_dtype must be 'fp32' or 'bf16'")
        self.mma_dtype = dtype
        return self

    def forward(self, cloud_data):
        cloud, xyz = cloud_data["cloud"], cloud_data["xyz"]
        dev = self.lin1.weight.device
        if dev.type != "cuda":
            raise StrataHipError("PointNet2.forward needs a HIP device (args.cuda): the product path has no CPU "
                                 "fallback; the CPU restatement lives in oracle/ and is test infrastructure")
        if cloud.dim() != 3 or cloud.shape[1] != self.n_input_feats + 2 or xyz.shape != (cloud.shape[0], 3, cloud.shape[2]):
            raise ValueError(f"expected cloud (B,{self.n_input_feats + 2},N) and xyz (B,3,N), got "
                             f"{tuple(cloud.shape)} and {tuple(xyz.shape)}")
        with torch.cuda.device(dev):
            geo = cloud_data.get("geometry", None) if isinstance(cloud_data, dict) else None
            if geo is None and not cloud.is_cuda and not xyz.is_cuda and self.host_upload_overlap:
                return self._forward_from_host(cloud_data, cloud, dev)
            cloud_d = cloud.to(device=dev, dtype=F32, non_blocking=True).contiguous()
            if geo is not None:
                if getattr(geo, "ready", None) is not None:
                    cs = torch.cuda.current_stream()
                    cs.wait_event(geo.ready)
                    for v in geo.__dict__.values():
                        for t in (v if isinstance(v, tuple) else (v,)):
                            if isinstance(t, torch.Tensor):
                                t.record_stream(cs)
                xyz_d, fs = geo.xyz, None
            else:
                xyz_d, fs = self._stage_positions(cloud_data, dev)
                self._n_live_at_call = self._stage_live(cloud_data, dev, xyz_d.shape[0])
            self._last_cloud_dev = (cloud, cloud_d)
            params = self._params()
            self._grad_mode_at_call = torch.is_grad_enabled()
            cov, proba = _PointNet2Fn.apply(self, xyz_d, cloud_d, fs, geo, self._dropout_keep(cloud_data, cloud_d), *params)
        return cov, proba

    host_upload_overlap = os.environ.get("SN2_HOST_UPLOAD_OVERLAP", "1") == "1"

    def _forward_from_host(self, cloud_data, cloud, dev):
        ring = ops.pinned_ring(dev)
        cur = torch.cuda.current_stream(dev)
        cloud_d = torch.empty(cloud.shape, dtype=F32, device=dev)
        start = torch.cuda.Event()
        start.record(cur)
        xyz_d, fs = self._stage_positions(cloud_data, dev, ring=ring)
        g = self._geometry(xyz_d, fs, defer_join=True, inverted=self.training or torch.is_grad_enabled(),
                           **self._live_kw(self._stage_live(cloud_data, dev, xyz_d.shape[0])))
        up = ops.shared_stream(dev, "upload")
        up.wait_event(start)
        ring.upload(cloud, stream=up, dtype=F32, out=cloud_d, consumer=cur)
        self._last_cloud_dev = (cloud, cloud_d)
        from .project_to_2d import remember_upload
        remember_upload(cloud, cloud_d)
        params = self._params()
        self._grad_mode_at_call = torch.is_grad_enabled()
        return _PointNet2Fn.apply(self, xyz_d, cloud_d, None, g, self._dropout_keep(cloud_data, cloud_d), *params)

    def _params(self):
        c = self.__dict__.get("_leafs")
        if c is not None:
            mods = self._modules
            ok = all(mods.get(k) is v for k, v in c[0]) and all(m._parameters.get(n) is p for m, n, p in c[1]) and \
                all(m._buffers.get(n) is b for m, n, b in c[2])
            if ok:
                return self.__dict__["_param_list"]
        self.invalidate_caches()
        ps = list(self.parameters())
        leaf_p, leaf_b = [], []
        for mod in self.modules():
            leaf_p += [(mod, n, p) for n, p in mod._parameters.items() if p is not None]
            leaf_b += [(mod, n, b) for n, b in mod._buffers.items() if b is not None]
        self.__dict__["_param_list"] = ps
        self.__dict__["_leafs"] = (tuple(self._modules.items()), leaf_p, leaf_b)
        return ps

    def invalidate_caches(self):
        for k in ("_param_list", "_leafs", "_net_ms"):
            self.__dict__.pop(k, None)

# ... 377 lines not shown
            raise ValueError("prefetched geometry does not match this batch")
        join = getattr(geo, "_join", None)
        geo._join = None
        if join == "ctx":
            raise StrataHipError("a geometry pass launched by the executor with a deferred join must be consumed by the executor")
        if keep and not getattr(geo, "has_inverted", True):
            if join is not None:
                cur_stream.wait_stream(join[0])
                cur_stream.wait_stream(join[1])
                join = None
            for l in range(1, L + 1):
                ops.count_sum(_at(geo, "cnt", l), _at(geo, "tot", l))
            for j in range(G, 0, -1):
                self._inverted_table(geo, Ms, j)
            geo.has_inverted = True
        s = _Saved()
        s.__dict__.update({k: v for k, v in geo.__dict__.items()
                           if k not in ("ready", "stream", "totals", "nn_ws", "fps_start", "_join", "has_rows0")
                           and not k.startswith(("ws", "fps_live"))})
        s.xyz = xyz
        seqs = self._block_seqs()
        width = sum(blk[0].out_features for _, seq in seqs for blk in seq)
        aux = torch.empty(4 * width, dtype=F32, device=dev)
        stats = torch.empty(STAT_SLOTS * 2 * width, dtype=F32, device=dev)
        cur = [0, 0]
        blocks = [_blocks_of(seq, aux, stats, cur, self.mma_dtype == "bf16" and prefix in self.BF16_BLOCKS) for prefix, seq in seqs]
        s.b_sa = dict(enumerate(blocks[:L], 1))
        s.b_glob = blocks[L][0]
        s.b_fp = dict(zip(range(G, 0, -1), (b[0] for b in blocks[G:])))
        s.blocks = [bb for b in blocks for bb in b]
        s.aux, s.stats = aux, stats
        for bb in s.blocks:
            bb.frozen = frozen
        e = lambda *shape, dt=F32: torch.empty(*shape, dtype=dt, device=dev)

        if packed is not None:
            cur_stream.wait_event(packed)
            s.rows0 = rows0
        elif rows0 is not None:
            s.rows0 = rows0
        else:
            s.rows0 = ops.pack_rows(cloud, xyz)
        for l in range(1, L + 1):
            R, C = B * Ms[l], s.b_sa[l][-1].cout
            _put(s, "ext", l, e(R, C))
            _put(s, "arg", l, e(R, C, dt=I32))
            _put(s, "x", l, e(R, C))
            ops.sa_forward(self._sa_desc(s, l), mode)
            if l == 1 and join is not None:
                cur_stream.wait_stream(join[0])
        R, C = B * Ms[L], s.b_glob.cout
        _put(s, "h_sa", G, e(R, _pad4(C)))
        _put(s, "h", G, e(R, _pad4(s.b_fp[G].cout)))
        if training and self.fuse_global_level and ops.global_level_forward_fused(B, s.b_glob, s.b_fp[G]):
            _put(s, "x", G, e(B, C))
            _put(s, "arg", G, e(B, C, dt=I32))
            ops.global_level_forward(self._global_sa_desc(s), self._fp_desc(s, G), _at(s, "x", G), _at(s, "arg", G), owner=self)
        else:
            ops.fp_forward(self._global_sa_desc(s), mode)
            x, arg = ops.plot_max_forward(_at(s, "h_sa", G), s.b_glob.a, s.b_glob.c, B, Ms[L], C)
            _put(s, "x", G, x)
            _put(s, "arg", G, arg)
            ops.fp_forward(self._fp_desc(s, G), mode)
        if self.log_embeddings:
            self.last_G_tensor = _at(s, "x", G)
        for j in range(L, 1, -1):
            _put(s, "h", j, e(B * Ms[j - 1], _pad4(s.b_fp[j].cout)))
            ops.fp_forward(self._fp_desc(s, j), mode)
        if join is not None:
            cur_stream.wait_stream(join[1])
        cov, proba = e(B * N, 4), e(B * N, 4)
        s.drop_keep = drop_keep
        b1 = s.b_fp[1]
        if not keep and self.fuse_eval_head and self._act_dtype(B * N) == F32 and ops.SOURCE_SIDE:
            s.h1 = None
            ops.fp_head_eval(self._fp_desc(s, 1, force_src_ws=True),
                             ops.head_desc(None, b1.a, b1.c, self.lin1, self.lin2, cov, proba, rows=B * N))
            return cov, proba, s
        s.h1 = torch.empty(B * N, _pad4(b1.cout), dtype=self._act_dtype(B * N), device=dev)
        ops.fp_forward(self._fp_desc(s, 1), mode)
        ops.head_forward(ops.head_desc(s.h1, b1.a, b1.c, self.lin1, self.lin2, cov, proba, drop_mask=drop_keep, drop_p=self.drop))
        return cov, proba, s

    def _sa_desc(self, s, l, dout=None, dfeat=None, g=False, bwd_ws=None):
        blocks = s.b_sa[l]
        cf = blocks[0].cin - 3
        if l == 1:
            feat, spos, S = s.rows0[:, 0:cf], s.rows0[:, cf:cf + 4], s.N
        else:
            feat, spos, S = _at(s, "x", l - 1), _at(s, "pos", l - 1, "_aos"), _at(s, "M", l - 1)
        return ops.sa_desc(blocks, feat, cf, spos, _at(s, "pos", l, "_aos"), _at(s, "nbr", l), _at(s, "cnt", l), _at(s, "tot", l), s.B, S,
                           _at(s, "M", l), _at(s, "ext", l), _at(s, "arg", l), _at(s, "x", l), dout=dout, dfeat=dfeat, with_grads=g,
                           order=getattr(s, f"ord{l}", None), bwd_ws=bwd_ws)

    def _global_sa_desc(self, s, **kw):
        L = len(s.b_sa)
        M = _at(s, "M", L)
        return ops.fp_desc(s.b_glob, s.B, M, M, s.b_glob.cin - 3, 3, _at(s, "x", L), _at(s, "h_sa", L + 1), skip=_at(s, "pos", L, "_aos"), **kw)

    def _fp_desc(self, s, j, **kw):
        L, blk = len(s.b_sa), s.b_fp[j]
        if j == L + 1:
            src, S, ca, affine = _at(s, "x", j), 1, s.b_glob.cout, None
        else:
            up = s.b_fp[j + 1]
            src, S, ca, affine = _at(s, "h", j + 1), _at(s, "M", j), up.cout, (up.a, up.c)
        if j == 1:
            R, skip = s.N, s.rows0[:, 0:blk.cin - ca]
            kw["row_perm"] = getattr(s, "rank1", None)
        else:
            R, skip = _at(s, "M", j - 1), _at(s, "x", j - 1)
        return ops.fp_desc(blk, s.B, R, S, ca, blk.cin - ca, src, _at(s, "h", j), src_affine=affine, knn=_at(s, "knn", j), skip=skip, **kw)

    def _backward_impl(self, s, dcov, dproba, loss=None):
        if isinstance(s, X.NetSaved):
            return X.backward(self, s, dcov, dproba, loss=loss)
        dev = s.xyz.device
        B, N, L = s.B, s.N, len(s.b_sa)
        G = L + 1
        Ms = [N] + [_at(s, "M", l) for l in range(1, G)]
        params = self._params()
        shapes = OrderedDict((f"dy{j}", (B * Ms[j - 1], _pad4(s.b_fp[j].cout))) for j in range(2, G + 1))
        shapes.update((f"dx{l}", (B * Ms[l], s.b_sa[l][-1].cout)) for l in range(1, G))
        shapes[f"dx{G}"] = (B, s.b_glob.cout)
        shapes[f"dy_sa{G}"] = (B * Ms[L], _pad4(s.b_glob.cout))
        sizes = OrderedDict((k, r * c) for k, (r, c) in shapes.items())
        sizes["sa1_ws"] = ops.SA_BWD_WS_WORDS
        flat, buf, views, images, arena = self._grad_arena(params, sizes, dev)
        dy = {j: buf[f"dy{j}"].view(shapes[f"dy{j}"]) for j in range(2, G + 1)}
        dx = {l: buf[f"dx{l}"].view(shapes[f"dx{l}"]) for l in range(1, G + 1)}
        for bb in s.blocks:
            bb.grads = (views[id(bb.lin.weight)], views[id(bb.lin.bias)], views[id(bb.bn.weight)], views[id(bb.bn.bias)])
            bb.grad_images = images
        dcov = None if dcov is None else dcov.contiguous()
        dproba = None if dproba is None else dproba.contiguous()
        e = lambda *shape, dt=F32: torch.empty(*shape, dtype=dt, device=dev)
        bn_ok = e(L + 2, dt=I32)

        def bn_sums(fn, d, blk, k):
            fn(d, blk.bn.weight.detach(), blk.bn.bias.detach(), blk.aux[2], blk.aux[3], views[id(blk.bn.weight)], views[id(blk.bn.bias)],
               bn_ok[k:k + 1])

        b1 = s.b_fp[1]
        dy[1] = e(B * N, _pad4(b1.cout), dt=s.h1.dtype)
        hg = (views[id(self.lin1.weight)], views[id(self.lin1.bias)], views[id(self.lin2.weight)], views[id(self.lin2.bias)])
        hd = ops.head_desc(s.h1, b1.a, b1.c, self.lin1, self.lin2, dcov=dcov, dproba=dproba, dy=dy[1], grads=hg,
                           grad_images=images, drop_mask=getattr(s, "drop_keep", None), drop_p=self.drop, loss=loss)
        ops.head_backward(hd)
        bn_sums(ops.head_bn_sums, hd, b1, 0)
        for j in range(1, G):
            blk, ca = s.b_fp[j], s.b_fp[j + 1].cout
            du = e(B * Ms[j - 1], max(ca, _pad4(blk.cout)), dt=dy[j].dtype)
            d = self._fp_desc(s, j, dy=dy[j], dsrc=dy[j + 1], du_scratch=du, with_grads=True, interp_index=_at(s, "inv", j),
                              bn_sums_done=bn_ok[j - 1:j], **({"dskip": dx[j - 1]} if j > 1 else {}))
            ops.fp_backward(d)
            if j < L:
                bn_sums(ops.fp_bn_sums, d, s.b_fp[j + 1], j)
        top, gb = s.b_fp[G], s.b_glob
        if self.fuse_global_level and ops.global_level_backward_fused(B, Ms[L], getattr(top, "frozen", False), gb, top):
            ops.global_level_backward(self._global_sa_desc(s, dsrc=dx[L], with_grads=True),
                                      self._fp_desc(s, G, dy=dy[G], dsrc=dx[G], dskip=dx[L], with_grads=True), _at(s, "arg", G), owner=self)
        else:
            bn_sums(ops.fp_bn_sums, d, top, L)
            du = e(B * Ms[L], max(gb.cout, _pad4(top.cout)))
            ops.fp_backward(self._fp_desc(s, G, dy=dy[G], dsrc=dx[G], dskip=dx[L], du_scratch=du, with_grads=True,
                                          interp_index=_at(s, "inv", G), bn_sums_done=bn_ok[L:L + 1], gather=False))
            dy_sa = buf[f"dy_sa{G}"].view(shapes[f"dy_sa{G}"])
            ops.global_pool_backward(du, _at(s, "arg", G), _at(s, "h_sa", G), gb.aux[2], gb.aux[3], B, Ms[L], dx[G], dy_sa,
                                     views[id(gb.bn.weight)], views[id(gb.bn.bias)])
            ops.fp_backward(self._global_sa_desc(s, dy=dy_sa, dsrc=dx[L], with_grads=True, bn_sums_done=bn_ok[L + 1:L + 2]))
        for l in range(L, 1, -1):
            ops.sa_backward(self._sa_desc(s, l, dout=dx[l], dfeat=dx[l - 1], g=True))
        ops.sa_backward(self._sa_desc(s, 1, dout=dx[1], g=True, bwd_ws=buf["sa1_ws"]))
        if getattr(self, "defer_grad_reduce", False):
            self._grad_images_pending = (arena,) + tuple(images)
        else:
            ops.grad_reduce(arena, flat.numel(), images)
            self._grad_images_pending = None
        s.flat_grad = flat
        self._last_flat_grad = flat
        return [views[id(p)] for p in params]

    @staticmethod
    def _grad_arena(params, sizes, dev):
        poffs, n_flat = ops.flat_layout(params)
        offs, tot = {}, 0
        for k, n in sizes.items():
            offs[k] = tot
            tot += (n + 3) // 4 * 4
        arena, flat, images, extra = ops.grad_images_alloc(n_flat, dev, tot)
        buf = {k: extra[offs[k]:offs[k] + n] for k, n in sizes.items()}
        views = {id(p): flat[o:o + p.numel()].view(p.shape) for p, o in zip(params, poffs)}
        return flat, buf, views, images, arena

    @staticmethod
    def get_long_form(data):
        B, f, N = data.shape
        return data.permute(1, 0, 2).reshape(f, B * N).transpose(1, 0)

    def get_batch_format(self, data):
        n = self.subsample_size
        return data.view(-1, n, data.shape[1]).transpose(1, 2)

    def set_patience_attributes(self, args):
        self.stopped_early = False
        self.best_metric_value = 10 ** 6
        self.best_metric_epoch = 1
        self.patience_in_epochs = args.patience_in_epochs

    def stop_early(self, val_metric, epoch, args):
        if val_metric < self.best_metric_value:
            self.best_metric_value, self.best_metric_epoch = val_metric, epoch
            self.save_state(args)
            return False
        if epoch < args.epoch_to_start_early_stop:
            return False
        if epoch >= self.best_metric_epoch + self.patience_in_epochs:
            self.stopped_early = True
            return True
        return False

    @staticmethod
    def _checkpoint_path(args):
        tag = f"fold_n={args.current_fold_id}" if args.current_fold_id > 0 else "full"
        return os.path.join(args.stats_path, f"PCC_model_{tag}.pt")

    def save_state(self, args):
        torch.save({"best_metric_epoch": self.best_metric_epoch, "state_dict": self.state_dict(),
                    "best_metric_value": self.best_metric_value}, self._checkpoint_path(args))

    def load_state(self, save_path):
        checkpoint = torch.load(save_path, map_location=None if self.cuda_device is not None else torch.device("cpu"))
        self.load_state_dict(checkpoint["state_dict"])
        self.best_metric_epoch = checkpoint["best_metric_epoch"]
        self.best_metric_value = checkpoint["best_metric_value"]
        return self

    def load_best_state(self, args):
        return self.load_state(self._checkpoint_path(args))
```

Measured before the change: 24240 plots/s.

## Fuse SA2 BatchNorm backward sums into the global-level backward kernel

The fused global-level backward kernel now also accumulates the dbeta/dgamma partial sums for the last SA2 BatchNorm layer while it writes dx2, using the saved pre-activation and argmax from SA2. When this route is taken, the separate sa_bwd_prep kernel launch is skipped. The SA MFMA backward kernel folds the per-replica gradient images in registers and broadcasts them with lane shuffles instead of reading the reduced values. This saves one kernel launch and one pass over dx2/ext2, at the cost of extra registers, LDS and loads inside the already heavy global-level kernel, plus atomic flushes into replica images.

```diff
diff --git a/include/strata_hip.h b/include/strata_hip.h
--- a/include/strata_hip.h
+++ b/include/strata_hip.h
@@ -141,6 +141,7 @@
     const float *dout;
     float *dfeat;
     float *bwd_ws;
+    int bn_sums_done;
 } sn2_sa;
 #define SN2_SA_BWD_WS_REPLICAS 32
 #define SN2_SA_BWD_WS_WORDS (SN2_SA_BWD_WS_REPLICAS * 2 * 16 * 12)
@@ -211,6 +212,8 @@
 #define SN2_GLOBAL_BWD_CTL_WORDS 64
 int sn2_global_level_backward(const sn2_fp *sa3, const sn2_fp *fp3, const int *arg3, unsigned long long *xchg, unsigned *ctl,
                               void *stream);
+int sn2_global_level_backward_below(const sn2_fp *sa3, const sn2_fp *fp3, const int *arg3, unsigned long long *xchg, unsigned *ctl,
+                                    const sn2_sa *below, void *stream);
 int sn2_debug_global_spin_limit(unsigned sweeps);
 
 #define SN2_HEAD_LOSS_MAX_PLOTS 128
@@ -364,6 +367,7 @@
     float drop_p;
     int fuse_global_level;
     int fuse_eval_head;
+    int fuse_sa_bn_sums;
     int source_side;
     int fps_waves_shared, fps_waves_many;
 } sn2_net_model;
@@ -473,6 +477,7 @@
 int sn2_fp_source_side(long R, int cb, int force);
 int sn2_global_level_forward_route(int B, int bf16);
 int sn2_global_level_backward_route(int B, int M2, int frozen, int bf16);
+int sn2_sa_bn_sums_route(int B, int M2, int frozen, int bf16);
 int sn2_head_loss_route(int B, int N, int D);
 
 #ifdef __cplusplus
diff --git a/stratanet2_vegetation_coverage_maps_amd/_lib.py b/stratanet2_vegetation_coverage_maps_amd/_lib.py
--- a/stratanet2_vegetation_coverage_maps_amd/_lib.py
+++ b/stratanet2_vegetation_coverage_maps_amd/_lib.py
@@ -43,7 +43,7 @@
                 ("cpos", c_void_p), ("nbr", c_void_p), ("cnt", c_void_p), ("total", c_void_p), ("order", c_void_p),
                 ("blk", Block * 2),
                 ("ext", c_void_p), ("arg", c_void_p), ("out", c_void_p), ("dout", c_void_p), ("dfeat", c_void_p),
-                ("bwd_ws", c_void_p)]
+                ("bwd_ws", c_void_p), ("bn_sums_done", c_int)]
 
 
 class FP(Structure):
@@ -81,7 +81,7 @@
                 ("lin1_W", c_void_p), ("lin1_b", c_void_p), ("lin2_W", c_void_p), ("lin2_b", c_void_p),
                 ("g_lin1_W", c_int), ("g_lin1_b", c_int), ("g_lin2_W", c_int), ("g_lin2_b", c_int), ("n_flat", c_int),
                 ("r1_sq", c_float), ("r2_sq", c_float), ("max_neighbors", c_int), ("drop_p", c_float),
-                ("fuse_global_level", c_int), ("fuse_eval_head", c_int), ("source_side", c_int),
+                ("fuse_global_level", c_int), ("fuse_eval_head", c_int), ("fuse_sa_bn_sums", c_int), ("source_side", c_int),
                 ("fps_waves_shared", c_int), ("fps_waves_many", c_int)]
 
 
@@ -178,6 +178,7 @@
                                  c_void_p, c_void_p, c_void_p],
     "sn2_global_level_forward": [POINTER(FP), POINTER(FP), c_void_p, c_void_p, c_void_p, c_void_p, c_void_p],
     "sn2_global_level_backward": [POINTER(FP), POINTER(FP), c_void_p, c_void_p, c_void_p, c_void_p],
+    "sn2_global_level_backward_below": [POINTER(FP), POINTER(FP), c_void_p, c_void_p, c_void_p, POINTER(SA), c_void_p],
     "sn2_debug_global_spin_limit": [ctypes.c_uint],
     "sn2_head_forward": [POINTER(Head), c_void_p],
     "sn2_fp_head_eval": [POINTER(FP), POINTER(Head), c_void_p],
@@ -239,6 +240,7 @@
     "sn2_fp_source_side": [c_long, c_int, c_int],
     "sn2_global_level_forward_route": [c_int, c_int],
     "sn2_global_level_backward_route": [c_int, c_int, c_int, c_int],
+    "sn2_sa_bn_sums_route": [c_int, c_int, c_int, c_int],
     "sn2_head_loss_route": [c_int, c_int, c_int],
 }
 
diff --git a/stratanet2_vegetation_coverage_maps_amd/csrc/common.h b/stratanet2_vegetation_coverage_maps_amd/csrc/common.h
--- a/stratanet2_vegetation_coverage_maps_amd/csrc/common.h
+++ b/stratanet2_vegetation_coverage_maps_amd/csrc/common.h
@@ -27,6 +27,31 @@
 #ifdef __HIPCC__
 __device__ __forceinline__ int sn2_grad_image(int replicas, int stride) {
     return replicas > 1 ? (int)(blockIdx.x % (unsigned)replicas) * stride : 0;
+}
+template <int R>
+__device__ __forceinline__ float sn2_fold_images(const float* __restrict__ w, int replicas, int stride) {
+    float s0 = 0.f, s1 = 0.f, s2 = 0.f, s3 = 0.f;
+    if constexpr (R > 0) {
+        float v[R];
+#pragma unroll
+        for (int r = 0; r < R; ++r) v[r] = w[(size_t)r * stride];
+        int r = 1;
+#pragma unroll
+        for (; r + 4 <= R; r += 4) s0 += v[r], s1 += v[r + 1], s2 += v[r + 2], s3 += v[r + 3];
+#pragma unroll
+        for (; r < R; ++r) s0 += v[r];
+        return v[0] + ((s0 + s1) + (s2 + s3));
+    } else {
+        int r = 1;
+        for (; r + 4 <= replicas; r += 4) {
+            s0 += w[(size_t)r * stride];
+            s1 += w[(size_t)(r + 1) * stride];
+            s2 += w[(size_t)(r + 2) * stride];
+            s3 += w[(size_t)(r + 3) * stride];
+        }
+        for (; r < replicas; ++r) s0 += w[(size_t)r * stride];
+        return w[0] + ((s0 + s1) + (s2 + s3));
+    }
 }
 #endif
 
diff --git a/stratanet2_vegetation_coverage_maps_amd/csrc/global_level_bwd.hip b/stratanet2_vegetation_coverage_maps_amd/csrc/global_level_bwd.hip
--- a/stratanet2_vegetation_coverage_maps_amd/csrc/global_level_bwd.hip
+++ b/stratanet2_vegetation_coverage_maps_amd/csrc/global_level_bwd.hip
@@ -21,7 +21,7 @@
 constexpr int GB_LD = 68;
 constexpr int GB_WC = 33;
 constexpr int GB_TILES = GL_GROUPS * 64 * (GB_QS + GB_LD);
-constexpr int GB_FIXED_FLOATS = GB_TILES + 128 * GB_WC + 8 * 64 + 16 * 128 + 2 * 128 + 4 * 64;
+constexpr int GB_FIXED_FLOATS = GB_TILES + 128 * GB_WC + 8 * 64 + 16 * 128 + 2 * 128 + 5 * 64;
 static_assert(GB_QS >= 48, "three 16-column tiles of staged inputs");
 static_assert(GL_GROUPS * 128 * 37 <= GB_TILES, "the groups' dW | db partials go through the staging tiles");
 static_assert((GB_FIXED_FLOATS + GL_MAX_PLOTS * 128) * 4 <= 160 * 1024, "LDS");
@@ -44,6 +44,11 @@
     gl_u64* xchg;
     unsigned* ctl;
     unsigned spin_limit;
+    const float* ext2;
+    const int* arg2;
+    const float *mean2, *invstd2;
+    float *dgamma2, *dbeta2;
+    int bn2_images, bn2_stride;
 };
 
 __device__ __forceinline__ void gb_wave_sums(float (&s)[4], float* s_red, int wv, int lane, int off) {
@@ -75,7 +80,8 @@
     float* s_g = s_sdp + 64;
     float* s_x3 = s_g + 64;
     int* s_arg = reinterpret_cast<int*>(s_x3 + 64);
-    float* s_x = s_x3 + 128;
+    float* s_m2 = s_x3 + 128;
+    float* s_x = s_m2 + 64;
     __shared__ int s_fail;
     const int B = A.B, M2 = A.M2;
     const long row_lo = (long)b * M2, R_lim = row_lo + M2;
@@ -109,6 +115,7 @@
         s_arg[tid] = arg_ok ? ra : -1;
         if (arg_ok) xh_arg = (A.sa3.h[(size_t)(row_lo + ra) * 64 + tid] - m3) * is3;
         dx3_old = A.dx3[(size_t)b * 64 + tid];
+        if (A.ext2) s_m2[tid] = tid < 32 ? A.mean2[tid] : A.invstd2[tid - 32];
     }
     if (tid == 0) s_fail = 0;
     if constexpr (ONE_TRIP) {
@@ -250,13 +257,18 @@
     acc_f[0] = acc_f[1] = acc_3[0] = acc_3[1] = acc_3[2] = D[0] = D[1] = f32x4{0.f, 0.f, 0.f, 0.f};
     float4 hs[4];
     float dx2_old[2][4];
+    float e2[2][4];
+    int a2[2][4];
+    float sb2[2] = {0.f, 0.f}, sg2[2] = {0.f, 0.f};
     auto ask_block = [&](long r0) {
 #pragma unroll
         for (int jt = 0; jt < 2; ++jt)
 #pragma unroll
             for (int r = 0; r < 4; ++r) {
                 const long row = r0 + 16 * g + 4 * r4 + r;
-                dx2_old[jt][r] = A.dx2[(size_t)(row < R_lim ? row : R_lim - 1) * 32 + 16 * jt + c16];
+                const size_t w = (size_t)(row < R_lim ? row : R_lim - 1) * 32 + 16 * jt + c16;
+                dx2_old[jt][r] = A.dx2[w];
+                if (A.ext2) e2[jt][r] = A.ext2[w], a2[jt][r] = A.arg2[w];
             }
         load_rows(A.sa3.h, r0, hs);
     };
@@ -338,6 +350,19 @@
                     const long row = r0 + 16 * g + 4 * r4 + r;
                     if (row < R_lim) A.dx2[(size_t)row * 32 + 16 * jt + c16] = dx2_old[jt][r] + D[jt][r];
                 }
+            if (A.ext2) {
+#pragma unroll
+                for (int jt = 0; jt < 2; ++jt) {
+                    const float m2 = s_m2[16 * jt + c16], is2 = s_m2[32 + 16 * jt + c16];
+#pragma unroll
+                    for (int r = 0; r < 4; ++r)
+                        if (r0 + 16 * g + 4 * r4 + r < R_lim && a2[jt][r] >= 0) {
+                            const float v = dx2_old[jt][r] + D[jt][r];
+                            sb2[jt] += v;
+                            sg2[jt] = fmaf(v, (e2[jt][r] - m2) * is2, sg2[jt]);
+                        }
+                }
+            }
         }
         __syncthreads();
     }
@@ -372,6 +397,14 @@
             bn_dst[1] = tid < 64 ? A.sa3.dbeta + tid : A.sa3.dgamma + (tid - 64);
             old_bn[0] = *bn_dst[0], old_bn[1] = *bn_dst[1];
         }
+        if (A.ext2) {
+#pragma unroll
+            for (int jt = 0; jt < 2; ++jt) {
+                sb2[jt] += __shfl_xor(sb2[jt], 16), sb2[jt] += __shfl_xor(sb2[jt], 32);
+                sg2[jt] += __shfl_xor(sg2[jt], 16), sg2[jt] += __shfl_xor(sg2[jt], 32);
+                if (lane < 16) s_red[wv * 128 + 16 * jt + lane] = sb2[jt], s_red[wv * 128 + 32 + 16 * jt + lane] = sg2[jt];
+            }
+        }
 #pragma unroll
         for (int c = 0; c < 3; ++c)
 #pragma unroll
@@ -402,6 +435,13 @@
         if (bn_dst[0]) {
             *bn_dst[0] = old_bn[0] + s_bnf[tid];
             *bn_dst[1] = old_bn[1] + s_bn3[tid];
+        }
+        if (A.ext2 && tid < 64) {
+            float v = 0.f;
+#pragma unroll
+            for (int w = 0; w < 16; ++w) v += s_red[w * 128 + tid];
+            float* dst = (tid < 32 ? A.dbeta2 + tid : A.dgamma2 + (tid - 32)) + (size_t)(b % A.bn2_images) * A.bn2_stride;
+            if (v != 0.f) SN2_FLUSH_ADD(dst, v);
         }
     }
     BSTAMP(7)
@@ -461,8 +501,17 @@
     return gl_bwd_covers(B, frozen, bf16) && M2 <= GL_BWD_MAX_ROWS;
 }
 
+extern "C" int sn2_sa_bn_sums_route(int B, int M2, int frozen, int bf16) {
+    return sn2_global_level_backward_route(B, M2, frozen, bf16);
+}
+
 extern "C" int sn2_global_level_backward(const sn2_fp* sa3, const sn2_fp* fp3, const int* arg3, unsigned long long* xchg,
                                          unsigned* ctl, void* stream) {
+    return sn2_global_level_backward_below(sa3, fp3, arg3, xchg, ctl, nullptr, stream);
+}
+
+extern "C" int sn2_global_level_backward_below(const sn2_fp* sa3, const sn2_fp* fp3, const int* arg3, unsigned long long* xchg,
+                                               unsigned* ctl, const sn2_sa* below, void* stream) {
     if (!sa3 || !fp3 || !arg3 || !xchg || !ctl) return SN2_EINVAL;
     const int B = sa3->B, M2 = sa3->R_per_plot;
     if (!(B > 0 && M2 > 0 && fp3->B == B && fp3->R_per_plot == M2 && sa3->S_per_plot == M2 && fp3->S_per_plot == 1)) return SN2_EINVAL;
@@ -497,6 +546,16 @@
     A.img_stride = sa3->blk.grad_replica_stride;
     A.xchg = xchg, A.ctl = ctl;
     A.spin_limit = g_gl_spin_limit;
+    A.ext2 = nullptr, A.arg2 = nullptr, A.mean2 = A.invstd2 = nullptr, A.dgamma2 = A.dbeta2 = nullptr, A.bn2_images = 1, A.bn2_stride = 0;
+    if (below) {
+        if (below->nl < 1 || below->nl > 2) return SN2_EINVAL;
+        const sn2_block* k = &below->blk[below->nl - 1];
+        if (below->B != B || below->M != M2 || k->cout != 32 || below->dout != fp3->dskip) return SN2_EINVAL;
+        if (!below->ext || !below->arg || !k->mean || !k->invstd || !k->dgamma || !k->dbeta) return SN2_EINVAL;
+        if (k->grad_replicas > 1 && k->grad_replica_stride < 32) return SN2_EINVAL;
+        A.ext2 = below->ext, A.arg2 = below->arg, A.mean2 = k->mean, A.invstd2 = k->invstd, A.dgamma2 = k->dgamma, A.dbeta2 = k->dbeta;
+        A.bn2_images = k->grad_replicas > 1 ? k->grad_replicas : 1, A.bn2_stride = k->grad_replica_stride;
+    }
     const size_t lds = ((size_t)GB_FIXED_FLOATS + (size_t)B * 128) * 4;
     auto kern = M2 <= GL_GROUPS * 64 ? &global_level_bwd_kernel<true> : &global_level_bwd_kernel<false>;
     (void)hipFuncSetAttribute(reinterpret_cast<const void*>(kern), hipFuncAttributeMaxDynamicSharedMemorySize, (int)lds);
diff --git a/stratanet2_vegetation_coverage_maps_amd/csrc/net.hip b/stratanet2_vegetation_coverage_maps_amd/csrc/net.hip
--- a/stratanet2_vegetation_coverage_maps_amd/csrc/net.hip
+++ b/stratanet2_vegetation_coverage_maps_amd/csrc/net.hip
@@ -560,8 +560,11 @@
     pf3.dy = b->dy3, pf3.dsrc = b->dx3, pf3.dsrc_stride = 64, pf3.dskip = b->dx2, pf3.dskip_stride = 32;
     fp_desc(&p3, d, a, sa3_in(m, d, g, a), gd);
     p3.dsrc = b->dx2, p3.dsrc_stride = 32;
+    sn2_sa sa;
+    sa2_desc(&sa, m, d, g, a, gd, b->dx2, b->dx1);
     if (m->fuse_global_level && b->gl_xchg && b->gl_ctl && sn2_global_level_backward_route(B, M2, b->frozen_stats, gl_bf16(m))) {
-        SN2_TRY(sn2_global_level_backward(&p3, &pf3, a->arg3, b->gl_xchg, b->gl_ctl, cur));
+        sa.bn_sums_done = (m->fuse_sa_bn_sums && sn2_sa_bn_sums_route(B, M2, b->frozen_stats, gl_bf16(m) || m->sa2.mma_bf16)) ? 1 : 0;
+        SN2_TRY(sn2_global_level_backward_below(&p3, &pf3, a->arg3, b->gl_xchg, b->gl_ctl, sa.bn_sums_done ? &sa : nullptr, cur));
     } else {
         SN2_TRY(sn2_fp_bn_sums(&p2, m->fp3.gamma, m->fp3.beta, aux_row(a, 4, 2), aux_row(a, 4, 3), b->arena + m->fp3.ggamma,
                                b->arena + m->fp3.gbeta, b->bn_ok + 2, cur));
@@ -572,8 +575,6 @@
         p3.dy = b->dy_sa3, p3.bn_sums_done = b->bn_ok + 3;
         SN2_TRY(sn2_fp_backward(&p3, cur));
     }
-    sn2_sa sa;
-    sa2_desc(&sa, m, d, g, a, gd, b->dx2, b->dx1);
     SN2_TRY(sn2_sa_backward(&sa, cur));
     sa1_desc(&sa, m, d, g, a, gd, b->dx1, b->sa1_ws);
     SN2_TRY(sn2_sa_backward(&sa, cur));
diff --git a/stratanet2_vegetation_coverage_maps_amd/csrc/sa.hip b/stratanet2_vegetation_coverage_maps_amd/csrc/sa.hip
--- a/stratanet2_vegetation_coverage_maps_amd/csrc/sa.hip
+++ b/stratanet2_vegetation_coverage_maps_amd/csrc/sa.hip
@@ -105,10 +105,14 @@
 int backward_t(const sn2_sa* p, hipStream_t st) {
     const sn2_block* last = &p->blk[NL - 1];
     const int rows = p->B * p->M, C = last->cout;
-    int pb = sn2_cdiv(rows, 256 / C);
-    if (pb > 256) pb = 256;
-    hipLaunchKernelGGL(sa_bwd_prep_kernel, dim3(pb), dim3(256), 0, st, p->dout, p->ext, p->arg, last->mean, last->invstd,
-                       rows, C, last->dgamma, last->dbeta);
+    if (p->bn_sums_done) {
+        if (2 * C > 64) return SN2_ELIMIT;
+    } else {
+        int pb = sn2_cdiv(rows, 256 / C);
+        if (pb > 256) pb = 256;
+        hipLaunchKernelGGL(sa_bwd_prep_kernel, dim3(pb), dim3(256), 0, st, p->dout, p->ext, p->arg, last->mean, last->invstd,
+                           rows, C, last->dgamma, last->dbeta);
+    }
     if constexpr (NL == 2) {
         const sn2_block* k0 = &p->blk[0];
         if (!p->dfeat && p->bwd_ws && !k0->mma_bf16) {
diff --git a/stratanet2_vegetation_coverage_maps_amd/csrc/sa_mfma.hip b/stratanet2_vegetation_coverage_maps_amd/csrc/sa_mfma.hip
--- a/stratanet2_vegetation_coverage_maps_amd/csrc/sa_mfma.hip
+++ b/stratanet2_vegetation_coverage_maps_amd/csrc/sa_mfma.hip
@@ -416,6 +416,7 @@
     int rep_k, rep_stride;
     float* dfeat;
     float* ws;
+    int bn_images, bn_stride;
 };
 
 #ifdef SN2_SA_STAMPS
@@ -472,6 +473,16 @@
     const unsigned long long etot = *a.total;
     const float invE = (etot > 0 && !a.frozen) ? (float)(1.0 / (double)etot) : 0.f;
 
+    constexpr int CLAST = NL == 2 ? C2 : C1;
+    constexpr bool LANE_FOLD = 2 * CLAST <= 64;
+    float bn_last = 0.f;
+    if (LANE_FOLD && lane < 2 * CLAST) {
+        const float* w = NL == 2 ? (lane < CLAST ? a.dbeta1 + lane : a.dgamma1 + (lane - CLAST))
+                                 : (lane < CLAST ? a.dbeta0 + lane : a.dgamma0 + (lane - CLAST));
+        bn_last = a.bn_images == SN2_NET_GRAD_IMAGES ? sn2_fold_images<SN2_NET_GRAD_IMAGES>(w, a.bn_images, a.bn_stride)
+                                                     : sn2_fold_images<0>(w, a.bn_images, a.bn_stride);
+    }
+
     float A1[TO1][KB1], bias1[TO1][4];
 #pragma unroll
     for (int io = 0; io < TO1; ++io) {
@@ -496,7 +507,9 @@
             a1v[is][r] = NL == 2 ? a.a0[ch] : 0.f;
             c1v[is][r] = NL == 2 ? a.c0[ch] : 0.f;
             if (NL == 1 || PASS == 3) {
-                const float g = a.gamma0[ch], dg = a.dgamma0[ch], db = a.dbeta0[ch], m = mu0[is][r], s = is0[is][r];
+                const float g = a.gamma0[ch], m = mu0[is][r], s = is0[is][r];
+                const bool lf = NL == 1 && LANE_FOLD;
+                const float dg = lf ? __shfl(bn_last, CLAST + ch) : a.dgamma0[ch], db = lf ? __shfl(bn_last, ch) : a.dbeta0[ch];
                 cA0[is][r] = g * s;
                 cC0[is][r] = g * s * s * dg * invE;
                 cD0[is][r] = g * s * (m * s * dg - db) * invE;
@@ -518,7 +531,7 @@
             for (int r = 0; r < 4; ++r) {
                 const int ch = 16 * io + 4 * q + r;
                 bias2[io][r] = a.b1[ch];
-                const float g = a.gamma1[ch], dg = a.dgamma1[ch], db = a.dbeta1[ch], m = a.mean1[ch], s = a.invstd1[ch];
+                const float g = a.gamma1[ch], dg = __shfl(bn_last, CLAST + ch), db = __shfl(bn_last, ch), m = a.mean1[ch], s = a.invstd1[ch];
                 cA1[io][r] = g * s;
                 cC1[io][r] = g * s * s * dg * invE;
                 cD1[io][r] = g * s * (m * s * dg - db) * invE;
@@ -978,6 +991,7 @@
     a.rep_k = k0.grad_replicas; a.rep_stride = k0.grad_replica_stride;
     a.dfeat = p->dfeat;
     a.ws = ws;
+    a.bn_images = (p->bn_sums_done && k1.grad_replicas > 1) ? k1.grad_replicas : 1, a.bn_stride = k1.grad_replica_stride;
     int blocks = sn2_cdiv((long)p->B * p->M, 16);
     static const int occ_env = getenv("SN2_SA_BWD_OCC") ? atoi(getenv("SN2_SA_BWD_OCC")) : 0;
     const int occ = occ_env > 0 ? occ_env : (CF == 8 ? 2 : 1);
diff --git a/stratanet2_vegetation_coverage_maps_amd/executor.py b/stratanet2_vegetation_coverage_maps_amd/executor.py
--- a/stratanet2_vegetation_coverage_maps_amd/executor.py
+++ b/stratanet2_vegetation_coverage_maps_amd/executor.py
@@ -245,6 +245,7 @@
         m.max_neighbors = int(max_neighbors)
         m.drop_p = float(model.drop)
         m.fuse_global_level, m.fuse_eval_head, m.source_side = int(bool(model.fuse_global_level)), int(bool(model.fuse_eval_head)), int(bool(ops.SOURCE_SIDE))
+        m.fuse_sa_bn_sums = int(bool(model.fuse_sa_bn_sums))
         m.fps_waves_shared, m.fps_waves_many = int(model.fps_waves_shared), int(model.fps_waves_many)
         self.c = m
         self.settings = settings_of(model, max_neighbors)
@@ -268,7 +269,8 @@
 
 
 def settings_of(model, max_neighbors):
-    return (model.mma_dtype, float(model.drop), bool(model.fuse_global_level), bool(model.fuse_eval_head), bool(ops.SOURCE_SIDE),
+    return (model.mma_dtype, float(model.drop), bool(model.fuse_global_level), bool(model.fuse_eval_head), bool(model.fuse_sa_bn_sums),
+            bool(ops.SOURCE_SIDE),
             int(model.fps_waves_shared), int(model.fps_waves_many), float(model.sa1_module.r), float(model.sa2_module.r),
             float(model.sa1_module.ratio), float(model.sa2_module.ratio), int(max_neighbors), model.p2_diam_pix,
             bool(model.fp1_morton_rows))
diff --git a/stratanet2_vegetation_coverage_maps_amd/hip_ops.py b/stratanet2_vegetation_coverage_maps_amd/hip_ops.py
--- a/stratanet2_vegetation_coverage_maps_amd/hip_ops.py
+++ b/stratanet2_vegetation_coverage_maps_amd/hip_ops.py
@@ -715,7 +715,7 @@
 
 
 def sa_desc(blocks, feat, cf, spos, cpos_aos, nbr, cnt, total, B, Nsrc, M, ext, arg, out, dout=None, dfeat=None,
-            with_grads=False, order=None, bwd_ws=None) -> SA:
+            with_grads=False, order=None, bwd_ws=None, bn_sums_done=False) -> SA:
     cap = nbr.shape[1]
     cl = blocks[-1].cout
     feat_stride = _chk_rows(feat, F32, B * Nsrc, cf, "feat")
@@ -744,6 +744,7 @@
     if bwd_ws is not None:
         _chk(bwd_ws, F32, (SA_BWD_WS_WORDS,), "bwd_ws")
     d.dout, d.dfeat, d.bwd_ws = _ptr(dout), _ptr(dfeat), _ptr(bwd_ws)
+    d.bn_sums_done = int(bool(bn_sums_done))
     return d
 
 
@@ -963,11 +964,19 @@
     return bool(_host("sn2_global_level_backward_route", int(B), int(M2), int(bool(frozen)), int(any(b.mma_bf16 for b in blocks))))
 
 
-def global_level_backward(d_sa3: FP, d_fp3: FP, arg3: torch.Tensor, owner=None):
+def sa_bn_sums_fused(B: int, M2: int, frozen: bool, *blocks) -> bool:
+    return bool(_host("sn2_sa_bn_sums_route", int(B), int(M2), int(bool(frozen)), int(any(b.mma_bf16 for b in blocks))))
+
+
+def global_level_backward(d_sa3: FP, d_fp3: FP, arg3: torch.Tensor, owner=None, below: SA = None):
     B = d_sa3.B
     _chk(arg3, I32, (B, 64), "arg3")
     ws = global_level_ws(arg3.device, B, owner=owner)
-    _call("sn2_global_level_backward", d_sa3, d_fp3, _ptr(arg3), _ptr(ws[3]), _ptr(ws[4]), _stream())
+    if below is None:
+        _call("sn2_global_level_backward", d_sa3, d_fp3, _ptr(arg3), _ptr(ws[3]), _ptr(ws[4]), _stream())
+    else:
+        _call("sn2_global_level_backward_below", d_sa3, d_fp3, _ptr(arg3), _ptr(ws[3]), _ptr(ws[4]), below, _stream(),
+              key="sn2_global_level_backward")
 
 
 def global_level_gave_up(dev, warn: bool = True) -> int:
diff --git a/stratanet2_vegetation_coverage_maps_amd/point_net2.py b/stratanet2_vegetation_coverage_maps_amd/point_net2.py
--- a/stratanet2_vegetation_coverage_maps_amd/point_net2.py
+++ b/stratanet2_vegetation_coverage_maps_amd/point_net2.py
@@ -165,6 +165,7 @@
     fuse_eval_head = os.environ.get("SN2_FUSE_EVAL_HEAD", "1") == "1"
     fuse_global_level = os.environ.get("SN2_FUSE_GLOBAL_LEVEL", "1") == "1"
     fuse_loss_backward = os.environ.get("SN2_FUSE_LOSS_BACKWARD", "1") == "1"
+    fuse_sa_bn_sums = os.environ.get("SN2_FUSE_SA_BN_SUMS", "1") == "1"
     p2_diam_pix = None
 
     def set_mma_dtype(self, dtype: str):
@@ -708,7 +709,7 @@
         ops.head_forward(ops.head_desc(s.h1, b1.a, b1.c, self.lin1, self.lin2, cov, proba, drop_mask=drop_keep, drop_p=self.drop))
         return cov, proba, s
 
-    def _sa_desc(self, s, l, dout=None, dfeat=None, g=False, bwd_ws=None):
+    def _sa_desc(self, s, l, dout=None, dfeat=None, g=False, bwd_ws=None, bn_sums_done=False):
         blocks = s.b_sa[l]
         cf = blocks[0].cin - 3
         if l == 1:
@@ -717,7 +718,7 @@
             feat, spos, S = _at(s, "x", l - 1), _at(s, "pos", l - 1, "_aos"), _at(s, "M", l - 1)
         return ops.sa_desc(blocks, feat, cf, spos, _at(s, "pos", l, "_aos"), _at(s, "nbr", l), _at(s, "cnt", l), _at(s, "tot", l), s.B, S,
                            _at(s, "M", l), _at(s, "ext", l), _at(s, "arg", l), _at(s, "x", l), dout=dout, dfeat=dfeat, with_grads=g,
-                           order=getattr(s, f"ord{l}", None), bwd_ws=bwd_ws)
+                           order=getattr(s, f"ord{l}", None), bwd_ws=bwd_ws, bn_sums_done=bn_sums_done)
 
     def _global_sa_desc(self, s, **kw):
         L = len(s.b_sa)
@@ -783,9 +784,13 @@
             if j < L:
                 bn_sums(ops.fp_bn_sums, d, s.b_fp[j + 1], j)
         top, gb = s.b_fp[G], s.b_glob
+        sa_top = dict(dout=dx[L], g=True, **({"dfeat": dx[L - 1]} if L > 1 else {"bwd_ws": buf["sa1_ws"]}))
         if self.fuse_global_level and ops.global_level_backward_fused(B, Ms[L], getattr(top, "frozen", False), gb, top):
+            if self.fuse_sa_bn_sums and ops.sa_bn_sums_fused(B, Ms[L], getattr(top, "frozen", False), gb, top, *s.b_sa[L]):
+                sa_top["bn_sums_done"] = True
             ops.global_level_backward(self._global_sa_desc(s, dsrc=dx[L], with_grads=True),
-                                      self._fp_desc(s, G, dy=dy[G], dsrc=dx[G], dskip=dx[L], with_grads=True), _at(s, "arg", G), owner=self)
+                                      self._fp_desc(s, G, dy=dy[G], dsrc=dx[G], dskip=dx[L], with_grads=True), _at(s, "arg", G), owner=self,
+                                      below=self._sa_desc(s, L, **sa_top) if sa_top.get("bn_sums_done") else None)
         else:
             bn_sums(ops.fp_bn_sums, d, top, L)
             du = e(B * Ms[L], max(gb.cout, _pad4(top.cout)))
@@ -796,8 +801,8 @@
                                      views[id(gb.bn.weight)], views[id(gb.bn.bias)])
             ops.fp_backward(self._global_sa_desc(s, dy=dy_sa, dsrc=dx[L], with_grads=True, bn_sums_done=bn_ok[L + 1:L + 2]))
         for l in range(L, 1, -1):
-            ops.sa_backward(self._sa_desc(s, l, dout=dx[l], dfeat=dx[l - 1], g=True))
-        ops.sa_backward(self._sa_desc(s, 1, dout=dx[1], g=True, bwd_ws=buf["sa1_ws"]))
+            ops.sa_backward(self._sa_desc(s, l, **sa_top) if l == L else self._sa_desc(s, l, dout=dx[l], dfeat=dx[l - 1], g=True))
+        ops.sa_backward(self._sa_desc(s, 1, **sa_top) if L == 1 else self._sa_desc(s, 1, dout=dx[1], g=True, bwd_ws=buf["sa1_ws"]))
         if getattr(self, "defer_grad_reduce", False):
             self._grad_images_pending = (arena,) + tuple(images)
         else:
```

After: 24300 plots/s, median of 6. Within noise of the previous version (+0.3%).
